# HaydenFaulkner/VidDet

Hardware: AMD Instinct MI355X
Metric: frames/sec (416x416) yolo3_darknet53 fwd+bwd (higher is better)
Workload: dtype f32; 1 GPU; yolo3_darknet53_coco training, batch 64/GPU, 416x416, fp32, fwd+bwd+SGD-momentum (BASELINE configs[2]; the reference trains with SGD, not Adam); classes=80, global_batch=64, parallelism=dp1, hip_graph=False

## Files before the change

### include/viddet_hip.h

```cpp
#ifndef VIDDET_HIP_H
#define VIDDET_HIP_H

#include <stdint.h>

#ifdef __cplusplus
extern "C" {
#endif

#define VD_OK            0
#define VD_EINVAL       -1
#define VD_ELAUNCH      -2
#define VD_EWORKSPACE   -3

#define VD_MAX_TAPS 27

#define VD_EPI_AFFINE    1
#define VD_EPI_LEAKY     2
#define VD_EPI_RESIDUAL  4
#define VD_MATH_SPLIT    16
#define VD_MATH_BF16     32

#define VD_MATH_F16X2    64
#define VD_MATH_NOHALO   128
#define VD_STORE_BF16    256
#define VD_WGRAD_HALO    512
#define VD_CONV_STREAMK  1024
#define VD_CONV_PARITY4  2048
#define VD_CONV_SPLITK   4096
#define VD_SK_MAX_WG        2048
#define VD_SK_HEADER_BYTES  32768
#define VD_SK_SPLIT_CNT_OFF   4096
#define VD_SK_SPLIT_MAX_TILES 4096
#define VD_SK_TIMEOUT_TICKS 4000
#define VD_AMAX_SLOTS    32
#define VD_AMAX_STRIDE   64
#define VD_AMAX_FLOATS   (VD_AMAX_SLOTS * VD_AMAX_STRIDE)

const char* vd_last_error(void);
int vd_version(void);
#define VD_ABI_VERSION 8
int vd_abi_version(void);
int64_t vd_sizeof_desc(int which);

typedef struct {
    const float* in;
    const float* wp;
    float*       out;
    const float* scale;
    const float* shift;
    const float* residual;
    int32_t N, Hi, Wi, Ci;
    int32_t Hg, Wg;
    int32_t in_stride;
    int32_t T;
    int32_t dy[VD_MAX_TAPS], dx[VD_MAX_TAPS];
    int32_t dz[VD_MAX_TAPS];
    int32_t Kfr;
    int32_t Ho, Wo, Co;
    int32_t out_stride, out_oy, out_ox;
    int32_t ldo, ldr;
    int32_t flags;
    float   slope;
    const float* in_scale;
    const float* in_shift;
    float   in_slope;
    int32_t tile;
    float*  stats_part;
    const float* bs_z;
    const float* bs_scale;
    const float* bs_shift;
    const float* bs_mean;
    const float* bs_invstd;
    float*  bs_part;
    float   bs_slope;
    const float* amax_in;
    const float* amax_w;
    float*  amax_out;
    void*   sk_ws;
    int64_t sk_ws_bytes;
    int32_t par_cin;
    int32_t par_mask;
} vd_conv_desc;

int vd_conv_igemm(const vd_conv_desc* d, void* stream);
int vd_conv_igemm_streamk(const vd_conv_desc* d);
int64_t vd_conv_igemm_streamk_ws_bytes(void);
int vd_conv_igemm_mtiles(const vd_conv_desc* d);

int vd_conv_igemm_bf16(const vd_conv_desc* d, int out_f32, void* stream);
int vd_conv_igemm_bf16_streamk(const vd_conv_desc* d, int out_f32);
int vd_conv_igemm_bf16_mtiles(const vd_conv_desc* d);
int vd_pack_weight_bf16(const float* wp_f32, void* wp_bf16, int Co, int Co_pad, int Ci, int Ci_pad, int T,
                        void* stream);
int vd_stem_im2col_bf16(const float* in, void* col, int N, int H, int W, int nchw, void* stream);

typedef struct {
    const float* in;
    const float* dout;
    float*       dwp;
    int32_t N, Hi, Wi, Ci;
    int32_t Hg, Wg, Co, ldd;
    int32_t in_stride;
    int32_t T;
    int32_t dy[VD_MAX_TAPS], dx[VD_MAX_TAPS];
    int32_t dz[VD_MAX_TAPS];
    int32_t Kfr;
    int32_t splits;
    const float* in_scale;
    const float* in_shift;
    float   in_slope;
    int32_t flags;
    const float* amax_in;
    const float* amax_dout;
} vd_wgrad_desc;

int64_t vd_conv_wgrad_ws_bytes(const vd_wgrad_desc* d);
int vd_conv_wgrad(const vd_wgrad_desc* d, void* ws, int64_t ws_bytes, void* stream);
int vd_conv_wgrad_uses_halo(const vd_wgrad_desc* d);

int vd_stem_conv_c32_bf16(const float* x_nchw, const float* stem_wp, const float* stem_scale, const float* stem_shift,
                          float stem_slope, const vd_conv_desc* d, void* stream);
int vd_stem_conv_blocks(int N, int H, int W);
int vd_stem_conv(const float* x_nchw, const float* wp, void* out, int ldo, int N, int H, int W, const float* scale,
                 const float* shift, float slope, int flags, int out_bf16, float* stats_part, void* stream);
int64_t vd_stem_wgrad_ws_bytes(int N, int H, int W);
int vd_stem_wgrad(const float* x_nchw, const float* dz, int ldd, float* dwp, int N, int H, int W, void* ws,
                  int64_t ws_bytes, void* stream);
int vd_stem_im2col(const float* in, float* col, int N, int H, int W, int nchw, void* stream);

int vd_pack_weight_fwd(const float* w_oihw, float* wp, int Co, int Co_pad, int Ci,
                       int kd, int kh, int kw, void* stream);
int vd_pack_weight_dgrad(const float* w_oihw, float* wp, int Co, int Co_pad, int Ci,
                         int kd, int kh, int kw, const int32_t* taps, int ntaps, int src_packed,
                         void* stream);
int vd_pack_weight_dgrad_s2(const float* wp_fwd, float* wp4, int Co, int Co_pad, int Ci, int32_t* par_mask, void* stream);
int vd_unpack_wgrad(const float* dwp, float* dw_oihw, int Co, int Ci, int kd, int kh, int kw,
                    void* stream);

int64_t vd_bn_stats_ws_bytes(int64_t M, int C);
int vd_bn_stats(const float* x, int64_t M, int C, double* sums, void* ws, int64_t ws_bytes,
                void* stream);
int64_t vd_bn_sum_partials_ws_bytes(int nblk, int C);
int vd_bn_sum_partials(const float* part, int nblk, int C, double* sums, void* ws, int64_t ws_bytes, void* stream);
int vd_bn_sum_finalize(const float* part, int nblk, int C, double* sums, double count, const float* gamma,
                       const float* beta, float eps, float momentum, float* running_mean, float* running_var,
                       float* scale, float* shift, float* save_mean, float* save_invstd, void* ws, int64_t ws_bytes,
                       void* stream);
int vd_bn_sum_param_grads(const float* part, int nblk, int C, double* sums2, float* dgamma, float* dbeta, void* ws,
                          int64_t ws_bytes, void* stream);
int vd_bn_finalize(const double* sums, double count, int C, const float* gamma, const float* beta,
                   float eps, float momentum, float* running_mean, float* running_var,
                   float* scale, float* shift, float* save_mean, float* save_invstd, void* stream);
int vd_bn_fold_eval(const float* gamma, const float* beta, const float* running_mean,
                    const float* running_var, float eps, int C, float* scale, float* shift,
                    void* stream);
int vd_bn_apply_leaky(const float* x, const float* scale, const float* shift, const float* residual,
                      float* y, int64_t M, int C, float slope, float* amax_out, void* stream);
int vd_bn_stream_grid(int64_t n_vec, int cvec, int* unroll);
int vd_bn_bwd_reduce(const float* x, const float* dy, const float* scale, const float* shift,
                     const float* save_mean, const float* save_invstd, int64_t M, int C, float slope,
                     double* sums2, void* ws, int64_t ws_bytes, void* stream);
int vd_bn_param_grads(const double* sums2, int C, float* dgamma, float* dbeta, void* stream);
int vd_bn_bwd_apply(const float* x, const float* dy, const float* scale, const float* shift,
                    const float* save_mean, const float* save_invstd,
                    const double* sums2, double count, int64_t M, int C, float slope,
                    float* dx, float* amax_out , void* stream);

typedef struct {
    const float* gamma;
    const float* beta;
    const float* scale;
    int32_t C;
    int32_t pad_;
} vd_guard_item;
int vd_range_guard(const vd_guard_item* items, int n, float thresh, float* ratios, int32_t* flags, void* stream);

int vd_amax_merge(const float* a, const float* b, float* out, void* stream);
int vd_amax(const float* x, int64_t n, float* amax, void* stream);
int vd_amax_segments(const float* base, const int64_t* seg, int nseg, float* amax, void* stream);

int vd_add(const float* a, const float* b, float* out, int64_t n, void* stream);
int vd_fill(float* out, float v, int64_t n, void* stream);
int vd_upsample2x_concat(const float* up, const float* route, float* out,
                         int N, int Ho, int Wo, int Cu, int Cr, void* stream);
int vd_upsample2x_concat_bwd(const float* dout, float* dup, float* droute,
                             int N, int Ho, int Wo, int Cu, int Cr, void* stream);
int vd_nchw_to_nhwc(const float* in, float* out, int N, int C, int H, int W, void* stream);
int vd_preprocess_u8_nhwc(const uint8_t* in, float* out, int64_t npix, void* stream);
int vd_preprocess_u8_nchw(const uint8_t* in, float* out, int N, int H, int W, void* stream);
int vd_temporal_pool(const float* x, float* y, int32_t* argmax, int B, int K, int64_t inner, int type,
                     void* stream);
int vd_temporal_pool_bwd(const float* dy, const int32_t* argmax, float* dx, int B, int K,
                         int64_t inner, int type, void* stream);
int vd_frame_slice(const float* x, float* y, int B, int K, int k0, int kc, int64_t inner, int backward, void* stream);
int vd_temporal_cat(const float* x, float* y, int B, int K, int64_t hw, int C, int backward, void* stream);
int vd_corr_fwd(const float* x, float* y, int B, int K, int H, int W, int C, int d, int ldy, void* stream);
int vd_corr_bwd(const float* dy, const float* x, float* dx, int B, int K, int H, int W, int C, int d, int ldy, void* stream);
int vd_corr_fwd_bf16(const void* x, void* y, int B, int K, int H, int W, int C, int d, int ldy, void* stream);

int vd_gru_gate_fwd(const float* I, const float* H, const float* hbias, const float* hprev, float* h, int B, int K, int t,
                    int64_t HW, int Ch, void* stream);
int vd_gru_gate_bwd(float* I, float* H, int h_valid, const float* hbias, const float* hprev, const float* dy, float dy_scale,
                    float* dh, int carry, int B, int K, int t, int64_t HW, int Ch, void* stream);
int vd_gru_avg(const float* hl, const float* hr, float* y, int B, int K, int64_t inner, float* amax_out, void* stream);

int vd_tdw_fwd(const float* x, const float* w, const float* res, float* y, int B, int K, int64_t HW, int C, float* amax_out,
               void* stream);
int64_t vd_tdw_bwd_ws_bytes(int B, int K, int64_t HW, int C);
int vd_tdw_bwd(const float* dy, const float* x, const float* w, float* dx, float* dw, int B, int K, int64_t HW, int C, void* ws,
               int64_t ws_bytes, void* stream);

typedef struct {
    const float* head[3];
    int32_t g[3];
    int32_t ldh;
    float   stride[3];
    float   anchors[3][6];
    int32_t B, C;
} vd_head_desc;

int vd_yolo_decode_filter(const vd_head_desc* h, float valid_thresh,
                          float* cand_score, int32_t* cand_row, int32_t cap, int32_t* counts,
                          void* stream);
int64_t vd_nms_ws_bytes(int B, int cap, int topk);
int vd_nms_topk(const vd_head_desc* h, const float* cand_score, const int32_t* cand_row,
                int32_t cap, const int32_t* counts, float nms_thresh, int topk, int post_nms,
                float* out_ids, float* out_scores, float* out_boxes, int32_t* out_rows,
                void* ws, int64_t ws_bytes, void* stream);
int vd_yolo_decode_filter_agnostic(const vd_head_desc* h, int head_bf16, float valid_thresh,
                                   float* cand_score, int32_t* cand_row, int32_t cap, int32_t* counts,
                                   void* stream);
int vd_nms_agnostic(const vd_head_desc* h, int head_bf16, const float* cand_score, const int32_t* cand_row,
                    int32_t cap, const int32_t* counts, float nms_thresh, int topk, int post_nms,
                    float* out_ids, float* out_scores, float* out_boxes, int32_t* out_rows,
                    void* ws, int64_t ws_bytes, void* stream);

int vd_yolo_loss_fwd_bwd(const vd_head_desc* h, const float* gt, int M,
                         const float* obj_t, const float* center_t, const float* scale_t,
                         const float* weight_t, const float* class_t,
                         float ignore_thresh, int label_smooth,
                         float* losses, float* const dhead[3], float* box_out,
                         float* const dhead_amax[3] ,
                         void* ws, int64_t ws_bytes, void* stream);
int64_t vd_yolo_loss_ws_bytes(const vd_head_desc* h);

int vd_sgd_momentum(float* w, const float* grad, float* mom, int64_t n,
                    float lr, float momentum, float wd, float rescale, void* stream);

int vd_bn_stats_bf16(const void* x, int64_t M, int C, double* sums, void* ws, int64_t ws_bytes, void* stream);
int vd_bn_apply_leaky_bf16(const void* x, const float* scale, const float* shift, const void* residual, void* y,
                           int64_t M, int C, float slope, void* stream);
int vd_bn_bwd_reduce_bf16(const void* x, const void* dy, const float* scale, const float* shift, const float* save_mean,
                          const float* save_invstd, int64_t M, int C, float slope, double* sums2, void* ws, int64_t ws_bytes,
                          void* stream);
int vd_bn_bwd_apply_bf16(const void* x, const void* dy, const float* scale, const float* shift, const float* save_mean,
                         const float* save_invstd, const double* sums2, double count, int64_t M, int C, float slope,
                         void* dx, void* stream);
int vd_pack_weight_dgrad_bf16(const float* w, void* wp_bf16, int Co, int Co_pad, int Ci, int kd, int kh, int kw,
                              const int32_t* taps, int ntaps, int src_packed, void* stream);
int vd_add_bf16(const void* a, const void* b, void* out, int64_t n, void* stream);
int vd_temporal_pool_bf16(const void* x, void* y, int B, int K, int64_t inner, int type, void* stream);
int vd_upsample2x_concat_bwd_bf16(const void* dout, void* dup, void* droute, int N, int Ho, int Wo, int Cu, int Cr, void* stream);
int vd_temporal_pool_train_bf16(const void* x, void* y, uint8_t* argmax_u8, int B, int K, int64_t inner, int type, void* stream);
int vd_temporal_pool_bwd_bf16(const void* dy, const uint8_t* argmax_u8, void* dx, int B, int K, int64_t inner, int type,
                              void* stream);
int vd_corr_bwd_bf16(const void* dy, const void* x, void* dx, int B, int K, int H, int W, int C, int d, int ldy, void* stream);
int vd_stem_wgrad_bf16(const float* x_nchw, const void* dz, int ldd, float* dwp, int N, int H, int W, void* ws, int64_t ws_bytes,
                       void* stream);
int vd_yolo_loss_fwd_bwd_bf16(const vd_head_desc* h, const float* gt, int M, const float* obj_t, const float* center_t,
                              const float* scale_t, const float* weight_t, const float* class_t, float ignore_thresh,
                              int label_smooth, float* losses, void* const dhead[3], float* box_out, void* ws, int64_t ws_bytes,
                              void* stream);

int vd_temporal_pool_idx(const float* ring, const int32_t* slots, float* y, int S, int B, int K, int64_t inner, int type,
                         void* stream);
int vd_temporal_pool_idx_bf16(const void* ring, const int32_t* slots, void* y, int S, int B, int K, int64_t inner, int type,
                              void* stream);
int vd_temporal_cat_idx(const float* ring, const int32_t* slots, float* y, int S, int B, int K, int64_t hw, int C, void* stream);

int vd_resize_u8_nchw(const uint8_t* in, float* out, uint8_t* out_u8, int N, int H0, int W0, int H, int W, const int32_t* idx_y,
                      const float* w_y, int Ty, const int32_t* idx_x, const float* w_x, int Tx, void* stream);

int vd_resize_nv12_nchw(const uint8_t* in, int64_t in_bytes, int64_t frame_stride, int64_t pitch, int64_t uv_offset, float* out,
                        uint8_t* out_u8, int N, int H0, int W0, int H, int W, const int32_t* idx_y, const float* w_y, int Ty,
                        const int32_t* idx_x, const float* w_x, int Tx, int off, int gain, int ru, int rv, int gu, int gv, int bu,
                        void* stream);

int vd_augment_u8_nchw(const uint8_t* raw, const int64_t* src_off, const int32_t* src_hw, const float* color, const int32_t* idx_y,
                       const float* w_y, int Ty, const int32_t* idx_x, const float* w_x, int Tx, const float* fill, float* out, int N,
                       int K, int H, int W, void* stream);

int vd_yolo_targets(const float* gt, const float* ids, int idw, const float* mix, int N, int M, int C, int H, int W, float* obj,
                    float* ctr, float* scl, float* wgt, float* cls, void* stream);

int vd_voc_match(const float* det_ids, const float* det_scores, const float* det_boxes, int B, int N, const float* gt, int M,
                 int gt_w, float clip_hi, float iou_thresh, int32_t* rec_cls, float* rec_score, int8_t* rec_hit, int32_t* npos,
                 int32_t* ndiff, int C, void* stream);

int vd_vid_match(const double* det, int B, int N, const double* gt, int M, const double* motion_ranges, const double* area_ranges,
                 double iou_thresh, double pixel_tolerance, int32_t* rec_gt, int32_t* rec_tp, int32_t* rec_fp, int32_t* img_nig,
                 int32_t* img_ngt, int32_t* npos, int32_t* nout, int C, void* stream);

int vd_coco_match(const double* det, int B, int N, const double* gt, int M, const double* iou_thrs, const double* area_rng,
                  int32_t* rec_rank, int32_t* rec_bits, int32_t* npig, int K, void* stream);

int vd_seq_nms(const float* ids, const float* scores, const float* bboxes, const int32_t* clip_start, int V, int F, int N,
               int num_class, float link_thresh, float nms_thresh, int rescore, float* out_ids, float* out_scores,
               float* out_bboxes, int32_t* out_perm, void* ws, int64_t ws_bytes, void* stream);
int vd_seq_nms_stages(const float* ids, const float* scores, const float* bboxes, const int32_t* clip_start, int V, int F, int N,
                      int num_class, float link_thresh, float nms_thresh, int rescore, float* out_ids, float* out_scores,
                      float* out_bboxes, int32_t* out_perm, void* ws, int64_t ws_bytes, int stages, void* stream);

#define VD_TRACK_WS_PER_ROW 8
int vd_track(const float* ids, const float* scores, const float* bboxes, const int32_t* clip_start, int V, int F, int N,
             int num_class, float sigma_l, float sigma_h, float sigma_iou, int t_min, int max_age, int32_t* out_track,
             int32_t* out_len, float* out_score, void* ws, int64_t ws_bytes, void* stream);

#ifdef __cplusplus
}
#endif
#endif
```

### viddet_amd/csrc/vd_bn.hip

```cpp
#include "vd_common.h"
#include <stdlib.h>

namespace {

constexpr int RED_THREADS = 256;

template <int MODE, typename T = float>
__global__ __launch_bounds__(RED_THREADS) void k_bn_partial(const T* __restrict__ x,
                                                            const T* __restrict__ dy,
                                                            const float* __restrict__ scale,
                                                            const float* __restrict__ shift,
                                                            const float* __restrict__ mean,
                                                            const float* __restrict__ invstd, int64_t M,
                                                            int C, float slope, float* __restrict__ part) {
    __shared__ f32x4 sa[RED_THREADS], sb[RED_THREADS];
    const int cvec = C >> 2;
    const int cblk = cvec < RED_THREADS ? cvec : RED_THREADS;
    const int rl = RED_THREADS / cblk;
    const int tcol = threadIdx.x % cblk, trow = threadIdx.x / cblk;
    const int64_t rows_per_blk = vd_cdiv(M, gridDim.x);
    const int64_t r0 = (int64_t)blockIdx.x * rows_per_blk;
    int64_t r1 = r0 + rows_per_blk;
    if (r1 > M) r1 = M;
    for (int cb = 0; cb < cvec; cb += cblk) {
        const int col = cb + tcol;
        f32x4 a = {0.f, 0.f, 0.f, 0.f}, b = {0.f, 0.f, 0.f, 0.f};
        if (trow < rl && col < cvec) {
            f32x4 sc, sh, mu, is;
            if (MODE == 1) {
                sc = reinterpret_cast<const f32x4*>(scale)[col];
                sh = reinterpret_cast<const f32x4*>(shift)[col];
                mu = reinterpret_cast<const f32x4*>(mean)[col];
                is = reinterpret_cast<const f32x4*>(invstd)[col];
            }
            for (int64_t r = r0 + trow; r < r1; r += rl) {
                const f32x4 v = vd_ld4(x, r * cvec + col);
                if (MODE == 0) {
                    a += v;
                    b += v * v;
                } else {
                    const f32x4 d = vd_ld4(dy, r * cvec + col);
#pragma unroll
                    for (int e = 0; e < 4; ++e) {
                        const float u = v[e] * sc[e] + sh[e];
                        const float g = u > 0.f ? d[e] : d[e] * slope;
                        a[e] += g;
                        b[e] += g * (v[e] - mu[e]) * is[e];
                    }
                }
            }
        }
        sa[threadIdx.x] = a;
        sb[threadIdx.x] = b;
        __syncthreads();
        if (trow == 0 && col < cvec) {
            for (int j = 1; j < rl; ++j) {
                a += sa[j * cblk + tcol];
                b += sb[j * cblk + tcol];
            }
            float* dst = part + (int64_t)blockIdx.x * 2 * C;
            reinterpret_cast<f32x4*>(dst)[col] = a;
            reinterpret_cast<f32x4*>(dst + C)[col] = b;
        }
        __syncthreads();
    }
}

template <int MODE>
__global__ __launch_bounds__(RED_THREADS) void k_bn_partial_bf16x8(const __bf16* __restrict__ x, const __bf16* __restrict__ dy,
                                                                   const float* __restrict__ scale, const float* __restrict__ shift,
                                                                   const float* __restrict__ mean, const float* __restrict__ invstd,
                                                                   int64_t M, int C, float slope, float* __restrict__ part) {
    __shared__ f32x8 sa[RED_THREADS], sb[RED_THREADS];
    const int cvec = C >> 3;
    const int cblk = cvec < RED_THREADS ? cvec : RED_THREADS;
    const int rl = RED_THREADS / cblk;
    const int tcol = threadIdx.x % cblk, trow = threadIdx.x / cblk;
    const int64_t rows_per_blk = vd_cdiv(M, gridDim.x);
    const int64_t r0 = (int64_t)blockIdx.x * rows_per_blk;
    int64_t r1 = r0 + rows_per_blk;
    if (r1 > M) r1 = M;
    for (int cb = 0; cb < cvec; cb += cblk) {
        const int col = cb + tcol;
        f32x8 a, b;
#pragma unroll
        for (int e = 0; e < 8; ++e) a[e] = b[e] = 0.f;
        if (trow < rl && col < cvec) {
            f32x8 sc, sh, mu, is;
            if (MODE == 1) {
#pragma unroll
                for (int e = 0; e < 8; ++e) {
                    sc[e] = scale[col * 8 + e]; sh[e] = shift[col * 8 + e];
                    mu[e] = mean[col * 8 + e]; is[e] = invstd[col * 8 + e];
                }
            }
            for (int64_t r = r0 + trow; r < r1; r += 2 * rl) {
                const bool two = r + rl < r1;
                const f32x8 v0 = vd_ld8(x, r * cvec + col);
                const f32x8 v1 = two ? vd_ld8(x, (r + rl) * cvec + col) : f32x8{0, 0, 0, 0, 0, 0, 0, 0};
                if (MODE == 0) {
                    a += v0 + v1;
                    b += v0 * v0 + v1 * v1;
                } else {
                    const f32x8 d0 = vd_ld8(dy, r * cvec + col);
                    const f32x8 d1 = two ? vd_ld8(dy, (r + rl) * cvec + col) : f32x8{0, 0, 0, 0, 0, 0, 0, 0};
#pragma unroll
                    for (int e = 0; e < 8; ++e) {
                        const float u0 = v0[e] * sc[e] + sh[e], u1 = v1[e] * sc[e] + sh[e];
                        const float g0 = u0 > 0.f ? d0[e] : d0[e] * slope, g1 = u1 > 0.f ? d1[e] : d1[e] * slope;
                        a[e] += g0 + g1;
                        b[e] += g0 * (v0[e] - mu[e]) * is[e] + (two ? g1 * (v1[e] - mu[e]) * is[e] : 0.f);
                    }
                }
            }
        }
        sa[threadIdx.x] = a;
        sb[threadIdx.x] = b;
        __syncthreads();
        if (trow == 0 && col < cvec) {
            for (int j = 1; j < rl; ++j) {
                a += sa[j * cblk + tcol];
                b += sb[j * cblk + tcol];
            }
            float* dst = part + (int64_t)blockIdx.x * 2 * C;
#pragma unroll
            for (int e = 0; e < 8; ++e) {
                dst[col * 8 + e] = a[e];
                dst[C + col * 8 + e] = b[e];
            }
        }
        __syncthreads();
    }
}

__global__ __launch_bounds__(1024) void k_bn_sum_partials(const float* __restrict__ part, int nblk, int C2,
                                                          double* __restrict__ sums) {
    __shared__ double sh[16][64];
    const int cx = threadIdx.x & 63, sl = threadIdx.x >> 6;
    const int i = blockIdx.x * 64 + cx;
    double s = 0.0;
    if (i < C2) {
        int b = sl;
        for (; b + 48 < nblk; b += 64) {
            const float p0 = part[(int64_t)b * C2 + i], p1 = part[(int64_t)(b + 16) * C2 + i];
            const float p2 = part[(int64_t)(b + 32) * C2 + i], p3 = part[(int64_t)(b + 48) * C2 + i];
            s += (double)p0; s += (double)p1; s += (double)p2; s += (double)p3;
        }
        for (; b < nblk; b += 16) s += (double)part[(int64_t)b * C2 + i];
    }
    sh[sl][cx] = s;
    __syncthreads();
    if (sl == 0 && i < C2) {
        double t = 0.0;
// ... 41 lines not shown
__global__ void k_bn_sum_partials_l2(const double* __restrict__ in, int rows, int C2, double* __restrict__ sums) {
    const int i = blockIdx.x * blockDim.x + threadIdx.x;
    if (i >= C2) return;
    double s = 0.0;
    int r = 0;
    for (; r + 8 <= rows; r += 8) {
        double v[8];
#pragma unroll
        for (int u = 0; u < 8; ++u) v[u] = in[(int64_t)(r + u) * C2 + i];
#pragma unroll
        for (int u = 0; u < 8; ++u) s += v[u];
    }
    for (; r < rows; ++r) s += in[(int64_t)r * C2 + i];
    sums[i] = s;
}

__global__ void k_bn_finalize(const double* __restrict__ sums, double count, int C,
                              const float* __restrict__ gamma, const float* __restrict__ beta, float eps,
                              float momentum, float* __restrict__ rmean, float* __restrict__ rvar,
                              float* __restrict__ scale, float* __restrict__ shift,
                              float* __restrict__ smean, float* __restrict__ sinv) {
    const int c = blockIdx.x * blockDim.x + threadIdx.x;
    if (c >= C) return;
    const double mean = sums[c] / count;
    double var = sums[C + c] / count - mean * mean;
    if (var < 0.0) var = 0.0;
    const float invstd = (float)(1.0 / sqrt(var + (double)eps));
    const float g = gamma[c], b = beta[c];
    const float sc = g * invstd;
    scale[c] = sc;
    shift[c] = b - (float)mean * sc;
    if (smean) smean[c] = (float)mean;
    if (sinv) sinv[c] = invstd;
    if (rmean) rmean[c] = rmean[c] * momentum + (float)mean * (1.f - momentum);
    if (rvar) rvar[c] = rvar[c] * momentum + (float)var * (1.f - momentum);
}

template <int MODE>
__global__ __launch_bounds__(1024) void k_bn_sum_fused(const float* __restrict__ part, int nblk, int C, double* __restrict__ sums,
                                                       double count, const float* __restrict__ gamma,
                                                       const float* __restrict__ beta, float eps, float momentum,
                                                       float* __restrict__ rmean, float* __restrict__ rvar,
                                                       float* __restrict__ scale, float* __restrict__ shift,
                                                       float* __restrict__ smean, float* __restrict__ sinv,
                                                       float* __restrict__ dgamma, float* __restrict__ dbeta) {
    __shared__ double sh[16][64];
    const int cx = threadIdx.x & 63, sl = threadIdx.x >> 6;
    const int ch = blockIdx.x * 32 + (cx & 31);
    const int col = (cx >> 5) * C + ch;
    double s = 0.0;
    if (ch < C) {
        const int C2 = 2 * C;
        int b = sl;
        for (; b + 48 < nblk; b += 64) {
            const float p0 = part[(int64_t)b * C2 + col], p1 = part[(int64_t)(b + 16) * C2 + col];
            const float p2 = part[(int64_t)(b + 32) * C2 + col], p3 = part[(int64_t)(b + 48) * C2 + col];
            s += (double)p0; s += (double)p1; s += (double)p2; s += (double)p3;
        }
        for (; b < nblk; b += 16) s += (double)part[(int64_t)b * C2 + col];
    }
    sh[sl][cx] = s;
    __syncthreads();
    if (sl == 0 && ch < C) {
        double t = 0.0;
#pragma unroll
        for (int j = 0; j < 16; ++j) t += sh[j][cx];
        sums[col] = t;
        sh[0][cx] = t;
    }
    __syncthreads();
    if (threadIdx.x < 32 && ch < C) {
        const double a = sh[0][threadIdx.x], bq = sh[0][32 + threadIdx.x];
        if (MODE == 0) {
            const double mean = a / count;
            double var = bq / count - mean * mean;
            if (var < 0.0) var = 0.0;
            const float invstd = (float)(1.0 / sqrt(var + (double)eps));
            const float sc = gamma[ch] * invstd;
            scale[ch] = sc;
            shift[ch] = beta[ch] - (float)mean * sc;
            if (smean) smean[ch] = (float)mean;
            if (sinv) sinv[ch] = invstd;
            if (rmean) rmean[ch] = rmean[ch] * momentum + (float)mean * (1.f - momentum);
            if (rvar) rvar[ch] = rvar[ch] * momentum + (float)var * (1.f - momentum);
        } else {
            dbeta[ch] = (float)a;
            dgamma[ch] = (float)bq;
        }
    }
}

constexpr int SUMP_FUSED = 1024;

__global__ void k_bn_fold_eval(const float* __restrict__ gamma, const float* __restrict__ beta,
                               const float* __restrict__ rmean, const float* __restrict__ rvar, float eps,
                               int C, float* __restrict__ scale, float* __restrict__ shift) {
    const int c = blockIdx.x * blockDim.x + threadIdx.x;
    if (c >= C) return;
    const float sc = gamma[c] / sqrtf(rvar[c] + eps);
    scale[c] = sc;
    shift[c] = beta[c] - rmean[c] * sc;
}

template <typename T = float>
__global__ void k_bn_apply_leaky_v0(const T* __restrict__ x, const float* __restrict__ scale,
                                 const float* __restrict__ shift, const T* __restrict__ res,
                                 T* __restrict__ y, int64_t n4, int cvec, float slope, float* __restrict__ amax) {
    const int64_t i0 = (int64_t)blockIdx.x * blockDim.x + threadIdx.x;
    const int col = (int)(i0 % cvec);
    const f32x4 sc = reinterpret_cast<const f32x4*>(scale)[col];
    const f32x4 sh = reinterpret_cast<const f32x4*>(shift)[col];
    float amx = 0.f;
    for (int64_t i = i0; i < n4; i += (int64_t)gridDim.x * blockDim.x) {
        const f32x4 v = vd_ld4(x, i);
        f32x4 o;
#pragma unroll
        for (int e = 0; e < 4; ++e) {
            const float u = v[e] * sc[e] + sh[e];
            o[e] = u > 0.f ? u : u * slope;
        }
        if (res) o += vd_ld4(res, i);
        vd_st4(y, i, o);
        amx = fmaxf(amx, fmaxf(fmaxf(fabsf(o[0]), fabsf(o[1])), fmaxf(fabsf(o[2]), fabsf(o[3]))));
    }
    if (amax) vd_amax_publish(amax, amx);
}

template <typename T = float>
__global__ void k_bn_bwd_apply_v0(const T* __restrict__ x, const T* __restrict__ dy,
                               const float* __restrict__ scale, const float* __restrict__ shift,
                               const float* __restrict__ mean, const float* __restrict__ invstd,
                               const double* __restrict__ sums2, double count, int64_t n4, int C,
                               float slope, T* __restrict__ dx, float* __restrict__ amax) {
    const int cvec = C >> 2;
    const float inv_count = (float)(1.0 / count);
    const int64_t i0 = (int64_t)blockIdx.x * blockDim.x + threadIdx.x;
    const int col = (int)(i0 % cvec);
    const f32x4 sc = reinterpret_cast<const f32x4*>(scale)[col];
    const f32x4 sh = reinterpret_cast<const f32x4*>(shift)[col];
    const f32x4 mu = reinterpret_cast<const f32x4*>(mean)[col];
    const f32x4 is = reinterpret_cast<const f32x4*>(invstd)[col];
    f32x4 mg, mgx;
#pragma unroll
    for (int e = 0; e < 4; ++e) {
        mg[e] = (float)sums2[col * 4 + e] * inv_count;
        mgx[e] = (float)sums2[C + col * 4 + e] * inv_count;
    }
    float amx = 0.f;
    for (int64_t i = i0; i < n4; i += (int64_t)gridDim.x * blockDim.x) {
        const f32x4 v = vd_ld4(x, i);
        const f32x4 d = vd_ld4(dy, i);
        f32x4 o;
#pragma unroll
        for (int e = 0; e < 4; ++e) {
            const float u = v[e] * sc[e] + sh[e];
            const float g = u > 0.f ? d[e] : d[e] * slope;
            const float xh = (v[e] - mu[e]) * is[e];
            o[e] = sc[e] * (g - mg[e] - xh * mgx[e]);
        }
        vd_st4(dx, i, o);
        amx = fmaxf(amx, fmaxf(fmaxf(fabsf(o[0]), fabsf(o[1])), fmaxf(fabsf(o[2]), fabsf(o[3]))));
    }
    if (amax) vd_amax_publish(amax, amx);
}

typedef unsigned int u32x2 __attribute__((ext_vector_type(2)));
typedef unsigned int u32x4 __attribute__((ext_vector_type(4)));
template <int V> struct bn_vec { typedef f32x4 type; };
template <> struct bn_vec<8> { typedef f32x8 type; };

template <int V, bool NT> struct bn_io;
template <bool NT> struct bn_io<4, NT> {
    static __device__ __forceinline__ f32x4 ld(const float* p, int64_t i) {
        const f32x4* q = reinterpret_cast<const f32x4*>(p) + i;
        return NT ? __builtin_nontemporal_load(q) : *q;
    }
    static __device__ __forceinline__ f32x4 ld(const __bf16* p, int64_t i) {
        const u32x2* q = reinterpret_cast<const u32x2*>(p) + i;
        const vd_bf16x4 v = __builtin_bit_cast(vd_bf16x4, NT ? __builtin_nontemporal_load(q) : *q);
        return f32x4{(float)v[0], (float)v[1], (float)v[2], (float)v[3]};
    }
    template <typename T> static __device__ __forceinline__ void st(T* p, int64_t i, const f32x4 v) { vd_st4(p, i, v); }
};
template <bool NT> struct bn_io<8, NT> {
    static __device__ __forceinline__ f32x8 ld(const __bf16* p, int64_t i) {
        const u32x4* q = reinterpret_cast<const u32x4*>(p) + i;
        const vd_bf16x8 v = __builtin_bit_cast(vd_bf16x8, NT ? __builtin_nontemporal_load(q) : *q);
        f32x8 o;
#pragma unroll
        for (int e = 0; e < 8; ++e) o[e] = (float)v[e];
        return o;
    }
    static __device__ __forceinline__ void st(__bf16* p, int64_t i, const f32x8 v) { vd_st8(p, i, v); }
};

template <int V, typename VEC> __device__ __forceinline__ float bn_vec_amax(float amx, const VEC o) {
    float m = fmaxf(fmaxf(fabsf(o[0]), fabsf(o[1])), fmaxf(fabsf(o[2]), fabsf(o[3])));
    if (V == 8) m = fmaxf(m, fmaxf(fmaxf(fabsf(o[4]), fabsf(o[5])), fmaxf(fabsf(o[6]), fabsf(o[7]))));
    return fmaxf(amx, m);
}

template <typename T, int V, int U, bool NT, bool FULL, typename VEC>
__device__ __forceinline__ void bn_apply_trip(const T* __restrict__ x, const T* __restrict__ res, T* __restrict__ y, int64_t i,
                                              int64_t stride, int64_t nv, const VEC sc, const VEC sh, float slope, float& amx) {
    VEC v[U], r[U];
    bool ok[U];
#pragma unroll
    for (int j = 0; j < U; ++j) {
        ok[j] = FULL || i + j * stride < nv;
        if (ok[j]) v[j] = bn_io<V, NT>::ld(x, i + j * stride);
    }
    if (res) {
#pragma unroll
        for (int j = 0; j < U; ++j)
            if (ok[j]) r[j] = bn_io<V, false>::ld(res, i + j * stride);
    }
    __builtin_amdgcn_sched_barrier(0);
#pragma unroll
    for (int j = 0; j < U; ++j) {
        if (!ok[j]) continue;
        VEC o;
#pragma unroll
        for (int e = 0; e < V; ++e) {
            const float u = v[j][e] * sc[e] + sh[e];
            o[e] = u > 0.f ? u : u * slope;
        }
        if (res) o += r[j];
        bn_io<V, false>::st(y, i + j * stride, o);
        amx = bn_vec_amax<V>(amx, o);
    }
}

template <typename T, int V, int U, bool NT>
__global__ __launch_bounds__(256) void k_bn_apply_leaky(const T* __restrict__ x, const float* __restrict__ scale,
                                                        const float* __restrict__ shift, const T* __restrict__ res,
                                                        T* __restrict__ y, int64_t nv, int cvec, float slope,
                                                        float* __restrict__ amax, int step) {
    typedef typename bn_vec<V>::type VEC;
    const int64_t span = (int64_t)step * 256;
    const int64_t i = (int64_t)(blockIdx.x / step) * U * span + (blockIdx.x % step) * 256 + threadIdx.x;
    const int col = (int)(i % cvec);
    VEC sc, sh;
#pragma unroll
    for (int e = 0; e < V; ++e) {
        sc[e] = scale[col * V + e];
        sh[e] = shift[col * V + e];
    }
    float amx = 0.f;
    if (i + (U - 1) * span < nv) bn_apply_trip<T, V, U, NT, true>(x, res, y, i, span, nv, sc, sh, slope, amx);
    else if (i < nv) bn_apply_trip<T, V, U, NT, false>(x, res, y, i, span, nv, sc, sh, slope, amx);
    if (amax) vd_amax_publish(amax, amx);
}

template <typename VEC> struct bn_bwd_consts { VEC sc, sh, mu, is, mg, mgx; };

template <typename T, int V, int U, bool NT, bool FULL, typename VEC>
__device__ __forceinline__ void bn_bwd_trip(const T* __restrict__ x, const T* __restrict__ dy, T* __restrict__ dx, int64_t i,
                                            int64_t stride, int64_t nv, const bn_bwd_consts<VEC>& k, float slope, float& amx) {
    VEC v[U], d[U];
    bool ok[U];
#pragma unroll
    for (int j = 0; j < U; ++j) {
        ok[j] = FULL || i + j * stride < nv;
        if (ok[j]) {
            v[j] = bn_io<V, NT>::ld(x, i + j * stride);
            d[j] = bn_io<V, NT>::ld(dy, i + j * stride);
        }
    }
    __builtin_amdgcn_sched_barrier(0);
#pragma unroll
    for (int j = 0; j < U; ++j) {
        if (!ok[j]) continue;
        VEC o;
#pragma unroll
        for (int e = 0; e < V; ++e) {
            const float u = v[j][e] * k.sc[e] + k.sh[e];
            const float g = u > 0.f ? d[j][e] : d[j][e] * slope;
            const float xh = (v[j][e] - k.mu[e]) * k.is[e];
            o[e] = k.sc[e] * (g - k.mg[e] - xh * k.mgx[e]);
        }
        bn_io<V, false>::st(dx, i + j * stride, o);
        amx = bn_vec_amax<V>(amx, o);
    }
}

template <typename T, int V, int U, bool NT>
__global__ __launch_bounds__(256) void k_bn_bwd_apply(const T* __restrict__ x, const T* __restrict__ dy,
                                                      const float* __restrict__ scale, const float* __restrict__ shift,
                                                      const float* __restrict__ mean, const float* __restrict__ invstd,
                                                      const double* __restrict__ sums2, double count, int64_t nv, int C,
                                                      float slope, T* __restrict__ dx, float* __restrict__ amax, int step) {
    typedef typename bn_vec<V>::type VEC;
    const int cvec = C / V;
    const float inv_count = (float)(1.0 / count);
    const int64_t span = (int64_t)step * 256;
    const int64_t i = (int64_t)(blockIdx.x / step) * U * span + (blockIdx.x % step) * 256 + threadIdx.x;
    const int col = (int)(i % cvec);
    bn_bwd_consts<VEC> k;
#pragma unroll
    for (int e = 0; e < V; ++e) {
        k.sc[e] = scale[col * V + e];
        k.sh[e] = shift[col * V + e];
        k.mu[e] = mean[col * V + e];
        k.is[e] = invstd[col * V + e];
        k.mg[e] = (float)sums2[col * V + e] * inv_count;
        k.mgx[e] = (float)sums2[C + col * V + e] * inv_count;
    }
    float amx = 0.f;
    if (i + (U - 1) * span < nv) bn_bwd_trip<T, V, U, NT, true>(x, dy, dx, i, span, nv, k, slope, amx);
    else if (i < nv) bn_bwd_trip<T, V, U, NT, false>(x, dy, dx, i, span, nv, k, slope, amx);
    if (amax) vd_amax_publish(amax, amx);
}

__global__ void k_bn_param_grads(const double* __restrict__ sums2, int C, float* __restrict__ dgamma,
                                 float* __restrict__ dbeta) {
    const int c = blockIdx.x * blockDim.x + threadIdx.x;
    if (c >= C) return;
    dbeta[c] = (float)sums2[c];
    dgamma[c] = (float)sums2[C + c];
}

bool bf16x8_enabled() {
    static const int v = getenv("VD_BN_BF16X8") ? atoi(getenv("VD_BN_BF16X8")) : 1;
    return v != 0;
}

int red_blocks(int64_t M) {
    int64_t nb = vd_cdiv(M, 64);
    if (nb > 1024) nb = 1024;
    if (nb < 1) nb = 1;
    return (int)nb;
}

int stream_blocks(int64_t n) {
    int64_t nb = vd_cdiv(n, 256);
    if (nb > 4096) nb = 4096;
    if (nb < 1) nb = 1;
    return (int)nb;
}

int fixed_col_blocks(int64_t n4, int cvec) {
    int a = 256, b = cvec;
    while (b) { const int t = a % b; a = b; b = t; }
    const int64_t step = cvec / a;
    int64_t nb = stream_blocks(n4);
    nb = vd_cdiv(nb, step) * step;
    return (int)nb;
}

bool bn_stream_enabled() {
    static const int v = getenv("VD_BN_STREAM") ? atoi(getenv("VD_BN_STREAM")) : 1;
    return v != 0;
}

constexpr int64_t BN_NT_MIN_BYTES = (int64_t)128 << 20;
constexpr int BN_UNROLL = 4;

int stream_step(int cvec) {
    int a = 256, b = cvec;
    while (b) { const int t = a % b; a = b; b = t; }
    return cvec / a;
}

int64_t stream_grid(int64_t nv, int cvec) {
    const int64_t step = stream_step(cvec);
    return vd_cdiv(nv, BN_UNROLL * step * 256) * step;
}

bool aligned16(const void* a, const void* b, const void* c) {
    return (((uintptr_t)a | (uintptr_t)b | (uintptr_t)c) & 15) == 0;
}

template <typename T, int V>
void launch_apply(const T* x, const float* scale, const float* shift, const T* res, T* y, int64_t M, int C, float slope,
                  float* amax, hipStream_t s) {
    const int cvec = C / V;
    const int64_t nv = M * cvec;
    const int step = stream_step(cvec);
    const dim3 g((unsigned)stream_grid(nv, cvec)), b(256);
    const bool nt = nv * V * (int64_t)sizeof(T) >= BN_NT_MIN_BYTES;
#define VD_GO(NT_) hipLaunchKernelGGL((k_bn_apply_leaky<T, V, BN_UNROLL, NT_>), g, b, 0, s, x, scale, shift, res, y, nv, cvec, slope, amax, step)
    if (nt) VD_GO(true); else VD_GO(false);
#undef VD_GO
}

template <typename T, int V>
void launch_bwd_apply(const T* x, const T* dy, const float* scale, const float* shift, const float* mean, const float* invstd,
                      const double* sums2, double count, int64_t M, int C, float slope, T* dx, float* amax, hipStream_t s) {
    const int cvec = C / V;
    const int64_t nv = M * cvec;
    const int step = stream_step(cvec);
    const dim3 g((unsigned)stream_grid(nv, cvec)), b(256);
    const bool nt = nv * V * (int64_t)sizeof(T) >= BN_NT_MIN_BYTES;
#define VD_GO(NT_) hipLaunchKernelGGL((k_bn_bwd_apply<T, V, BN_UNROLL, NT_>), g, b, 0, s, x, dy, scale, shift, mean, invstd, sums2, count, nv, C, slope, dx, amax, step)
    if (nt) VD_GO(true); else VD_GO(false);
#undef VD_GO
}

__global__ void k_range_guard(const vd_guard_item* __restrict__ items, float thresh, float* __restrict__ ratios,
                              int32_t* __restrict__ flags) {
    const vd_guard_item it = items[blockIdx.x];
    float lo[2] = {3.0e38f, 3.0e38f}, hi[2] = {0.f, 0.f};
    for (int c = threadIdx.x; c < it.C; c += blockDim.x) {
        const float u = fabsf(it.gamma[c]) + fabsf(it.beta[c]);
        const float v = it.scale ? fabsf(it.scale[c]) : 1.f;
        lo[0] = fminf(lo[0], u); hi[0] = fmaxf(hi[0], u);
        lo[1] = fminf(lo[1], v); hi[1] = fmaxf(hi[1], v);
    }
    __shared__ float red[4][4];
#pragma unroll
    for (int k = 0; k < 2; ++k) {
#pragma unroll
        for (int off = 32; off > 0; off >>= 1) {
            lo[k] = fminf(lo[k], __shfl_xor(lo[k], off));
            hi[k] = fmaxf(hi[k], __shfl_xor(hi[k], off));
        }
    }
    const int wave = threadIdx.x >> 6;
    if ((threadIdx.x & 63) == 0) { red[wave][0] = lo[0]; red[wave][1] = hi[0]; red[wave][2] = lo[1]; red[wave][3] = hi[1]; }
    __syncthreads();
    if (threadIdx.x == 0) {
        const int nw = blockDim.x >> 6;
        float a = red[0][0], b = red[0][1], c2 = red[0][2], d = red[0][3];
        for (int w = 1; w < nw; ++w) { a = fminf(a, red[w][0]); b = fmaxf(b, red[w][1]); c2 = fminf(c2, red[w][2]); d = fmaxf(d, red[w][3]); }
        const float r0 = b > 0.f ? a / b : 1.f, r1 = d > 0.f ? c2 / d : 1.f;
        ratios[2 * blockIdx.x] = r0;
        ratios[2 * blockIdx.x + 1] = r1;
        flags[2 * blockIdx.x] = r0 < thresh ? 1 : 0;
        flags[2 * blockIdx.x + 1] = r1 < thresh ? 1 : 0;
    }
}

}
// ... 251 lines not shown
```

### viddet_amd/csrc/vd_stem.hip

```cpp
#include "vd_common.h"
#include <stdlib.h>

namespace {

typedef __bf16 bf16x4 __attribute__((ext_vector_type(4)));

constexpr int SC = 32;
constexpr int SK = 27;
constexpr int SPX = 256;

template <bool OUT_BF16, bool MF = false>
__global__ __launch_bounds__(SPX) void k_stem_fwd(const float* __restrict__ x, const float* __restrict__ w,
                                                  void* __restrict__ out, int ldo, int N, int H, int W,
                                                  const float* __restrict__ scale, const float* __restrict__ shift,
                                                  float slope, int flags, float* __restrict__ stats_part) {
    __shared__ float tile[SPX][SC + 1];
    if constexpr (MF) {
        typedef __bf16 bf16x8_t __attribute__((ext_vector_type(8)));
        const int tid = threadIdx.x, lane = tid & 63, wave = tid >> 6;
        const int64_t HW = (int64_t)H * W;
        const int64_t P = (int64_t)N * HW;
        const int hh = lane >> 5;
        bf16x8_t b0, b1;
#pragma unroll
        for (int e = 0; e < 8; ++e) {
            b0[e] = (__bf16)w[(lane & 31) * 32 + 8 * hh + e];
            b1[e] = (__bf16)w[(lane & 31) * 32 + 16 + 8 * hh + e];
        }
#pragma unroll
        for (int gsel = 0; gsel < 2; ++gsel) {
            const int prow = wave * 64 + gsel * 32 + (lane & 31);
            const int64_t pix = (int64_t)blockIdx.x * SPX + prow;
            bf16x8_t a0, a1;
            {
                const bool pin = pix < P;
                const int64_t pp = pin ? pix : 0;
                const int n = (int)(pp / HW);
                const int r = (int)(pp - (int64_t)n * HW);
                const int y = r / W, xx = r - y * W;
                const float* xn = x + (int64_t)n * 3 * HW;
                float v[16];
#pragma unroll
                for (int e = 0; e < 16; ++e) {
                    const int k = (e < 8 ? 8 * hh : 16 + 8 * hh) + (e & 7);
                    const int tap = k / 3, c = k - 3 * tap;
                    const int iy = y + tap / 3 - 1, ix = xx + tap % 3 - 1;
                    const bool ok = pin && k < SK && (unsigned)iy < (unsigned)H && (unsigned)ix < (unsigned)W;
                    const float t = xn[ok ? (int64_t)c * HW + (int64_t)iy * W + ix : 0];
                    v[e] = ok ? t : 0.f;
                }
#pragma unroll
                for (int e = 0; e < 8; ++e) { a0[e] = (__bf16)v[e]; a1[e] = (__bf16)v[8 + e]; }
            }
            f32x16 acc;
#pragma unroll
            for (int r2 = 0; r2 < 16; ++r2) acc[r2] = 0.f;
            acc = __builtin_amdgcn_mfma_f32_32x32x16_bf16(a0, b0, acc, 0, 0, 0);
            acc = __builtin_amdgcn_mfma_f32_32x32x16_bf16(a1, b1, acc, 0, 0, 0);
            const int co = lane & 31;
            const float sc = (flags & VD_EPI_AFFINE) ? scale[co] : 1.f, sh = (flags & VD_EPI_AFFINE) ? shift[co] : 0.f;
#pragma unroll
            for (int r2 = 0; r2 < 16; ++r2) {
                float t = acc[r2];
                if (flags & VD_EPI_AFFINE) t = t * sc + sh;
                if (flags & VD_EPI_LEAKY) t = t > 0.f ? t : t * slope;
                tile[wave * 64 + gsel * 32 + (r2 & 3) + 8 * (r2 >> 2) + 4 * hh][co] = t;
            }
        }
        __syncthreads();
    } else {
    __shared__ __attribute__((aligned(16))) float wT[SK][SC];
    const int tid = threadIdx.x;
    for (int i = tid; i < SK * SC; i += SPX) wT[i / SC][i % SC] = w[(i % SC) * 32 + i / SC];
    __syncthreads();
    const int64_t HW = (int64_t)H * W;
    const int64_t P = (int64_t)N * HW;
    const int64_t pix = (int64_t)blockIdx.x * SPX + tid;
    float acc[SC];
#pragma unroll
    for (int c = 0; c < SC; ++c) acc[c] = 0.f;
    if (pix < P) {
        const int n = (int)(pix / HW);
        const int r = (int)(pix - (int64_t)n * HW);
        const int y = r / W, xx = r - y * W;
        const float* xn = x + (int64_t)n * 3 * HW;
        float xv[SK];
#pragma unroll
        for (int ky = 0; ky < 3; ++ky)
#pragma unroll
            for (int kx = 0; kx < 3; ++kx) {
                const int iy = y + ky - 1, ix = xx + kx - 1;
                const bool ok = (unsigned)iy < (unsigned)H && (unsigned)ix < (unsigned)W;
                const int64_t o = ok ? (int64_t)iy * W + ix : 0;
#pragma unroll
                for (int c = 0; c < 3; ++c) {
                    const float t = xn[(int64_t)c * HW + o];
                    xv[(ky * 3 + kx) * 3 + c] = ok ? t : 0.f;
                }
            }
#pragma unroll
        for (int k = 0; k < SK; ++k) {
#pragma unroll
            for (int c4 = 0; c4 < SC; c4 += 4) {
                const f32x4 wv = *reinterpret_cast<const f32x4*>(&wT[k][c4]);
#pragma unroll
                for (int e = 0; e < 4; ++e) acc[c4 + e] = fmaf(xv[k], wv[e], acc[c4 + e]);
            }
            __builtin_amdgcn_sched_barrier(0);
        }
    }
#pragma unroll
    for (int c = 0; c < SC; ++c) {
        float v = acc[c];
        if (flags & VD_EPI_AFFINE) v = v * scale[c] + shift[c];
        if (flags & VD_EPI_LEAKY) v = v > 0.f ? v : v * slope;
        tile[tid][c] = v;
    }
    __syncthreads();
    }
    const int tid = threadIdx.x;
    const int64_t P = (int64_t)N * H * W;
    if (stats_part) {
        __shared__ float red[8][2 * SC];
        const int c = tid & 31, seg = tid >> 5;
        float s1 = 0.f, s2 = 0.f;
#pragma unroll 8
        for (int r = seg * 32; r < seg * 32 + 32; ++r) {
            const float v = tile[r][c];
            s1 += v;
            s2 += v * v;
        }
        red[seg][c] = s1;
        red[seg][SC + c] = s2;
        __syncthreads();
        if (tid < 2 * SC) {
            float t = 0.f;
#pragma unroll
            for (int q = 0; q < 8; ++q) t += red[q][tid];
            stats_part[(int64_t)blockIdx.x * 2 * SC + tid] = t;
        }
    }
    const int64_t p0 = (int64_t)blockIdx.x * SPX;
#pragma unroll
    for (int j = 0; j < 8; ++j) {
        const int pl = (tid >> 3) + 32 * j, c4 = (tid & 7) * 4;
        if (p0 + pl < P) {
            const f32x4 v = {tile[pl][c4], tile[pl][c4 + 1], tile[pl][c4 + 2], tile[pl][c4 + 3]};
            if (OUT_BF16) {
                bf16x4 o;
#pragma unroll
                for (int e = 0; e < 4; ++e) o[e] = (__bf16)v[e];
                *reinterpret_cast<bf16x4*>(reinterpret_cast<__bf16*>(out) + (p0 + pl) * ldo + c4) = o;
            } else {
                *reinterpret_cast<f32x4*>(reinterpret_cast<float*>(out) + (p0 + pl) * ldo + c4) = v;
            }
        }
    }
}

template <typename T>
__global__ __launch_bounds__(256) void k_stem_wgrad(const float* __restrict__ x, const T* __restrict__ dz, int ldd,
                                                    float* __restrict__ part, int N, int H, int W, int64_t px_per_wave) {
    const int lane = threadIdx.x & 63, wave = threadIdx.x >> 6;
    const int64_t HW = (int64_t)H * W, P = (int64_t)N * HW;
    const int64_t gw = (int64_t)blockIdx.x * 4 + wave;
    const int64_t p_begin = gw * px_per_wave;
    int64_t p_end = p_begin + px_per_wave;
    if (p_end > P) p_end = P;
    const int k = lane & 31, par = lane >> 5;
    const bool k_ok = k < SK;
    const int c = k_ok ? k % 3 : 0, tap = k_ok ? k / 3 : 0;
    const int dy = tap / 3 - 1, dx = tap % 3 - 1;
    f32x16 acc;
#pragma unroll
    for (int r = 0; r < 16; ++r) acc[r] = 0.f;
    int64_t p = p_begin + par;
    int n = 0, y = 0, xx = 0;
    if (p < P) {
        n = (int)(p / HW);
        const int r = (int)(p - (int64_t)n * HW);
        y = r / W;
        xx = r - y * W;
    }
    constexpr int UNR = 8;
    for (; p - par < p_end; p += 2 * UNR) {
        float a[UNR], b[UNR];
#pragma unroll
        for (int u = 0; u < UNR; ++u) {
            const int64_t pu = p + 2 * u;
            const bool in_run = pu < p_end;
            a[u] = in_run ? (float)dz[pu * ldd + k] : 0.f;
            const int iy = y + dy, ix = xx + dx;
            const bool ok = in_run && k_ok && (unsigned)iy < (unsigned)H && (unsigned)ix < (unsigned)W;
            b[u] = ok ? x[((int64_t)n * 3 + c) * HW + (int64_t)iy * W + ix] : 0.f;
            xx += 2;
            while (xx >= W) { xx -= W; ++y; }
            if (y >= H) { y -= H; ++n; }
        }
#pragma unroll
        for (int u = 0; u < UNR; ++u) acc = __builtin_amdgcn_mfma_f32_32x32x2f32(a[u], b[u], acc, 0, 0, 0);
    }
    float* dst = part + gw * (SC * 32);
#pragma unroll
    for (int r = 0; r < 16; ++r) {
        const int co = (r & 3) + 8 * (r >> 2) + 4 * (lane >> 5);
        dst[co * 32 + (lane & 31)] = acc[r];
    }
}

constexpr int SROWS = 4;
template <typename T>
__global__ __launch_bounds__(256) void k_stem_wgrad_rows(const float* __restrict__ x, const T* __restrict__ dz, int ldd,
                                                         float* __restrict__ part, int N, int H, int W, int P) {
    extern __shared__ float win[];
    const int tid = threadIdx.x, lane = tid & 63, wave = tid >> 6;
    const int groups = (H + SROWS - 1) / SROWS;
    const int n = blockIdx.x / groups, y0 = (blockIdx.x % groups) * SROWS;
    const int64_t HW = (int64_t)H * W;
    const float* xn = x + (int64_t)n * 3 * HW;
    for (int i = tid; i < 3 * (SROWS + 2) * P; i += 256) {
        const int col = i % P - 1, rr = i / P;
        const int c = rr / (SROWS + 2), iy = y0 - 1 + rr % (SROWS + 2);
        const bool ok = (unsigned)iy < (unsigned)H && (unsigned)col < (unsigned)W;
        win[i] = ok ? xn[(int64_t)c * HW + (int64_t)iy * W + col] : 0.f;
    }
    __syncthreads();
    const int k = lane & 31, par = lane >> 5;
    const bool k_ok = k < SK;
    const int c = k_ok ? k % 3 : 0, tap = k_ok ? k / 3 : 0;
    const int y = y0 + wave;
    f32x16 acc;
#pragma unroll
    for (int r = 0; r < 16; ++r) acc[r] = 0.f;
    if (y < H) {
        const float* b0 = win + (c * (SROWS + 2) + wave + tap / 3) * P + (tap % 3) + par;
        const T* a0 = dz + ((int64_t)n * HW + (int64_t)y * W + par) * ldd + k;
        constexpr int UNR = 8;
        for (int x0 = 0; x0 < W; x0 += 2 * UNR) {
            float a[UNR], b[UNR];
#pragma unroll
            for (int u = 0; u < UNR; ++u) {
                const bool in = x0 + 2 * u + par < W;
                a[u] = in ? (float)a0[(int64_t)(x0 + 2 * u) * ldd] : 0.f;
                b[u] = (in && k_ok) ? b0[x0 + 2 * u] : 0.f;
            }
#pragma unroll
            for (int u = 0; u < UNR; ++u) acc = __builtin_amdgcn_mfma_f32_32x32x2f32(a[u], b[u], acc, 0, 0, 0);
        }
    }
    __syncthreads();
#pragma unroll
    for (int r = 0; r < 16; ++r) {
        const int co = (r & 3) + 8 * (r >> 2) + 4 * (lane >> 5);
        win[wave * (SC * 32) + co * 32 + (lane & 31)] = acc[r];
    }
    __syncthreads();
    float* dst = part + (int64_t)blockIdx.x * (SC * 32);
    for (int i = tid; i < SC * 32; i += 256)
        dst[i] = ((win[i] + win[SC * 32 + i]) + win[2 * SC * 32 + i]) + win[3 * SC * 32 + i];
}

__global__ void k_stem_wgrad_reduce(const float* __restrict__ part, int nparts, float* __restrict__ dst) {
    const int i = blockIdx.x * blockDim.x + threadIdx.x;
    if (i >= SC * 32) return;
    const int per = (nparts + gridDim.y - 1) / gridDim.y;
    int q = blockIdx.y * per;
    int q1 = q + per;
    if (q1 > nparts) q1 = nparts;
    float s = 0.f;
    for (; q + 8 <= q1; q += 8) {
        float v[8];
#pragma unroll
        for (int u = 0; u < 8; ++u) v[u] = part[(int64_t)(q + u) * (SC * 32) + i];
#pragma unroll
        for (int u = 0; u < 8; ++u) s += v[u];
    }
    for (; q < q1; ++q) s += part[(int64_t)q * (SC * 32) + i];
    dst[(int64_t)blockIdx.y * (SC * 32) + i] = s;
}

constexpr int STEM_RED_CHUNKS = 64;
constexpr int64_t STEM_WG_WAVES = 8192;

}

extern "C" {

int vd_stem_conv_blocks(int N, int H, int W) { return (int)vd_cdiv((int64_t)N * H * W, SPX); }

int vd_stem_conv(const float* x_nchw, const float* wp, void* out, int ldo, int N, int H, int W, const float* scale,
                 const float* shift, float slope, int flags, int out_bf16, float* stats_part, void* stream) {
    VD_REQUIRE(x_nchw && wp && out && N > 0 && H > 0 && W > 0 && ldo >= SC && ldo % 4 == 0, "vd_stem_conv: bad args");
    VD_REQUIRE(!(flags & VD_EPI_AFFINE) || (scale && shift), "vd_stem_conv: affine epilogue needs scale and shift");
    VD_REQUIRE(!stats_part || flags == 0, "vd_stem_conv: fused statistics need the raw output (they come from the fp32 values, bf16 output or not)");
    VD_REQUIRE((int64_t)N * H * W < (1ll << 31), "vd_stem_conv: pixel count overflows int32");
    const int nb = vd_stem_conv_blocks(N, H, W);
    static const int use_mf = getenv("VD_STEM_MFMA") ? atoi(getenv("VD_STEM_MFMA")) : 1;
    if (out_bf16 && use_mf)
        hipLaunchKernelGGL((k_stem_fwd<true, true>), dim3(nb), dim3(SPX), 0, (hipStream_t)stream, x_nchw, wp, out, ldo, N, H, W,
                           scale, shift, slope, flags, stats_part);
    else if (out_bf16)
        hipLaunchKernelGGL(k_stem_fwd<true>, dim3(nb), dim3(SPX), 0, (hipStream_t)stream, x_nchw, wp, out, ldo, N, H, W,
                           scale, shift, slope, flags, stats_part);
    else
        hipLaunchKernelGGL(k_stem_fwd<false>, dim3(nb), dim3(SPX), 0, (hipStream_t)stream, x_nchw, wp, out, ldo, N, H, W,
                           scale, shift, slope, flags, stats_part);
    VD_CHECK_LAUNCH("vd_stem_conv");
    return VD_OK;
}

static int stem_rows_pitch(int W) {
    int p = W + 2;
    while (p % 32 != 4) ++p;
    return p;
}
static int64_t stem_rows_lds(int W) {
    const int64_t win = (int64_t)3 * (SROWS + 2) * stem_rows_pitch(W) * 4, tiles = (int64_t)4 * SC * 32 * 4;
    return win > tiles ? win : tiles;
}
static bool stem_rows_ok(int W) {
    static const int on = getenv("VD_STEM_WGRAD_ROWS") ? atoi(getenv("VD_STEM_WGRAD_ROWS")) : 1;
    return on && stem_rows_lds(W) <= 64 * 1024;
}
static int64_t stem_run_waves(int N, int H, int W) {
    const int64_t P = (int64_t)N * H * W;
    int64_t waves = vd_cdiv(P, 256);
    if (waves > STEM_WG_WAVES) waves = STEM_WG_WAVES;
    return vd_cdiv(waves, 4) * 4;
}

int64_t vd_stem_wgrad_ws_bytes(int N, int H, int W) {
    const int64_t tiles_rows = (int64_t)N * vd_cdiv(H, SROWS), tiles_run = stem_run_waves(N, H, W);
    const int64_t tiles = tiles_rows > tiles_run ? tiles_rows : tiles_run;
    return (tiles + STEM_RED_CHUNKS) * SC * 32 * (int64_t)sizeof(float);
}

static int stem_wgrad_any(const float* x_nchw, const void* dz, int dz_bf16, int ldd, float* dwp, int N, int H, int W, void* ws,
                         int64_t ws_bytes, void* stream) {
    VD_REQUIRE(x_nchw && dz && dwp && N > 0 && H > 0 && W > 0 && ldd >= SC, "vd_stem_wgrad: bad args");
    const int64_t need = vd_stem_wgrad_ws_bytes(N, H, W);
    if (!ws || ws_bytes < need) {
        vd_set_error("vd_stem_wgrad: workspace %lld < %lld", (long long)ws_bytes, (long long)need);
        return VD_EWORKSPACE;
    }
    hipStream_t s = (hipStream_t)stream;
    int64_t tiles;
    if (stem_rows_ok(W)) {
        tiles = (int64_t)N * vd_cdiv(H, SROWS);
        const int P = stem_rows_pitch(W), lds = (int)stem_rows_lds(W);
        if (dz_bf16)
            hipLaunchKernelGGL(k_stem_wgrad_rows<__bf16>, dim3((unsigned)tiles), dim3(256), lds, s, x_nchw, (const __bf16*)dz, ldd,
                               (float*)ws, N, H, W, P);
        else
            hipLaunchKernelGGL(k_stem_wgrad_rows<float>, dim3((unsigned)tiles), dim3(256), lds, s, x_nchw, (const float*)dz, ldd,
                               (float*)ws, N, H, W, P);
    } else {
        const int64_t P = (int64_t)N * H * W;
        tiles = stem_run_waves(N, H, W);
        int64_t ppw = vd_cdiv(P, tiles);
        ppw = vd_cdiv(ppw, 2) * 2;
        if (dz_bf16)
            hipLaunchKernelGGL(k_stem_wgrad<__bf16>, dim3((unsigned)(tiles / 4)), dim3(256), 0, s, x_nchw, (const __bf16*)dz, ldd, (float*)ws,
                               N, H, W, ppw);
        else
            hipLaunchKernelGGL(k_stem_wgrad<float>, dim3((unsigned)(tiles / 4)), dim3(256), 0, s, x_nchw, (const float*)dz, ldd, (float*)ws,
                               N, H, W, ppw);
    }
    VD_CHECK_LAUNCH("vd_stem_wgrad");
    float* lvl1 = (float*)ws + tiles * (SC * 32);
    hipLaunchKernelGGL(k_stem_wgrad_reduce, dim3(4, STEM_RED_CHUNKS), dim3(256), 0, s, (const float*)ws, (int)tiles, lvl1);
    VD_CHECK_LAUNCH("vd_stem_wgrad/reduce1");
    hipLaunchKernelGGL(k_stem_wgrad_reduce, dim3(4, 1), dim3(256), 0, s, (const float*)lvl1, STEM_RED_CHUNKS, dwp);
    VD_CHECK_LAUNCH("vd_stem_wgrad/reduce2");
    return VD_OK;
}

int vd_stem_wgrad(const float* x_nchw, const float* dz, int ldd, float* dwp, int N, int H, int W, void* ws, int64_t ws_bytes,
                  void* stream) {
    return stem_wgrad_any(x_nchw, dz, 0, ldd, dwp, N, H, W, ws, ws_bytes, stream);
}

int vd_stem_wgrad_bf16(const float* x_nchw, const void* dz, int ldd, float* dwp, int N, int H, int W, void* ws, int64_t ws_bytes,
                       void* stream) {
    return stem_wgrad_any(x_nchw, dz, 1, ldd, dwp, N, H, W, ws, ws_bytes, stream);
}

}
```

### viddet_amd/lib.py

```python
import ctypes as C
import os

_HERE = os.path.dirname(os.path.abspath(__file__))
LIB_PATH = os.environ.get("VD_LIB") or os.path.join(_HERE, "csrc", "libviddet_hip.so")

ABI_VERSION = 8
VOC_MATCH_MAX_DET, VOC_MATCH_MAX_GT = 1024, 512
VID_MATCH_MAX_DET, VID_MATCH_MAX_GT = 1024, 512
COCO_MATCH_MAX_DET, COCO_MATCH_MAX_GT = 1024, 512
SEQ_NMS_MAX_ROWS = 128
SEQ_NMS_WS_PER_ROW = 48
TRACK_MAX_ROWS, TRACK_MAX_ACTIVE = 128, 1024
TRACK_WS_PER_ROW = 8
VD_MAX_TAPS = 27
EPI_AFFINE, EPI_LEAKY, EPI_RESIDUAL = 1, 2, 4
MATH_SPLIT = 16
MATH_BF16 = 32
MATH_F16X2 = 64
MATH_NOHALO = 128
STORE_BF16 = 256
WGRAD_HALO = 512
CONV_STREAMK = 1024
CONV_SPLITK = 4096
CONV_PARITY4 = 2048
SK_HEADER_BYTES = 32768
AMAX_SLOTS, AMAX_STRIDE = 32, 64
AMAX_FLOATS = AMAX_SLOTS * AMAX_STRIDE
BN_STREAM_UNROLL = 4

_fp = C.c_void_p


class ConvDesc(C.Structure):
    _fields_ = [
        ("in_", _fp), ("wp", _fp), ("out", _fp), ("scale", _fp), ("shift", _fp), ("residual", _fp),
        ("N", C.c_int32), ("Hi", C.c_int32), ("Wi", C.c_int32), ("Ci", C.c_int32),
        ("Hg", C.c_int32), ("Wg", C.c_int32), ("in_stride", C.c_int32), ("T", C.c_int32),
        ("dy", C.c_int32 * VD_MAX_TAPS), ("dx", C.c_int32 * VD_MAX_TAPS), ("dz", C.c_int32 * VD_MAX_TAPS),
        ("Kfr", C.c_int32),
        ("Ho", C.c_int32), ("Wo", C.c_int32), ("Co", C.c_int32),
        ("out_stride", C.c_int32), ("out_oy", C.c_int32), ("out_ox", C.c_int32),
        ("ldo", C.c_int32), ("ldr", C.c_int32), ("flags", C.c_int32), ("slope", C.c_float),
        ("in_scale", _fp), ("in_shift", _fp), ("in_slope", C.c_float), ("tile", C.c_int32),
        ("stats_part", _fp),
        ("bs_z", _fp), ("bs_scale", _fp), ("bs_shift", _fp), ("bs_mean", _fp), ("bs_invstd", _fp), ("bs_part", _fp),
        ("bs_slope", C.c_float),
        ("amax_in", _fp), ("amax_w", _fp), ("amax_out", _fp),
        ("sk_ws", _fp), ("sk_ws_bytes", C.c_int64),
        ("par_cin", C.c_int32), ("par_mask", C.c_int32),
    ]


class WgradDesc(C.Structure):
    _fields_ = [
        ("in_", _fp), ("dout", _fp), ("dwp", _fp),
        ("N", C.c_int32), ("Hi", C.c_int32), ("Wi", C.c_int32), ("Ci", C.c_int32),
        ("Hg", C.c_int32), ("Wg", C.c_int32), ("Co", C.c_int32), ("ldd", C.c_int32),
        ("in_stride", C.c_int32), ("T", C.c_int32),
        ("dy", C.c_int32 * VD_MAX_TAPS), ("dx", C.c_int32 * VD_MAX_TAPS), ("dz", C.c_int32 * VD_MAX_TAPS),
        ("Kfr", C.c_int32), ("splits", C.c_int32),
        ("in_scale", _fp), ("in_shift", _fp), ("in_slope", C.c_float), ("flags", C.c_int32),
        ("amax_in", _fp), ("amax_dout", _fp),
    ]


class GuardItem(C.Structure):
    _fields_ = [("gamma", _fp), ("beta", _fp), ("scale", _fp), ("C", C.c_int32), ("pad_", C.c_int32)]


class HeadDesc(C.Structure):
    _fields_ = [
        ("head", _fp * 3), ("g", C.c_int32 * 3), ("ldh", C.c_int32),
        ("stride", C.c_float * 3), ("anchors", (C.c_float * 6) * 3),
        ("B", C.c_int32), ("C", C.c_int32),
    ]


_i, _i64, _f, _d, _p = C.c_int, C.c_int64, C.c_float, C.c_double, C.c_void_p
SIGNATURES = {
    "vd_last_error": (C.c_char_p, []),
    "vd_version": (_i, []),
    "vd_abi_version": (_i, []),
    "vd_sizeof_desc": (_i64, [_i]),
    "vd_conv_igemm": (_i, [C.POINTER(ConvDesc), _p]),
    "vd_conv_igemm_mtiles": (_i, [C.POINTER(ConvDesc)]),
    "vd_conv_igemm_streamk": (_i, [C.POINTER(ConvDesc)]),
    "vd_conv_igemm_streamk_ws_bytes": (_i64, []),
    "vd_conv_igemm_bf16": (_i, [C.POINTER(ConvDesc), _i, _p]),
    "vd_conv_igemm_bf16_mtiles": (_i, [C.POINTER(ConvDesc)]),
    "vd_conv_igemm_bf16_streamk": (_i, [C.POINTER(ConvDesc), _i]),
    "vd_pack_weight_bf16": (_i, [_p, _p, _i, _i, _i, _i, _i, _p]),
    "vd_stem_im2col_bf16": (_i, [_p, _p, _i, _i, _i, _i, _p]),
    "vd_conv_wgrad_ws_bytes": (_i64, [C.POINTER(WgradDesc)]),
    "vd_conv_wgrad": (_i, [C.POINTER(WgradDesc), _p, _i64, _p]),
    "vd_conv_wgrad_uses_halo": (_i, [C.POINTER(WgradDesc)]),
    "vd_stem_im2col": (_i, [_p, _p, _i, _i, _i, _i, _p]),
    "vd_pack_weight_fwd": (_i, [_p, _p, _i, _i, _i, _i, _i, _i, _p]),
    "vd_pack_weight_dgrad": (_i, [_p, _p, _i, _i, _i, _i, _i, _i, C.POINTER(C.c_int32), _i, _i, _p]),
    "vd_pack_weight_dgrad_s2": (_i, [_p, _p, _i, _i, _i, C.POINTER(C.c_int32), _p]),
    "vd_unpack_wgrad": (_i, [_p, _p, _i, _i, _i, _i, _i, _p]),
    "vd_bn_stats_ws_bytes": (_i64, [_i64, _i]),
    "vd_bn_stats": (_i, [_p, _i64, _i, _p, _p, _i64, _p]),
    "vd_bn_sum_partials_ws_bytes": (_i64, [_i, _i]),
    "vd_bn_sum_partials": (_i, [_p, _i, _i, _p, _p, _i64, _p]),
    "vd_bn_finalize": (_i, [_p, _d, _i, _p, _p, _f, _f, _p, _p, _p, _p, _p, _p, _p]),
    "vd_bn_sum_finalize": (_i, [_p, _i, _i, _p, _d, _p, _p, _f, _f, _p, _p, _p, _p, _p, _p, _p, _i64, _p]),
    "vd_bn_sum_param_grads": (_i, [_p, _i, _i, _p, _p, _p, _p, _i64, _p]),
    "vd_bn_fold_eval": (_i, [_p, _p, _p, _p, _f, _i, _p, _p, _p]),
    "vd_bn_stream_grid": (_i, [_i64, _i, _p]),
    "vd_bn_apply_leaky": (_i, [_p, _p, _p, _p, _p, _i64, _i, _f, _p, _p]),
    "vd_bn_bwd_reduce": (_i, [_p, _p, _p, _p, _p, _p, _i64, _i, _f, _p, _p, _i64, _p]),
    "vd_bn_param_grads": (_i, [_p, _i, _p, _p, _p]),
    "vd_bn_bwd_apply": (_i, [_p, _p, _p, _p, _p, _p, _p, _d, _i64, _i, _f, _p, _p, _p]),
    "vd_range_guard": (_i, [_p, _i, _f, _p, _p, _p]),
    "vd_amax": (_i, [_p, _i64, _p, _p]),
    "vd_amax_segments": (_i, [_p, _p, _i, _p, _p]),
    "vd_amax_merge": (_i, [_p, _p, _p, _p]),
    "vd_add": (_i, [_p, _p, _p, _i64, _p]),
    "vd_fill": (_i, [_p, _f, _i64, _p]),
    "vd_upsample2x_concat": (_i, [_p, _p, _p, _i, _i, _i, _i, _i, _p]),
    "vd_upsample2x_concat_bwd": (_i, [_p, _p, _p, _i, _i, _i, _i, _i, _p]),
    "vd_nchw_to_nhwc": (_i, [_p, _p, _i, _i, _i, _i, _p]),
    "vd_stem_conv_blocks": (_i, [_i, _i, _i]),
    "vd_stem_conv": (_i, [_p, _p, _p, _i, _i, _i, _i, _p, _p, C.c_float, _i, _i, _p, _p]),
    "vd_stem_conv_c32_bf16": (_i, [_p, _p, _p, _p, C.c_float, C.POINTER(ConvDesc), _p]),
    "vd_stem_wgrad_ws_bytes": (_i64, [_i, _i, _i]),
    "vd_stem_wgrad": (_i, [_p, _p, _i, _p, _i, _i, _i, _p, _i64, _p]),
    "vd_preprocess_u8_nhwc": (_i, [_p, _p, _i64, _p]),
    "vd_preprocess_u8_nchw": (_i, [_p, _p, _i, _i, _i, _p]),
    "vd_temporal_pool": (_i, [_p, _p, _p, _i, _i, _i64, _i, _p]),
    "vd_temporal_pool_bwd": (_i, [_p, _p, _p, _i, _i, _i64, _i, _p]),
    "vd_temporal_cat": (_i, [_p, _p, _i, _i, _i64, _i, _i, _p]),
    "vd_corr_fwd": (_i, [_p, _p, _i, _i, _i, _i, _i, _i, _i, _p]),
    "vd_corr_bwd": (_i, [_p, _p, _p, _i, _i, _i, _i, _i, _i, _i, _p]),
    "vd_corr_fwd_bf16": (_i, [_p, _p, _i, _i, _i, _i, _i, _i, _i, _p]),
    "vd_corr_bwd_bf16": (_i, [_p, _p, _p, _i, _i, _i, _i, _i, _i, _i, _p]),
    "vd_gru_gate_fwd": (_i, [_p, _p, _p, _p, _p, _i, _i, _i, _i64, _i, _p]),
    "vd_gru_gate_bwd": (_i, [_p, _p, _i, _p, _p, _p, _f, _p, _i, _i, _i, _i, _i64, _i, _p]),
    "vd_gru_avg": (_i, [_p, _p, _p, _i, _i, _i64, _p, _p]),
    "vd_tdw_fwd": (_i, [_p, _p, _p, _p, _i, _i, _i64, _i, _p, _p]),
    "vd_tdw_bwd_ws_bytes": (_i64, [_i, _i, _i64, _i]),
    "vd_tdw_bwd": (_i, [_p, _p, _p, _p, _p, _i, _i, _i64, _i, _p, _i64, _p]),
    "vd_frame_slice": (_i, [_p, _p, _i, _i, _i, _i, _i64, _i, _p]),
    "vd_yolo_decode_filter": (_i, [C.POINTER(HeadDesc), _f, _p, _p, C.c_int32, _p, _p]),
    "vd_nms_ws_bytes": (_i64, [_i, _i, _i]),
    "vd_nms_topk": (_i, [C.POINTER(HeadDesc), _p, _p, C.c_int32, _p, _f, _i, _i, _p, _p, _p, _p, _p, _i64, _p]),
    "vd_yolo_decode_filter_agnostic": (_i, [C.POINTER(HeadDesc), _i, _f, _p, _p, C.c_int32, _p, _p]),
    "vd_nms_agnostic": (_i, [C.POINTER(HeadDesc), _i, _p, _p, C.c_int32, _p, _f, _i, _i, _p, _p, _p, _p, _p, _i64, _p]),
    "vd_yolo_loss_ws_bytes": (_i64, [C.POINTER(HeadDesc)]),
    "vd_yolo_loss_fwd_bwd": (_i, [C.POINTER(HeadDesc), _p, _i, _p, _p, _p, _p, _p, _f, _i, _p,
                                  C.POINTER(_fp * 3), _p, C.POINTER(_fp * 3), _p, _i64, _p]),
    "vd_sgd_momentum": (_i, [_p, _p, _p, _i64, _f, _f, _f, _f, _p]),
    "vd_bn_stats_bf16": (_i, [_p, _i64, _i, _p, _p, _i64, _p]),
    "vd_bn_apply_leaky_bf16": (_i, [_p, _p, _p, _p, _p, _i64, _i, _f, _p]),
    "vd_bn_bwd_reduce_bf16": (_i, [_p, _p, _p, _p, _p, _p, _i64, _i, _f, _p, _p, _i64, _p]),
    "vd_bn_bwd_apply_bf16": (_i, [_p, _p, _p, _p, _p, _p, _p, _d, _i64, _i, _f, _p, _p]),
    "vd_add_bf16": (_i, [_p, _p, _p, _i64, _p]),
    "vd_temporal_pool_bf16": (_i, [_p, _p, _i, _i, _i64, _i, _p]),
    "vd_temporal_pool_train_bf16": (_i, [_p, _p, _p, _i, _i, _i64, _i, _p]),
    "vd_temporal_pool_bwd_bf16": (_i, [_p, _p, _p, _i, _i, _i64, _i, _p]),
    "vd_pack_weight_dgrad_bf16": (_i, [_p, _p, _i, _i, _i, _i, _i, _i, C.POINTER(C.c_int32), _i, _i, _p]),
    "vd_upsample2x_concat_bwd_bf16": (_i, [_p, _p, _p, _i, _i, _i, _i, _i, _p]),
    "vd_stem_wgrad_bf16": (_i, [_p, _p, _i, _p, _i, _i, _i, _p, _i64, _p]),
    "vd_yolo_loss_fwd_bwd_bf16": (_i, [C.POINTER(HeadDesc), _p, _i, _p, _p, _p, _p, _p, _f, _i, _p,
                                       C.POINTER(_fp * 3), _p, _p, _i64, _p]),
    "vd_temporal_pool_idx": (_i, [_p, _p, _p, _i, _i, _i, _i64, _i, _p]),
    "vd_temporal_pool_idx_bf16": (_i, [_p, _p, _p, _i, _i, _i, _i64, _i, _p]),
    "vd_temporal_cat_idx": (_i, [_p, _p, _p, _i, _i, _i, _i64, _i, _p]),
    "vd_resize_u8_nchw": (_i, [_p, _p, _p, _i, _i, _i, _i, _i, _p, _p, _i, _p, _p, _i, _p]),
    "vd_resize_nv12_nchw": (_i, [_p, _i64, _i64, _i64, _i64, _p, _p, _i, _i, _i, _i, _i, _p, _p, _i, _p, _p, _i,
                                 _i, _i, _i, _i, _i, _i, _i, _p]),
    "vd_augment_u8_nchw": (_i, [_p, _p, _p, _p, _p, _p, _i, _p, _p, _i, _p, _p, _i, _i, _i, _i, _p]),
    "vd_yolo_targets": (_i, [_p, _p, _i, _p, _i, _i, _i, _i, _i, _p, _p, _p, _p, _p, _p]),
    "vd_voc_match": (_i, [_p, _p, _p, _i, _i, _p, _i, _i, _f, _f, _p, _p, _p, _p, _p, _i, _p]),
    "vd_vid_match": (_i, [_p, _i, _i, _p, _i, _p, _p, _d, _d, _p, _p, _p, _p, _p, _p, _p, _i, _p]),
    "vd_coco_match": (_i, [_p, _i, _i, _p, _i, _p, _p, _p, _p, _p, _i, _p]),
    "vd_seq_nms": (_i, [_p, _p, _p, _p, _i, _i, _i, _i, _f, _f, _i, _p, _p, _p, _p, _p, _i64, _p]),
    "vd_seq_nms_stages": (_i, [_p, _p, _p, _p, _i, _i, _i, _i, _f, _f, _i, _p, _p, _p, _p, _p, _i64, _i, _p]),
    "vd_track": (_i, [_p, _p, _p, _p, _i, _i, _i, _i, _f, _f, _f, _i, _i, _p, _p, _p, _p, _i64, _p]),
}

_lib = None


class VidDetHipError(RuntimeError):
    pass


def load():
    global _lib
    if _lib is not None:
        return _lib
    if not os.path.exists(LIB_PATH):
        raise VidDetHipError(
            "libviddet_hip.so not built (%s). Run `python -c 'import __graft_entry__ as g; g.build()'` "
            "or `make -C viddet_amd/csrc`. There is no CPU fallback." % LIB_PATH)
    import torch
    lib = C.CDLL(LIB_PATH)
    for name, (res, args) in SIGNATURES.items():
        fn = getattr(lib, name)
        fn.restype = res
        fn.argtypes = args
    if lib.vd_abi_version() != ABI_VERSION:
        raise VidDetHipError("%s has ABI revision %d, this binding is written for %d: rebuild (make -C viddet_amd/csrc)"
                             % (LIB_PATH, lib.vd_abi_version(), ABI_VERSION))
    for i, st in enumerate((ConvDesc, WgradDesc, HeadDesc)):
        if lib.vd_sizeof_desc(i) != C.sizeof(st):
            raise VidDetHipError("%s: sizeof(%s) is %d in the library, %d in this binding" %
                                 (LIB_PATH, st.__name__, lib.vd_sizeof_desc(i), C.sizeof(st)))
    _lib = lib
    return lib


def check(rc, what=""):
    if rc != 0:
        raise VidDetHipError("%s failed (rc=%d): %s" % (what, rc, load().vd_last_error().decode()))


def stream_ptr():
    import torch
    return C.c_void_p(torch.cuda.current_stream().cuda_stream)


def ptr(t):
    if t is None:
        return None
    return C.c_void_p(t.data_ptr())
```

### viddet_amd/model.py

```python
import ctypes as C
import math
import os
import re
from collections import OrderedDict

import numpy as np
import torch

from . import lib as L
from . import ops
from .lib import ConvDesc, WgradDesc, EPI_AFFINE, EPI_LEAKY, EPI_RESIDUAL
from .ops import round_up, fwd_taps, dgrad_plans

from .consts import BN_EPS, BN_MOMENTUM, LEAKY_SLOPE


class Slot:

    def __init__(self):
        self.value = None


class Program:

    def __init__(self):
        self.recs = []
        self.meta = []
        self.keep = []
        self.streams = []

    def add(self, fname, *args, meta=None, stream=None):
        fn = getattr(L.load(), fname)
        self.recs.append((fname, fn, args))
        self.meta.append(meta)
        self.streams.append(stream)

    def add_py(self, fn):
        self.recs.append((None, fn, ()))
        self.meta.append(None)
        self.streams.append(None)

    def add_coll(self, fn):
        self.recs.append((None, fn, ()))
        self.meta.append(dict(kind='collective'))
        self.streams.append(None)

    def hold(self, *objs):
        self.keep.extend(objs)

    def run(self):
        s = L.stream_ptr()
        for (fname, fn, args), st in zip(self.recs, self.streams):
            if fname is None:
                fn()
                continue
            a = [x.value if isinstance(x, Slot) else x for x in args]
            rc = fn(*a, s if st is None else C.c_void_p(st.cuda_stream))
            if rc != 0:
                L.check(rc, fname)

    def run_timed(self, select):
        s = L.stream_ptr()
        out = []
        for (fname, fn, args), meta in zip(self.recs, self.meta):
            if fname is None:
                if meta and meta.get('kind') == 'collective':
                    fn()
                continue
            a = [x.value if isinstance(x, Slot) else x for x in args]
            if fname in select:
                e0, e1 = torch.cuda.Event(enable_timing=True), torch.cuda.Event(enable_timing=True)
                e0.record()
                rc = fn(*a, s)
                e1.record()
                if fname in ("vd_conv_igemm", "vd_conv_wgrad"):
                    d = args[0]._obj
                    meta = dict(meta or {}, split=bool(d.flags & L.MATH_SPLIT), bf16=bool(d.flags & L.MATH_BF16),
                                f16x2=bool(d.flags & L.MATH_F16X2), nohalo=bool(d.flags & L.MATH_NOHALO), tile=int(getattr(d, "tile", 0)),
                                streamk=bool(fname == "vd_conv_igemm" and L.load().vd_conv_igemm_streamk(args[0])))
                    if fname == "vd_conv_wgrad":
                        meta["wgrad_halo"] = bool(L.load().vd_conv_wgrad_uses_halo(args[0]))
                    if fname == "vd_conv_igemm" and meta.get("bytes"):
                        out_bytes = 4.0 * d.N * d.Hg * d.Wg * d.Co
                        extra = (out_bytes if d.residual else 0.0) + (out_bytes if getattr(d, "bs_part", None) else 0.0)
                        meta["bytes_epilogue_reads"] = extra
                        meta["bytes"] = meta["bytes"] + extra
                if fname == "vd_conv_igemm_bf16":
                    form = int(L.load().vd_conv_igemm_bf16_streamk(args[0], args[1]))
                    meta = dict(meta or {}, tile=int(args[0]._obj.tile), nohalo=bool(args[0]._obj.flags & L.MATH_NOHALO),
                                streamk=form == 1, splitk=form == 2)
                out.append((fname, meta, e0, e1))
            else:
                rc = fn(*a, s)
            if rc != 0:
                L.check(rc, fname)
        return out


class TuneCache(dict):

    def __init__(self):
        super().__init__()
        self._loaded, self._dirty, self.tuned, self.hits, self._synced_world = False, False, 0, 0, 1

    @staticmethod
    def library_id():
        import hashlib
        here = os.path.dirname(os.path.abspath(__file__))
        srcs = [os.path.join(here, "csrc", f) for f in ("vd_conv.hip", "vd_conv_igemm.h", "vd_conv_sk.hip", "vd_conv_par.hip",
                                                         "vd_conv_bf16.hip", "vd_conv_igemm_bf16.h", "vd_conv_bf16_sk.hip", "vd_conv_c32_bf16.hip",
                                                         "vd_wgrad_halo.hip", "vd_common.h")]
        h = hashlib.sha256()
        if all(os.path.exists(f) for f in srcs):
            for f in srcs:
                h.update(open(f, "rb").read())
        else:
            h.update(open(L.LIB_PATH, "rb").read())
        for sw in ("VD_WGRAD_RESERVE",):
            if os.environ.get(sw):
                h.update(("%s=%s" % (sw, os.environ[sw])).encode())
        return h.hexdigest()[:12]

    def path(self):
        p = os.environ.get("VD_TUNE_CACHE", "")
        if p.lower() in ("off", "0", "none"):
            return None
        if p:
            return p
        return os.path.join(os.path.dirname(os.path.abspath(__file__)), "tune", "gfx950_%s.json" % self.library_id())

    @staticmethod
    def _world():
        if not torch.distributed.is_available() or not torch.distributed.is_initialized():
            return 1
        return torch.distributed.get_world_size()

    @staticmethod
    def device_arch():
        if not torch.cuda.is_available():
            return None
        return str(torch.cuda.get_device_properties(torch.cuda.current_device()).gcnArchName).split(":")[0]

    def _read_file(self):
        import ast
        import json
        out = {}
        p = self.path()
        if p is None or not os.path.exists(p):
            return out
        try:
            doc = json.load(open(p))
            if doc.get("library") not in (None, self.library_id()):
                return out
            arch = self.device_arch()
            if arch is not None and doc.get("device") not in (None, arch):
                return out
            for k, v in doc.get("entries", {}).items():
                out[ast.literal_eval(k)] = tuple(v) if isinstance(v, list) else v
        except (OSError, ValueError, SyntaxError) as e:
            print("viddet_amd: ignoring tuning table %s (%s)" % (p, e), flush=True)
            return {}
        return out

    def load(self):
        self._loaded = True
        world = self._world()
        self._synced_world = world
        if world > 1 and os.environ.get("VD_TUNE_AGREE", "1") != "0":
            box = [self._read_file() if torch.distributed.get_rank() == 0 else None]
            torch.distributed.broadcast_object_list(box, src=0)
            dict.clear(self)
            entries = box[0]
        else:
            entries = self._read_file()
        for key, v in entries.items():
            if not dict.__contains__(self, key):
                dict.__setitem__(self, key, v)

    def __contains__(self, key):
        if not self._loaded or self._synced_world != self._world():
            self.load()
        hit = dict.__contains__(self, key)
        self.hits += int(hit)
        return hit

    def __setitem__(self, key, value):
# ... 1021 lines not shown
            else:
                kind = 'stem_weight' if n.stem else 'conv_weight'
                reg(n.name + ".0.weight", n.weight_shape(), kind, n, wv, gv, off=n.w_off)
                n.gamma = self.weights[n.gamma_off:n.gamma_off + n.cout]
                n.beta = self.weights[n.beta_off:n.beta_off + n.cout]
                n.ggamma = self.grads[n.gamma_off:n.gamma_off + n.cout]
                n.gbeta = self.grads[n.beta_off:n.beta_off + n.cout]
                c64 = round_up(n.cout, 64)
                n.rmean = self.running[n.stat_off:n.stat_off + n.cout]
                n.rvar = self.running[n.stat_off + c64:n.stat_off + c64 + n.cout]
                reg(n.name + ".1.gamma", (n.cout,), 'vector', n, n.gamma, n.ggamma, off=n.gamma_off)
                reg(n.name + ".1.beta", (n.cout,), 'vector', n, n.beta, n.gbeta, off=n.beta_off)
                reg(n.name + ".1.running_mean", (n.cout,), 'vector', n, n.rmean, None, trainable=False)
                reg(n.name + ".1.running_var", (n.cout,), 'vector', n, n.rvar, None, trainable=False)
                t = getattr(n, 'tdw', None)
                if t is not None:
                    t.w = self.weights[t.w_off:t.w_off + t.w_numel]
                    t.gw = self.grads[t.w_off:t.w_off + t.w_numel]
                    reg(t.pname, (t.C, 1, 3, 1, 1), 'vector', t, t.w, t.gw, off=t.w_off)
        self._params = P
        self._opt_ranges = None

    @property
    def classes(self):
        return self._classes

    def collect_params(self, select=None):
        return self._params if select is None else self._params.select(select)

    def hybridize(self, active=True):
        return None

    def set_nms(self, nms_thresh=0.45, nms_topk=400, post_nms=100):
        self.nms_thresh, self.nms_topk, self.post_nms = nms_thresh, nms_topk, post_nms
        self._programs = {k: v for k, v in self._programs.items() if k[0] not in ('infer', 'infer_bf16', 'stream', 'stream_bf16')}
        self._graph_cache.clear()

    def initialize(self, init='uniform', seed=233, obj_bias=0.0):
        g = torch.Generator(device='cpu').manual_seed(seed)
        for name, p in self._params.items():
            if name.endswith('weight'):
                if init == 'uniform':
                    v = (torch.rand(p.shape, generator=g) * 2 - 1) * 0.07
                else:
                    fan = int(np.prod(p.shape[1:]))
                    v = torch.randn(p.shape, generator=g) * math.sqrt(2.0 / fan)
                    if 'prediction' in name:
                        v *= 0.05
                p.set_data(v)
            elif name.endswith('gamma') or name.endswith('running_var'):
                v = torch.ones(p.shape)
                if init == 'he' and name.endswith('gamma') and '.body.1.1.' in name and name.startswith('stages'):
                    v *= 0.3
                p.set_data(v)
            elif name.endswith('bias'):
                v = torch.zeros(p.shape)
                if obj_bias != 0.0 and p.kind != 'gru_bias':
                    v.view(3, -1)[:, 4] = obj_bias
                p.set_data(v)
            else:
                p.set_data(torch.zeros(p.shape))
        self.momentum_buf.zero_()
        self.grads.zero_()

    def reset_class(self, classes, reuse_weights=None):
        if self._rnn_pos == 'out':
            raise NotImplementedError("reset_class on an rnn_pos='out' network: its predictions come from the GRU cells' gate "
                                      "blocks, and the reference's own YOLOOutputV3.reset_class doubts that path; retrain it")
        old_classes, old = self._classes, {k: p.data().cpu() for k, p in self._params.items()}
        old_attr = {k: (p.grad_req, p.wd_mult, p.lr_mult) for k, p in self._params.items()}
        old_npred = 5 + len(old_classes)
        if isinstance(reuse_weights, (dict, list)):
            if isinstance(reuse_weights, dict):
                m = {}
                for k, v in reuse_weights.items():
                    if isinstance(v, str):
                        if v not in old_classes:
                            raise ValueError("{} not found in old class names {}".format(v, old_classes))
                        v = old_classes.index(v)
                    elif v < 0 or v >= len(old_classes):
                        raise ValueError("Index {} out of bounds for old class names".format(v))
                    if isinstance(k, str):
                        if k not in classes:
                            raise ValueError("{} not found in new class names {}".format(k, classes))
                        k = list(classes).index(k)
                    elif k < 0 or k >= len(classes):
                        raise ValueError("Index {} out of bounds for new class names".format(k))
                    m[k] = v
                reuse_weights = m
            else:
                reuse_weights = {list(classes).index(x): old_classes.index(x) for x in reuse_weights
                                 if x in classes and x in old_classes}
        self._classes = list(classes)
        self._programs.clear()
        self._graph_cache.clear()
        self._build(len(self._classes))
        new_npred = 5 + len(self._classes)
        g = torch.Generator(device='cpu').manual_seed(233)
        for name, p in self._params.items():
            if "yolo_outputs" not in name:
                p.set_data(old[name])
                if p.span is not None:
                    p.grad_req, p.wd_mult, p.lr_mult = old_attr[name]
                continue
            new = (torch.rand(p.shape, generator=g) * 2 - 1) * 0.07 if name.endswith('weight') else torch.zeros(p.shape)
            if reuse_weights:
                od = old[name]
                for k, v in reuse_weights.items():
                    for a in range(3):
                        new[5 + k + a * new_npred] = od[5 + v + a * old_npred]
                        new[a * new_npred:a * new_npred + 5] = od[a * old_npred:a * old_npred + 5]
            p.set_data(new)

    def _grad_req_changed(self):
        self._programs = {k: v for k, v in self._programs.items() if k[0] != 'train'}
        self._opt_ranges = None

    def _node_trainable(self, n):
        P = self._params
        if getattr(n, 'gru', None) is not None:
            return P[n.pw].grad_req != 'null', P[n.pb].grad_req != 'null'
        if n.head:
            return P[n.name + ".weight"].grad_req != 'null', P[n.name + ".bias"].grad_req != 'null'
        return (P[n.name + ".0.weight"].grad_req != 'null',
                P[n.name + ".1.gamma"].grad_req != 'null' or P[n.name + ".1.beta"].grad_req != 'null')

    def _optimizer_ranges(self):
        if self._opt_ranges is None:
            ps = sorted((p for p in self._params.values() if p.span is not None and p.grad_req != 'null'),
                        key=lambda p: p.span[0])
            out = []
            for p in ps:
                lo, hi = p.span
                if out and out[-1][1] == lo and out[-1][2] == p.lr_mult and out[-1][3] == p.wd_mult and \
                        (lo != self.n_weight):
                    out[-1][1] = hi
                else:
                    out.append([lo, hi, p.lr_mult, p.wd_mult])
            self._opt_ranges = [tuple(r) for r in out]
        return self._opt_ranges

    def _params_changed(self):
        self._fold_dirty = True
        self._weights_version += 1
        self._wamax_dirty = True

    def _refresh_wamax(self):
        if self._wamax_dirty:
            L.check(L.load().vd_amax_segments(self.weights.data_ptr(), self._wamax_seg.data_ptr(), len(self.conv_nodes),
                                              self._wamax.data_ptr(), L.stream_ptr()), 'vd_amax_segments')
            self._wamax_dirty = False

    def _buffers(self, key, B, H, W, train, bf16=False):
        ck = ('buf', B, H, W, train) + (('bf16',) if bf16 else ())
        if ck in self._programs:
            return self._programs[ck]
        dev = self.device
        dt = torch.bfloat16 if bf16 else torch.float32
        zeroed = set(self.head_names) | {'d:' + h for h in self.head_names} if bf16 else set()
        bufs = {}
        for name, (c, div, ld, fr) in self.tensors.items():
            if name == 'in':
                bufs['in'] = torch.empty(B * fr, 3, H, W, device=dev)
            elif name in zeroed:
                bufs[name] = torch.zeros(B * fr, H // div, W // div, _bf16_pitch(ld), device=dev)
            else:
                bufs[name] = torch.empty(B * fr, H // div, W // div, ld, dtype=dt, device=dev)
        if self.noback:
            for nm, c_, d_ in ROUTE_TENSORS:
                bufs['in:' + nm] = torch.empty(B, c_, H // d_, W // d_, device=dev)
        for g in self.gru_nodes:
            h_, w_ = H // g.div, W // g.div
            for cname, i2h, h2h in g.cells:
                bufs[i2h.dst] = torch.empty(B * g.K, h_, w_, 3 * g.chp, device=dev)
                bufs[h2h.dst] = torch.empty(B * g.K if train else B, h_, w_, 3 * g.chp, device=dev)
                bufs[g.key(cname, 'h')] = torch.empty(B * g.K, h_, w_, g.chp, device=dev)
                if train:
                    bufs[g.key(cname, 'dh')] = torch.empty(B, h_, w_, g.chp, device=dev)
        if not bf16:
            names = [nm for nm in self.tensors if nm != 'in'] + (['dz:' + n.name for n in self.conv_nodes] if train else [])
            bufs['amax'] = torch.zeros(len(names) * L.AMAX_FLOATS, device=dev)
            for i, nm in enumerate(names):
                bufs['amax:' + nm] = bufs['amax'][i * L.AMAX_FLOATS:(i + 1) * L.AMAX_FLOATS]
        for n in self.conv_nodes:
            if getattr(n, 'tvalid', False):
                bufs['zf:' + n.dst] = torch.empty(B * n.fr, H // n.div_out, W // n.div_out, n.cout, device=dev)
                if train:
                    bufs['dzf:' + n.dst] = torch.empty_like(bufs['zf:' + n.dst])
                else:
                    bufs['zs:' + n.dst] = torch.empty_like(bufs[n.dst])
        if train:
            for n in self.nodes:
                if isinstance(n, PoolNode) and n.type == 0:
                    bufs['am:' + n.dst] = torch.empty(bufs[n.dst].shape, dtype=torch.uint8 if bf16 else torch.int32, device=dev)
            for n in self.conv_nodes:
                if n.bn:
                    bufs['z:' + n.dst] = torch.empty_like(bufs[n.dst])
            for name in self.tensors:
                if name != 'in':
                    bufs['d:' + name] = (torch.zeros_like if 'd:' + name in zeroed else torch.empty_like)(bufs[name], dtype=dt)
            mx = max(bufs[n.dst].numel() for n in self.conv_nodes)
            bufs['dz'] = torch.empty(mx, dtype=dt, device=dev)
            bufs['dz2'] = torch.empty(mx, dtype=dt, device=dev)
            bufs['tmp'] = torch.empty(mx, dtype=dt, device=dev)
        for nm, t in bufs.items():
            if torch.is_tensor(t) and t.dtype == dt and not nm.startswith('amax') and nm not in zeroed:
                t.normal_()
        self._programs[ck] = bufs
        return bufs

    def _grid(self, H, W):
        assert H == W, "square inputs only (the reference resizes to data_shape x data_shape)"
        assert H % 32 == 0, "input side must be a multiple of 32"
        return [H // 32, H // 16, H // 8]

    def _conv_desc(self, n, bufs, B, H, W, out, *, scale=None, shift=None, residual=None, leaky=False, amax_out=False):
        d = ConvDesc()
        x = bufs[n.src]
        Hi, Wi = H // n.div_in, W // n.div_in
        Ho, Wo = H // n.div_out, W // n.div_out
        d.in_, d.wp, d.out = x.data_ptr(), n.wp.data_ptr(), out.data_ptr()
        d.N, d.Hi, d.Wi, d.Ci = B * n.fr, Hi, Wi, n.ci_eff
        d.Hg, d.Wg, d.in_stride = Ho, Wo, n.stride
        ops._set_taps(d, n.taps())
        d.Kfr = n.fr if n.kd > 1 else 1
        d.Ho, d.Wo, d.Co = Ho, Wo, n.co_pad
        d.out_stride, d.out_oy, d.out_ox = 1, 0, 0
        d.ldo = d.ldr = n.co_pad
        flags = 0
        if scale is not None or shift is not None:
            flags |= EPI_AFFINE
            d.scale = scale.data_ptr() if scale is not None else None
            d.shift = shift.data_ptr() if shift is not None else None
        if leaky:
            flags |= EPI_LEAKY
        if residual is not None:
            flags |= EPI_RESIDUAL
            d.residual = residual.data_ptr()
        d.flags, d.slope = flags, LEAKY_SLOPE
        d.amax_in, d.amax_w = self._amax_or_none(bufs, n.src), n.wamax.data_ptr()
        self._set_streamk(d, 0)
        if amax_out:
            d.amax_out = bufs['amax:' + n.dst].data_ptr()
        return d

    def _amax_or_none(self, bufs, name):
        if name in self._range_exact:
            return None
        return bufs['amax:' + name].data_ptr()

    def check_operand_ranges(self, thresh=2.0 ** -16):
        bn = [n for n in self.conv_nodes if n.bn]
        if not bn:
            return {}
        if getattr(self, '_guard', None) is None:
            arr = (L.GuardItem * len(bn))()
            for i, n in enumerate(bn):
                arr[i].gamma, arr[i].beta, arr[i].scale, arr[i].C = n.gamma.data_ptr(), n.beta.data_ptr(), n.b_scale.data_ptr(), n.cout
            items = torch.frombuffer(bytearray(bytes(arr)), dtype=torch.uint8).to(self.device)
            self._guard = (items, torch.zeros(2 * len(bn), device=self.device), torch.zeros(2 * len(bn), dtype=torch.int32, device=self.device))
        items, ratios, flags = self._guard
        L.check(L.load().vd_range_guard(items.data_ptr(), len(bn), float(thresh), ratios.data_ptr(), flags.data_ptr(), L.stream_ptr()),
                'vd_range_guard')
        if torch.distributed.is_available() and torch.distributed.is_initialized() and \
                torch.distributed.get_world_size(self.process_group) > 1:
            torch.distributed.all_reduce(flags, op=torch.distributed.ReduceOp.MAX, group=self.process_group)
        fl, ra = flags.cpu().numpy(), ratios.cpu().numpy()
        new = {}
        for i, n in enumerate(bn):
            for k, name in ((0, n.tdw.dst if getattr(n, 'tdw', None) is not None else n.dst), (1, 'dz:' + n.name)):
                if fl[2 * i + k] and name not in self._range_exact:
                    new[name] = float(ra[2 * i + k])
        if new:
            self._range_exact.update(new)
            self._drop_plans()
        return new

    def _set_streamk(self, d, stream_idx):
        if not _streamk_on():
            return
        ws = self._sk_ws.get(stream_idx)
        if ws is None:
            ws = self._sk_ws[stream_idx] = ops.streamk_workspace(self.device)
        d.sk_ws, d.sk_ws_bytes = ws.data_ptr(), ws.numel()

    def _syncbn_exchange(self, t):
        def f():
            if getattr(self, '_syncbn_suppress', False):
                return
            torch.distributed.all_reduce(t, group=self.process_group)
            if getattr(self, '_dp_stats', None) is not None:
                self._dp_stats['syncbn_exchanges'] = self._dp_stats.get('syncbn_exchanges', 0) + 1
        return f

    def _add_sel_add_fwd(self, prog, n, bufs, B, bf16=False):
        am = lambda t: bufs['amax:' + t].data_ptr()
        if isinstance(n, SelNode):
            xs, o = bufs[n.src], bufs[n.dst]
            prog.add('vd_frame_slice', xs.data_ptr(), o.data_ptr(), B, n.K, n.k0, n.kc, xs[0].numel() // (2 if bf16 else 1), 0)
            if not bf16:
                prog.add('vd_amax_merge', am(n.src), None, am(n.dst))
        else:
            a, b_, o = bufs[n.a], bufs[n.b], bufs[n.dst]
            prog.add('vd_add_bf16' if bf16 else 'vd_add', a.data_ptr(), b_.data_ptr(), o.data_ptr(), o.numel())
            if not bf16:
                prog.add('vd_amax', o.data_ptr(), o.numel(), am(n.dst))

    def _gru_conv_desc(self, cn, x, out, N, H, W, sidx, amax_in=None):
        d = ConvDesc()
        Hc, Wc = H // cn.div_in, W // cn.div_in
        d.in_, d.wp, d.out = x.data_ptr(), cn.wp.data_ptr(), out.data_ptr()
        d.N, d.Hi, d.Wi, d.Ci = N, Hc, Wc, cn.cin
        d.Hg, d.Wg, d.in_stride = Hc, Wc, 1
        ops._set_taps(d, cn.taps())
        d.Kfr, d.Ho, d.Wo, d.Co = 1, Hc, Wc, cn.co_pad
        d.out_stride, d.out_oy, d.out_ox = 1, 0, 0
        d.ldo = d.ldr = cn.co_pad
        d.flags, d.slope, d.shift = EPI_AFFINE, LEAKY_SLOPE, cn.bias.data_ptr()
        d.amax_in, d.amax_w = amax_in, cn.wamax.data_ptr()
        self._set_streamk(d, sidx)
        return d

    @staticmethod
    def _gru_meta(cn, N, H, W, kind):
        px = N * (H // cn.div_in) * (W // cn.div_in)
        return dict(kind=kind, node=cn.name, k=cn.k, stride=1, flops=2.0 * cn.cin * cn.cout * cn.k * cn.k * px,
                    bytes=4.0 * (px * cn.cin + px * cn.cout + cn.cout * cn.cin * cn.k * cn.k))

    def _add_gru_fwd(self, prog, g, bufs, B, H, W, train, side=None):
        K, hw = g.K, (H // g.div) * (W // g.div)
        x = bufs[g.src]
        par = train and side is not None
        if par:
            e_x, e_r = torch.cuda.Event(), torch.cuda.Event()
            prog.add_py(ev_record(e_x))
            prog.add_py(ev_wait(e_x, side))
            prog.hold(e_x, e_r)
        for di, (cname, i2h, h2h) in reversed(list(enumerate(g.cells))):
            st = side if (par and di == 1) else None
            sidx = 4 if st is not None else 0
            I, Hb, hs = bufs[i2h.dst], bufs[h2h.dst], bufs[g.key(cname, 'h')]
            d = self._gru_conv_desc(i2h, x, I, B * K, H, W, sidx, self._amax_or_none(bufs, g.src))
            prog.hold(d)
            prog.add('vd_conv_igemm', C.byref(d), meta=self._gru_meta(i2h, B * K, H, W, 'fwd'), stream=st)
            for s_ in range(K):
                t = s_ if di == 0 else K - 1 - s_
                Hs = None
                if s_ > 0:
                    Hs = Hb[s_ * B:(s_ + 1) * B] if train else Hb
                    d = self._gru_conv_desc(h2h, hs[(s_ - 1) * B:s_ * B], Hs, B, H, W, sidx)
                    prog.hold(d)
                    prog.add('vd_conv_igemm', C.byref(d), meta=self._gru_meta(h2h, B, H, W, 'fwd'), stream=st)
                prog.add('vd_gru_gate_fwd', I.data_ptr(), Hs.data_ptr() if s_ > 0 else None, h2h.bias.data_ptr(),
                         hs[(s_ - 1) * B:].data_ptr() if s_ > 0 else None, hs[s_ * B:].data_ptr(), B, K, t, hw, g.chp,
                         meta=dict(kind='gru_gate_fwd', node=g.name, flops=14.0 * B * hw * g.chp,
                                   bytes=4.0 * B * hw * g.chp * (8 if s_ > 0 else 4)), stream=st)
            if st is not None:
                prog.add_py(ev_record(e_r, side))
        if par:
            prog.add_py(ev_wait(e_r))
        y = bufs[g.dst]
        prog.add('vd_gru_avg', bufs[g.key('l_cell', 'h')].data_ptr(), bufs[g.key('r_cell', 'h')].data_ptr(), y.data_ptr(), B, K,
                 hw * g.chp, bufs['amax:' + g.dst].data_ptr(),
                 meta=dict(kind='gru_avg', node=g.name, flops=2.0 * B * K * hw * g.chp, bytes=12.0 * B * K * hw * g.chp))

    def _add_tdw_fwd(self, prog, n, bufs, B, H, W):
        hw = (H // n.div) * (W // n.div)
        prog.add('vd_tdw_fwd', bufs[n.src].data_ptr(), n.w.data_ptr(), bufs[n.residual].data_ptr() if n.residual else None,
                 bufs[n.dst].data_ptr(), B, n.K, hw, n.C, bufs['amax:' + n.dst].data_ptr(),
                 meta=dict(kind='tdw_fwd', node=n.name, flops=6.0 * B * n.K * hw * n.C,
                           bytes=4.0 * B * n.K * hw * n.C * (3 if n.residual else 2)))

    def _add_input_stage(self, prog, bufs, B, H, W):
        prog.add('vd_fill', bufs['amax'].data_ptr(), 0.0, bufs['amax'].numel())
        if self.noback:
            for nm, c_, d_ in ROUTE_TENSORS:
                prog.add('vd_nchw_to_nhwc', bufs['in:' + nm].data_ptr(), bufs[nm].data_ptr(), B, c_, H // d_, W // d_)
                prog.add('vd_amax', bufs[nm].data_ptr(), bufs[nm].numel(), bufs['amax:' + nm].data_ptr())

    def _add_stem(self, prog, n, bufs, B, H, W, out, *, scale=None, shift=None, leaky=False, bf16=False, stats=None):
        flags = (EPI_AFFINE if scale is not None else 0) | (EPI_LEAKY if leaky else 0)
        prog.add('vd_stem_conv', bufs['in'].data_ptr(), n.wp.data_ptr(), out.data_ptr(), out.shape[-1], bufs['in'].shape[0], H, W,
                 scale.data_ptr() if scale is not None else None, shift.data_ptr() if shift is not None else None,
                 LEAKY_SLOPE, flags, 1 if bf16 else 0, stats, meta=self._flops(n, B, H, W, 'fwd'))

    def _stage_inputs(self, bufs, x):
        if self.noback:
            for (nm, _, _), t in zip(ROUTE_TENSORS, x):
                bufs['in:' + nm].copy_(t.reshape(bufs['in:' + nm].shape))
        elif x.dtype == torch.uint8 and self._dev_nv12 is not None:
            n_ = bufs['in'].shape[0]
            assert x.numel() == n_ * x.shape[-2] * x.shape[-1], "NV12 input must be (B[,K],H0*3/2,W0)"
            self._preprocess_u8(self._frames_to_device(x), bufs['in'], n_)
        elif x.dtype == torch.uint8:
            n_, h_, w_ = bufs['in'].shape[0], bufs['in'].shape[2], bufs['in'].shape[3]
            if self._dev_resize is not None:
                h_, w_ = x.shape[-3], x.shape[-2]
            assert x.shape[-1] == 3 and x.numel() == n_ * h_ * w_ * 3, "uint8 input must be (B[,K],H,W,3)"
            self._preprocess_u8(x.to(self.device).contiguous(), bufs['in'], n_)
        else:
            bufs['in'].copy_(x.reshape(bufs['in'].shape))

    def _preprocess_u8(self, xd, dst, n):
        if self._dev_nv12 is not None:
            return self._preprocess_nv12(xd, dst, n)
        h, w = dst.shape[2], dst.shape[3]
        h0, w0 = xd.shape[-3], xd.shape[-2]
        if self._dev_resize is None or (h0, w0) == (h, w):
            L.check(L.load().vd_preprocess_u8_nchw(xd.data_ptr(), dst.data_ptr(), n, h, w, L.stream_ptr()), 'vd_preprocess_u8_nchw')
            return
        t = self._resize_tables(h0, w0)
        if t['dev'] is None:
            t['dev'] = [torch.from_numpy(a).to(self.device) for a in t['host']]
        iy, wy, ix, wx = t['dev']
        L.check(L.load().vd_resize_u8_nchw(xd.data_ptr(), dst.data_ptr(), None, n, h0, w0, h, w, iy.data_ptr(), wy.data_ptr(),
                                           iy.shape[1], ix.data_ptr(), wx.data_ptr(), ix.shape[1], L.stream_ptr()),
                'vd_resize_u8_nchw')

    def _frames_to_device(self, x):
        x = x.to(self.device)
        return x if self._dev_nv12 is not None else x.contiguous()

    def _preprocess_nv12(self, xd, dst, n):
# ... 782 lines not shown
```

### viddet_amd/ops.py

```python
import ctypes as C

import torch

from . import lib as L
from .lib import (ConvDesc, WgradDesc, HeadDesc, EPI_AFFINE, EPI_LEAKY, EPI_RESIDUAL, MATH_SPLIT, MATH_BF16, MATH_F16X2,
                  MATH_NOHALO, AMAX_FLOATS, check, ptr)


def round_up(v, m):
    return (v + m - 1) // m * m


def _lib():
    return L.load()


def _s():
    return L.stream_ptr()


def fwd_taps(k, pad, kd=1, pad_d=0):
    taps = []
    for kz in range(kd):
        for ky in range(k):
# ... 102 lines not shown
    d.N, d.Hi, d.Wi, d.Ci, d.Hg, d.Wg, d.in_stride = N, Hi, Wi, Ci, Hg, Wg, in_stride
    _set_taps(d, taps)
    d.Kfr, d.Ho, d.Wo, d.Co = 1, Ho, Wo, Co
    d.out_stride, d.out_oy, d.out_ox, d.ldo, d.ldr = out_stride, out_oy, out_ox, ldo, ldr
    d.flags = (EPI_AFFINE if (scale is not None or shift is not None) else 0) | (EPI_LEAKY if leaky else 0) | \
              (EPI_RESIDUAL if residual is not None else 0) | (MATH_NOHALO if nohalo else 0)
    d.slope, d.stats_part = slope, ptr(stats_part)
    if streamk_ws is not None:
        d.flags |= L.CONV_STREAMK | (L.CONV_SPLITK if splitk else 0)
        d.sk_ws, d.sk_ws_bytes = ptr(streamk_ws), streamk_ws.numel() * streamk_ws.element_size()
    check(_lib().vd_conv_igemm_bf16(C.byref(d), 1 if out.dtype == torch.float32 else 0, _s()), "vd_conv_igemm_bf16")
    return d


def conv_bf16_mtiles(N, Hg, Wg, Ci, Co, tile=0):
    d = ConvDesc()
    d.N, d.Hg, d.Wg, d.Ci, d.Co, d.tile = N, Hg, Wg, Ci, Co, tile
    return _lib().vd_conv_igemm_bf16_mtiles(C.byref(d))


def pack_weight_bf16(wp32, wb, *, Co, Co_pad, Ci, Ci_pad, T):
    check(_lib().vd_pack_weight_bf16(ptr(wp32), ptr(wb), Co, Co_pad, Ci, Ci_pad, T, _s()), "vd_pack_weight_bf16")


def conv_wgrad(x, dout, dwp, ws, *, k, stride, pad, Co, kd=1, pad_d=0, kfr=1, splits=0, split=False, amax_in=None,
               amax_dout=None, in_scale=None, in_shift=None, in_slope=0.1):
    N, Hi, Wi, Ci = x.shape
    _, Ho, Wo, ldd = dout.shape
    d = WgradDesc()
    d.in_, d.dout, d.dwp = ptr(x), ptr(dout), ptr(dwp)
    d.N, d.Hi, d.Wi, d.Ci = N, Hi, Wi, Ci
    d.Hg, d.Wg, d.Co, d.ldd = Ho, Wo, Co, ldd
    d.in_stride = stride
    _set_taps(d, fwd_taps(k, pad, kd, pad_d))
    d.Kfr, d.splits = kfr, splits
    d.in_scale, d.in_shift, d.in_slope = ptr(in_scale), ptr(in_shift), in_slope
    if split in ('f16x2', 'f16x2nh', 'f16x2h'):
        d.flags = MATH_F16X2 | (L.WGRAD_HALO if split == 'f16x2h' else 0)
        amax_in = amax(x) if amax_in is None else amax_in
        amax_dout = amax(dout) if amax_dout is None else amax_dout
        d.amax_in, d.amax_dout = ptr(amax_in), ptr(amax_dout)
    else:
        d.flags = (MATH_BF16 if split == 'bf16' else MATH_SPLIT) if split else 0
    if x.dtype == torch.bfloat16:
        assert dout.dtype == torch.bfloat16 and dwp.dtype == torch.float32
        assert Ci % 8 == 0 and Co % 8 == 0 and ldd % 8 == 0 and x.data_ptr() % 16 == 0 and dout.data_ptr() % 16 == 0, \
            "bf16-stored operands: Ci, Co and the gradient pitch multiples of 8, 16-byte aligned tensors"
        d.flags = L.STORE_BF16 | MATH_BF16 | (L.WGRAD_HALO if split == 'halo' else 0)
    lib = _lib()
    need = lib.vd_conv_wgrad_ws_bytes(C.byref(d))
    if need > ws.numel() * ws.element_size():
        raise L.VidDetHipError("conv_wgrad: workspace %d < %d bytes" % (ws.numel() * ws.element_size(), need))
    check(lib.vd_conv_wgrad(C.byref(d), ptr(ws), ws.numel() * ws.element_size(), _s()), "vd_conv_wgrad")


def wgrad_ws_bytes(N, Hi, Wi, Ci, Ho, Wo, Co, k, stride, pad, kd=1, pad_d=0):
    d = WgradDesc()
    d.N, d.Hi, d.Wi, d.Ci, d.Hg, d.Wg, d.Co, d.ldd = N, Hi, Wi, Ci, Ho, Wo, Co, Co
    d.in_stride = stride
    _set_taps(d, fwd_taps(k, pad, kd, pad_d))
    d.Kfr, d.splits = 1, 0
    need = 0
    for fl in (0, MATH_SPLIT, MATH_F16X2 | L.WGRAD_HALO, L.STORE_BF16 | L.WGRAD_HALO):
        d.flags = fl
        d.amax_in = d.amax_dout = 1 if fl & MATH_F16X2 else None
        need = max(need, _lib().vd_conv_wgrad_ws_bytes(C.byref(d)))
    return need


def pack_weight_fwd(w_oihw, wp, Co_pad):
    Co, Ci = w_oihw.shape[0], w_oihw.shape[1]
    if w_oihw.dim() == 4:
        kd, kh, kw = 1, w_oihw.shape[2], w_oihw.shape[3]
    else:
        kd, kh, kw = w_oihw.shape[2:]
    check(_lib().vd_pack_weight_fwd(ptr(w_oihw), ptr(wp), Co, Co_pad, Ci, kd, kh, kw, _s()), "vd_pack_weight_fwd")


def pack_weight_dgrad(w, wp, *, Co, Co_pad, Ci, kd, kh, kw, tap_ids, src_packed):
    arr = (C.c_int32 * len(tap_ids))(*tap_ids)
    check(_lib().vd_pack_weight_dgrad(ptr(w), ptr(wp), Co, Co_pad, Ci, kd, kh, kw, arr, len(tap_ids),
                                      1 if src_packed else 0, _s()), "vd_pack_weight_dgrad")


PARITY4_TAPS = [(0, 0, 0), (0, 1, 0), (1, 0, 0), (1, 1, 0)]


def _parity4_mask():
    tap = lambda parity, off: (1 if off == 0 else -1) if parity == 0 else (2 if off == 0 else 0)
    m = 0
    for o in range(4):
        for c in range(4):
            if tap(c >> 1, o >> 1) >= 0 and tap(c & 1, o & 1) >= 0:
                m |= 1 << (4 * o + c)
    return m


PARITY4_MASK = _parity4_mask()


def pack_weight_dgrad_s2(wp_fwd, wp4, *, Co, Co_pad, Ci):
    m = C.c_int32(0)
    check(_lib().vd_pack_weight_dgrad_s2(ptr(wp_fwd), ptr(wp4), Co, Co_pad, Ci, C.byref(m), _s()), "vd_pack_weight_dgrad_s2")
    return int(m.value)


def conv_dgrad_s2_fused(dz, wp4, dx, *, Cin, par_mask, residual=None, tile=0, amax_in=None, amax_w=None, desc_out=None):
    N, Ho, Wo, Cout = dz.shape
    d = ConvDesc()
    d.tile = tile
    d.in_, d.wp, d.out, d.residual = ptr(dz), ptr(wp4), ptr(dx), ptr(residual)
    d.N, d.Hi, d.Wi, d.Ci, d.Hg, d.Wg, d.in_stride = N, Ho, Wo, Cout, Ho, Wo, 1
    _set_taps(d, PARITY4_TAPS)
    d.Kfr, d.Ho, d.Wo, d.Co = 1, 2 * Ho, 2 * Wo, 4 * Cin
    d.out_stride, d.out_oy, d.out_ox, d.ldo, d.ldr = 2, 0, 0, dx.shape[-1], dx.shape[-1]
    d.flags = MATH_F16X2 | L.CONV_PARITY4 | (EPI_RESIDUAL if residual is not None else 0)
    d.par_cin, d.par_mask, d.slope = Cin, par_mask, 0.1
    amax_in = amax(dz) if amax_in is None else amax_in
    amax_w = amax(wp4) if amax_w is None else amax_w
    d.amax_in, d.amax_w = ptr(amax_in), ptr(amax_w)
    if desc_out is not None:
        desc_out.append((d, amax_in, amax_w))
    check(_lib().vd_conv_igemm(C.byref(d), _s()), "vd_conv_igemm/parity4")


def unpack_weight(wp, w_oihw):
    Co, Ci = w_oihw.shape[0], w_oihw.shape[1]
    if w_oihw.dim() == 4:
        kd, kh, kw = 1, w_oihw.shape[2], w_oihw.shape[3]
    else:
        kd, kh, kw = w_oihw.shape[2:]
    check(_lib().vd_unpack_wgrad(ptr(wp), ptr(w_oihw), Co, Ci, kd, kh, kw, _s()), "vd_unpack_wgrad")


def stem_im2col(x, col, nchw):
    if nchw:
        N, _, H, W = x.shape
    else:
        N, H, W, _ = x.shape
    check(_lib().vd_stem_im2col(ptr(x), ptr(col), N, H, W, 1 if nchw else 0, _s()), "vd_stem_im2col")


def stem_conv(x_nchw, wp, out, *, scale=None, shift=None, leaky=False, slope=0.1, stats_part=None):
    N, _, H, W = x_nchw.shape
    flags = (EPI_AFFINE if scale is not None else 0) | (EPI_LEAKY if leaky else 0)
    check(_lib().vd_stem_conv(ptr(x_nchw), ptr(wp), ptr(out), out.shape[-1], N, H, W, ptr(scale), ptr(shift), slope, flags,
                              1 if out.dtype == torch.bfloat16 else 0, ptr(stats_part), _s()), "vd_stem_conv")


def stem_wgrad(x_nchw, dz, dwp, ws):
    N, _, H, W = x_nchw.shape
    fn = _lib().vd_stem_wgrad_bf16 if dz.dtype == torch.bfloat16 else _lib().vd_stem_wgrad
    check(fn(ptr(x_nchw), ptr(dz), dz.shape[-1], ptr(dwp), N, H, W, ptr(ws), ws.numel() * ws.element_size(), _s()), "vd_stem_wgrad")


def bn_stats(x2d_rows, C_, x, sums, ws):
    fn = _lib().vd_bn_stats_bf16 if x.dtype == torch.bfloat16 else _lib().vd_bn_stats
    check(fn(ptr(x), x2d_rows, C_, ptr(sums), ptr(ws), ws.numel() * ws.element_size(), _s()), "vd_bn_stats")


def bn_stats_ws_bytes(M, C_):
    return _lib().vd_bn_stats_ws_bytes(M, C_)


def bn_finalize(sums, count, C_, gamma, beta, eps, momentum, rmean, rvar, scale, shift, smean, sinv):
    check(_lib().vd_bn_finalize(ptr(sums), float(count), C_, ptr(gamma), ptr(beta), eps, momentum, ptr(rmean),
                                ptr(rvar), ptr(scale), ptr(shift), ptr(smean), ptr(sinv), _s()), "vd_bn_finalize")


def _nbytes(t):
    return 0 if t is None else t.numel() * t.element_size()


def bn_sum_partials_ws_bytes(nblk, C_):
    return int(_lib().vd_bn_sum_partials_ws_bytes(nblk, C_))


def bn_sum_partials(part, nblk, C_, sums, ws=None):
    check(_lib().vd_bn_sum_partials(ptr(part), nblk, C_, ptr(sums), ptr(ws), _nbytes(ws), _s()), "vd_bn_sum_partials")


def bn_sum_finalize(part, nblk, C_, sums, count, gamma, beta, eps, momentum, rmean, rvar, scale, shift, smean, sinv, ws=None):
    check(_lib().vd_bn_sum_finalize(ptr(part), nblk, C_, ptr(sums), float(count), ptr(gamma), ptr(beta), eps, momentum,
                                    ptr(rmean), ptr(rvar), ptr(scale), ptr(shift), ptr(smean), ptr(sinv), ptr(ws), _nbytes(ws),
                                    _s()), "vd_bn_sum_finalize")


def bn_sum_param_grads(part, nblk, C_, sums2, dgamma, dbeta, ws=None):
    check(_lib().vd_bn_sum_param_grads(ptr(part), nblk, C_, ptr(sums2), ptr(dgamma), ptr(dbeta), ptr(ws), _nbytes(ws), _s()),
          "vd_bn_sum_param_grads")


def bn_fold_eval(gamma, beta, rmean, rvar, eps, scale, shift):
    check(_lib().vd_bn_fold_eval(ptr(gamma), ptr(beta), ptr(rmean), ptr(rvar), eps, gamma.numel(), ptr(scale),
                                 ptr(shift), _s()), "vd_bn_fold_eval")


def bn_apply_leaky(x, scale, shift, residual, y, M, C_, slope=0.1, amax_out=None):
    if x.dtype == torch.bfloat16:
        check(_lib().vd_bn_apply_leaky_bf16(ptr(x), ptr(scale), ptr(shift), ptr(residual), ptr(y), M, C_, slope, _s()),
              "vd_bn_apply_leaky_bf16")
        return
    check(_lib().vd_bn_apply_leaky(ptr(x), ptr(scale), ptr(shift), ptr(residual), ptr(y), M, C_, slope, ptr(amax_out),
                                   _s()), "vd_bn_apply_leaky")


def bn_bwd_reduce(x, dy, scale, shift, smean, sinv, M, C_, sums2, ws, slope=0.1):
    if x.dtype == torch.bfloat16:
        check(_lib().vd_bn_bwd_reduce_bf16(ptr(x), ptr(dy), ptr(scale), ptr(shift), ptr(smean), ptr(sinv), M, C_, slope,
                                           ptr(sums2), ptr(ws), ws.numel() * ws.element_size(), _s()), "vd_bn_bwd_reduce_bf16")
        return
    check(_lib().vd_bn_bwd_reduce(ptr(x), ptr(dy), ptr(scale), ptr(shift), ptr(smean), ptr(sinv), M, C_, slope,
                                  ptr(sums2), ptr(ws), ws.numel() * ws.element_size(), _s()), "vd_bn_bwd_reduce")


def bn_param_grads(sums2, C_, dgamma, dbeta):
    check(_lib().vd_bn_param_grads(ptr(sums2), C_, ptr(dgamma), ptr(dbeta), _s()), "vd_bn_param_grads")


def bn_bwd_apply(x, dy, scale, shift, smean, sinv, sums2, count, M, C_, dx, slope=0.1, amax_out=None):
    if x.dtype == torch.bfloat16:
        check(_lib().vd_bn_bwd_apply_bf16(ptr(x), ptr(dy), ptr(scale), ptr(shift), ptr(smean), ptr(sinv), ptr(sums2),
                                          float(count), M, C_, slope, ptr(dx), _s()), "vd_bn_bwd_apply_bf16")
        return
    check(_lib().vd_bn_bwd_apply(ptr(x), ptr(dy), ptr(scale), ptr(shift), ptr(smean), ptr(sinv), ptr(sums2),
                                 float(count), M, C_, slope, ptr(dx), ptr(amax_out), _s()), "vd_bn_bwd_apply")


def amax(x, out=None):
    out = torch.empty(AMAX_FLOATS, device=x.device) if out is None else out
    check(_lib().vd_amax(ptr(x), x.numel(), ptr(out), _s()), "vd_amax")
    return out


def amax_value(slots):
    return float(slots.view(-1)[::L.AMAX_STRIDE][:L.AMAX_SLOTS].max())


def add(a, b, out):
    if out.dtype == torch.bfloat16:
        check(_lib().vd_add_bf16(ptr(a), ptr(b), ptr(out), out.numel(), _s()), "vd_add_bf16")
        return
    check(_lib().vd_add(ptr(a), ptr(b), ptr(out), out.numel(), _s()), "vd_add")


def fill(t, v):
    check(_lib().vd_fill(ptr(t), float(v), t.numel(), _s()), "vd_fill")


def upsample2x_concat(up, route, out):
    N, Ho, Wo, Cr = route.shape
    Cu = up.shape[3]
    if out.dtype == torch.bfloat16:
        Cu, Cr = Cu // 2, Cr // 2
    check(_lib().vd_upsample2x_concat(ptr(up), ptr(route), ptr(out), N, Ho, Wo, Cu, Cr, _s()), "vd_upsample2x_concat")


def upsample2x_concat_bwd(dout, dup, droute):
    N, Ho, Wo, Cr = droute.shape
    Cu = dup.shape[3]
    if dout.dtype == torch.bfloat16:
        check(_lib().vd_upsample2x_concat_bwd_bf16(ptr(dout), ptr(dup), ptr(droute), N, Ho, Wo, Cu, Cr, _s()),
              "vd_upsample2x_concat_bwd_bf16")
        return
    check(_lib().vd_upsample2x_concat_bwd(ptr(dout), ptr(dup), ptr(droute), N, Ho, Wo, Cu, Cr, _s()),
          "vd_upsample2x_concat_bwd")


def nchw_to_nhwc(x, out):
    N, Cc, H, W = x.shape
    check(_lib().vd_nchw_to_nhwc(ptr(x), ptr(out), N, Cc, H, W, _s()), "vd_nchw_to_nhwc")


def preprocess_u8(x_u8, out):
    check(_lib().vd_preprocess_u8_nhwc(ptr(x_u8), ptr(out), x_u8.numel() // 3, _s()), "vd_preprocess_u8_nhwc")


def augment_u8_nchw(raw, src_off, src_hw, color, idx_y, w_y, Ty, idx_x, w_x, Tx, fill, out, N, K, H, W):
    check(_lib().vd_augment_u8_nchw(ptr(raw), ptr(src_off), ptr(src_hw), ptr(color), ptr(idx_y), ptr(w_y), Ty, ptr(idx_x), ptr(w_x),
                                    Tx, ptr(fill), ptr(out), N, K, H, W, _s()), "vd_augment_u8_nchw")


def yolo_targets(gt, ids, idw, mix, N, M, C, H, W, obj, ctr, scl, wgt, cls):
    check(_lib().vd_yolo_targets(ptr(gt), ptr(ids), idw, ptr(mix), N, M, C, H, W, ptr(obj), ptr(ctr), ptr(scl), ptr(wgt),
                                 ptr(cls), _s()), "vd_yolo_targets")


def voc_match(det_ids, det_scores, det_boxes, gt, clip_hi, iou_thresh, rec_cls, rec_score, rec_hit, npos, ndiff=None):
    if det_boxes.dim() != 3 or det_boxes.shape[-1] != 4:
        raise ValueError("voc_match: det_boxes must be (B,N,4), got %r" % (tuple(det_boxes.shape),))
    B, N = int(det_boxes.shape[0]), int(det_boxes.shape[1])
    if gt.dim() != 3 or gt.shape[-1] not in (5, 6):
        raise ValueError("voc_match: gt must be (B,M,5|6) [x1, y1, x2, y2, id(, difficult)], got %r" % (tuple(gt.shape),))
    M, gt_w = int(gt.shape[1]), int(gt.shape[2])
    if N > L.VOC_MATCH_MAX_DET:
        raise ValueError("voc_match: N=%d detections per image, vd_voc_match takes at most %d" % (N, L.VOC_MATCH_MAX_DET))
    if M > L.VOC_MATCH_MAX_GT:
        raise ValueError("voc_match: M=%d label rows per image, vd_voc_match takes at most %d" % (M, L.VOC_MATCH_MAX_GT))
    if int(gt.shape[0]) != B:
        raise ValueError("voc_match: gt holds %d images, det_boxes %d" % (int(gt.shape[0]), B))
    for name, t, n, dt in (("det_ids", det_ids, B * N, torch.float32), ("det_scores", det_scores, B * N, torch.float32),
                           ("det_boxes", det_boxes, B * N * 4, torch.float32), ("gt", gt, B * M * gt_w, torch.float32),
                           ("rec_cls", rec_cls, B * N, torch.int32), ("rec_score", rec_score, B * N, torch.float32),
                           ("rec_hit", rec_hit, B * N, torch.int8), ("npos", npos, npos.numel(), torch.int32),
                           ("ndiff", ndiff, npos.numel(), torch.int32)):
        if t is None and name == "ndiff":
# ... 230 lines not shown
```

### viddet_amd/train_plan.py

```python
import ctypes as C
import math
import os

import torch

from . import lib as L
from . import ops
from .consts import ANCHORS, STRIDES, BN_EPS, BN_MOMENTUM, LEAKY_SLOPE
from .lib import ConvDesc, WgradDesc, EPI_AFFINE, EPI_RESIDUAL
from .model import (Program, Slot, ConvNode, UpcatNode, PoolNode, CorrNode, GruNode, SelNode, AddNode, TdwNode,
                    autotune_desc, autotune_program, autotune_wgrad, autotune_wgrad_bf16, consumers_of, ev_record, ev_wait,
                    fp32_math, grad_required, _bf16_pitch, _TUNE_CACHE)
from .ops import dgrad_plans


class Switches:

    def __init__(self, env=os.environ):
        self.side_prio = int(env.get('VD_SIDE_PRIO', '0'))
        self.fuse_bwd_bf16 = env.get('VD_FUSE_BWD_BF16', '0') == '1'
        self.s2_fused = env.get('VD_S2_FUSED', '1') == '1'
        self.s2_fused_max_cin = int(env.get('VD_S2_FUSED_MAX_CIN', '64'))
        self.s2_chunk_mb = float(env.get('VD_S2_CHUNK_MB', '0'))
        self.parity_streams = env.get('VD_PARITY_STREAMS', '1') == '1'
        self.fuse_bwd_s2 = env.get('VD_FUSE_BWD_S2', '1') == '1'
        self.autotune = env.get('VD_AUTOTUNE', '1') != '0'


class TrainPlan:

    FWD = {UpcatNode: 'fwd_upcat', PoolNode: 'fwd_pool', CorrNode: 'fwd_corr', SelNode: 'fwd_sel_add', AddNode: 'fwd_sel_add',
           GruNode: 'fwd_gru', TdwNode: 'fwd_tdw', ConvNode: 'fwd_conv'}
    BWD = {UpcatNode: 'bwd_upcat', PoolNode: 'bwd_pool', CorrNode: 'bwd_corr', SelNode: 'bwd_sel', AddNode: 'bwd_add',
           GruNode: 'bwd_gru', TdwNode: 'bwd_tdw', ConvNode: 'bwd_conv'}

    def __init__(self, net, B, H, W):
        self.net, self.B, self.H, self.W = net, B, H, W
        self.sw = Switches()
        bf16 = self.bf16 = getattr(net, 'storage', 'fp32') == 'bf16'
        self.sfx, self.esz = ('_bf16', 2) if bf16 else ('', 4)
        self.dt = torch.bfloat16 if bf16 else torch.float32
        self.cw = 2 if bf16 else 1
        self.bufs = net._buffers('train', B, H, W, True, bf16=bf16)
        self.dev, self.lib = net.device, L.load()
        self.mtiles = self.lib.vd_conv_igemm_bf16_mtiles if bf16 else self.lib.vd_conv_igemm_mtiles
        self.size_workspaces()
        self.side = torch.cuda.Stream(priority=self.sw.side_prio) if net.overlap_wgrad else None
        self.seg = None

    def amx(self, t):
        return self.bufs['amax:' + t].data_ptr()

    def amx_arg(self, t):
        return () if self.bf16 else (None if t is None else self.amx(t),)

    def size_workspaces(self):
        net, bf16, lib, B, H, W = self.net, self.bf16, self.lib, self.B, self.H, self.W
        ws_bytes = 1 << 20
        for n in net.conv_nodes:
            Hi, Wi = H // n.div_in, W // n.div_in
            Ho, Wo = H // n.div_out, W // n.div_out
            if n.stem:
                ws_bytes = max(ws_bytes, int(lib.vd_stem_wgrad_ws_bytes(B * n.fr, Hi, Wi)))
            elif bf16:
                wd_ = WgradDesc()
                wd_.N, wd_.Hi, wd_.Wi, wd_.Ci, wd_.Hg, wd_.Wg, wd_.Co, wd_.ldd = B * n.fr, Hi, Wi, n.cin, Ho, Wo, n.co_pad, n.co_pad
                ops._set_taps(wd_, n.taps())
                for fl_ in (0, L.WGRAD_HALO):
                    wd_.in_stride, wd_.Kfr, wd_.flags = n.stride, (n.fr if n.kd > 1 else 1), L.STORE_BF16 | L.MATH_BF16 | fl_
                    ws_bytes = max(ws_bytes, int(lib.vd_conv_wgrad_ws_bytes(C.byref(wd_))))
            else:
                ws_bytes = max(ws_bytes, ops.wgrad_ws_bytes(B * n.fr, Hi, Wi, n.cin, Ho, Wo, n.co_pad, n.k, n.stride,
                                                            n.pad, n.kd, n.pad_d))
            ws_bytes = max(ws_bytes, ops.bn_stats_ws_bytes(B * n.fr * Ho * Wo, _bf16_pitch(n.co_pad) if bf16 else n.co_pad))
        for n in net.tdw_nodes:
            ws_bytes = max(ws_bytes, int(lib.vd_tdw_bwd_ws_bytes(B, n.K, (H // n.div) * (W // n.div), n.C)))
        self.ws_bytes = ws_bytes
        self.ws = torch.empty(ws_bytes, dtype=torch.uint8, device=self.dev)
        self.world = 1
        if torch.distributed.is_available() and torch.distributed.is_initialized():
            self.world = torch.distributed.get_world_size(net.process_group)
            if (self.world > 1 and net.syncbn_scope and net.bucketed_allreduce and net._bucket_group is None
                    and net.process_group is None):
                net._bucket_group = torch.distributed.new_group()
        smax = 16
        for n in net.conv_nodes:
            if n.bn:
                smax = max(smax, ((B * n.fr * (H // n.div_out) * (W // n.div_out) + 63) // 64 + 8 + 256) * 2 * n.cout)
        self.stats_ws = torch.empty(smax, device=self.dev)
        self.wb_arena = torch.empty(net.n_weight, dtype=self.dt, device=self.dev) if bf16 else None

    def stats_rows_fit(self, rows, cout):
        assert rows * 2 * cout <= self.stats_ws.numel(), "stats workspace too small"

    def tune(self, d, of32=0):
        if self.bf16:
            self.net._tune_bf16_desc(d, of32)
        else:
            autotune_desc(d)

    def add_conv(self, d, of32=0, **kw):
        if self.bf16:
            self.seg.add('vd_conv_igemm_bf16', C.byref(d), of32, **kw)
        else:
            self.seg.add('vd_conv_igemm', C.byref(d), **kw)

    def fwd_desc(self, n, out):
        net, bufs, B, H, W = self.net, self.bufs, self.B, self.H, self.W
        if not self.bf16:
            d = net._conv_desc(n, bufs, B, H, W, out, shift=n.bias if n.head else None)
            self.seg.hold(d)
            return d
        wb = self.wb_arena[n.w_off:n.w_off + n.w_numel]
        assert n.w_numel == n.co_pad * n.T * n.cin and n.w_off % 8 == 0
        Ho, Wo = H // n.div_out, W // n.div_out
        d = ConvDesc()
        net._set_streamk(d, 0)
        d.in_, d.wp, d.out = bufs[n.src].data_ptr(), wb.data_ptr(), out.data_ptr()
        d.N, d.Hi, d.Wi, d.Ci, d.Hg, d.Wg, d.in_stride = B * n.fr, H // n.div_in, W // n.div_in, n.cin, Ho, Wo, n.stride
        ops._set_taps(d, n.taps())
        d.Kfr, d.Ho, d.Wo, d.Co = (n.fr if n.kd > 1 else 1), Ho, Wo, n.co_pad
        d.out_stride, d.out_oy, d.out_ox, d.slope = 1, 0, 0, LEAKY_SLOPE
        d.ldo = d.ldr = out.shape[-1]
        if n.head:
            d.flags, d.shift = EPI_AFFINE, n.bias.data_ptr()
        self.seg.hold(d, wb)
        return d

    def build(self):
        net = self.net
        self.seg = Program()
        if not self.bf16:
            net._add_input_stage(self.seg, self.bufs, self.B, self.H, self.W)
        for n in net.nodes:
            getattr(self, self.FWD[type(n)])(n)
        slots, losses = self.add_loss()
        fwd = [self.seg]
        self.seg = Program()
        self.begin_backward()
        for n in reversed(net.nodes):
            getattr(self, self.BWD[type(n)])(n)
        if self.side is not None and self.last_side is not None:
            self.seg.add_py(ev_wait(self.last_side))
        self.seg.hold(self.ws_w, self.side, self.stats_ws)
        bwd = [self.seg]
        for sg in fwd + bwd:
            if isinstance(sg, Program):
                autotune_program(sg)
        _TUNE_CACHE.save()
        return dict(fwd=fwd, bwd=bwd, bufs=self.bufs, slots=slots, losses=losses, dgrad_packs=self.dgrad_packs, ws=self.ws,
                    wb_arena=self.wb_arena, storage='bf16' if self.bf16 else 'fp32')

    def fwd_upcat(self, n):
        seg, bufs = self.seg, self.bufs
        o = bufs[n.dst]
        seg.add('vd_upsample2x_concat', bufs[n.up].data_ptr(), bufs[n.route].data_ptr(), o.data_ptr(), self.B * n.fr,
                o.shape[1], o.shape[2], n.cu // self.cw, n.cr // self.cw)
        if not self.bf16:
            seg.add('vd_amax_merge', self.amx(n.up), self.amx(n.route), self.amx(n.dst))

    def fwd_pool(self, n):
        seg, bufs, B, cw = self.seg, self.bufs, self.B, self.cw
        o, xs = bufs[n.dst], bufs[n.src]
        if n.type == 2:
            assert xs.shape[3] % (4 * cw) == 0, "cat join: C = %d must keep 16-byte units" % xs.shape[3]
            seg.add('vd_temporal_cat', xs.data_ptr(), o.data_ptr(), B, n.K, xs.shape[1] * xs.shape[2], xs.shape[3] // cw, 0)
        else:
            am = bufs['am:' + n.dst].data_ptr() if n.type == 0 else None
            seg.add('vd_temporal_pool_train_bf16' if self.bf16 else 'vd_temporal_pool', xs.data_ptr(), o.data_ptr(), am, B, n.K,
                    o[0].numel(), n.type)
        if not self.bf16:
            seg.add('vd_amax_merge', self.amx(n.src), None, self.amx(n.dst))

    def fwd_corr(self, n):
        bufs = self.bufs
        xs = bufs[n.src]
        assert xs.shape[3] == n.C and bufs[n.dst].shape[3] == n.ldy
        self.seg.add('vd_corr_fwd' + self.sfx, xs.data_ptr(), bufs[n.dst].data_ptr(), self.B, n.K, xs.shape[1], xs.shape[2], n.C,
                     n.d, n.ldy, meta=self.net._corr_meta(n, self.B, xs, 'fwd', self.esz))

    def fwd_sel_add(self, n):
        if self.bf16:
            raise NotImplementedError("bf16-storage training: node type %s" % type(n).__name__)
        self.net._add_sel_add_fwd(self.seg, n, self.bufs, self.B)

    def fwd_gru(self, n):
        self.net._add_gru_fwd(self.seg, n, self.bufs, self.B, self.H, self.W, True, self.side)

    def fwd_tdw(self, n):
        self.net._add_tdw_fwd(self.seg, n, self.bufs, self.B, self.H, self.W)

    def fwd_conv(self, n):
        net, seg, bufs, B, H, W = self.net, self.seg, self.bufs, self.B, self.H, self.W
        Ho, Wo = H // n.div_out, W // n.div_out
        tvalid = getattr(n, 'tvalid', False)
        M = B * (n.fr - 2 if tvalid else n.fr) * Ho * Wo
        meta = net._flops(n, B, H, W, 'fwd', self.esz)
        if n.head:
            d = self.fwd_desc(n, bufs[n.dst])
            if self.bf16:
                self.tune(d, 1)
            self.add_conv(d, 1, meta=meta)
            return
        z = bufs['z:' + n.dst]
        ws, ws_bytes, stats_ws = self.ws, self.ws_bytes, self.stats_ws
        table_rows = None
        if n.stem:
            table_rows = self.lib.vd_stem_conv_blocks(B * n.fr, H, W)
            self.stats_rows_fit(table_rows, n.cout)
            net._add_stem(seg, n, bufs, B, H, W, z, bf16=self.bf16, stats=stats_ws.data_ptr())
        elif tvalid:
            zf = bufs['zf:' + n.dst]
            self.add_conv(self.fwd_desc(n, zf), meta=meta)
            seg.add('vd_frame_slice', zf.data_ptr(), z.data_ptr(), B, n.fr, 1, n.fr - 2, zf[0].numel(), 0)
            seg.add('vd_bn_stats', z.data_ptr(), M, n.cout, n.sums.data_ptr(), ws.data_ptr(), ws_bytes)
        elif self.bf16 or net.fuse_bn_stats:
            d = self.fwd_desc(n, z)
            d.stats_part = stats_ws.data_ptr()
            self.tune(d)
            table_rows = self.mtiles(C.byref(d))
            self.stats_rows_fit(table_rows, n.cout)
            self.add_conv(d, meta=meta)
        else:
            self.add_conv(self.fwd_desc(n, z), meta=meta)
            seg.add('vd_bn_stats', z.data_ptr(), M, n.cout, n.sums.data_ptr(), ws.data_ptr(), ws_bytes)
        count = float(M)
        fin = (n.gamma.data_ptr(), n.beta.data_ptr(), BN_EPS, BN_MOMENTUM, n.rmean.data_ptr(), n.rvar.data_ptr(),
               n.b_scale.data_ptr(), n.b_shift.data_ptr(), n.b_mean.data_ptr(), n.b_invstd.data_ptr())
        if table_rows is not None and not net._syncbn(n):
            seg.add('vd_bn_sum_finalize', stats_ws.data_ptr(), table_rows, n.cout, n.sums.data_ptr(), count, *fin,
                    ws.data_ptr(), ws_bytes)
        else:
            if table_rows is not None:
                seg.add('vd_bn_sum_partials', stats_ws.data_ptr(), table_rows, n.cout, n.sums.data_ptr(), ws.data_ptr(),
                        ws_bytes)
            if net._syncbn(n):
                seg.add_coll(net._syncbn_exchange(n.sums))
                count = float(M * self.world)
            seg.add('vd_bn_finalize', n.sums.data_ptr(), count, n.cout, *fin)
        res = bufs[n.residual].data_ptr() if n.residual else None
        seg.add('vd_bn_apply_leaky' + self.sfx, z.data_ptr(), n.b_scale.data_ptr(), n.b_shift.data_ptr(), res,
                bufs[n.dst].data_ptr(), M, n.cout, LEAKY_SLOPE, *self.amx_arg(n.dst),
                meta=dict(node=n.name, bytes=float(self.esz) * M * n.cout * (3 if n.residual else 2),
                          single_conv_consumer=not self.bf16 and n.dst in net.single_conv_consumer_tensors()))

    def add_loss(self):
        net, seg, bufs, bf16 = self.net, self.seg, self.bufs, self.bf16
        frames = self.B * net._head_frames
        grids = net._grid(self.H, self.W)
        hd = ops.make_head_desc([bufs[h] for h in net.head_names], grids, bufs[net.head_names[0]].shape[-1],
                                STRIDES[::-1], ANCHORS[::-1], frames, net.num_class)
        slots = dict(gt=Slot(), M=Slot(), obj=Slot(), ctr=Slot(), scl=Slot(), wgt=Slot(), cls=Slot(), smooth=Slot())
        losses = torch.zeros(frames, 4, device=self.dev)
        dh = (C.c_void_p * 3)(*[bufs['d:' + h].data_ptr() for h in net.head_names])
        head_node = {m.dst: m for m in net.conv_nodes if m.head}
        dha = None if (bf16 or not head_node) else \
            (C.c_void_p * 3)(*[self.amx('dz:' + head_node[h].name) for h in net.head_names])
        lws = torch.empty(max(16, ops.yolo_loss_ws_bytes(hd)), dtype=torch.uint8, device=self.dev)
        seg.hold(hd, dh, dha, lws)
        seg.add('vd_yolo_loss_fwd_bwd' + self.sfx, C.byref(hd), slots['gt'], slots['M'], slots['obj'], slots['ctr'], slots['scl'],
                slots['wgt'], slots['cls'], float(net._ignore_iou_thresh), slots['smooth'], losses.data_ptr(),
                C.byref(dh), None, *([] if bf16 else [C.byref(dha) if dha is not None else None]), lws.data_ptr(), lws.numel())
        return slots, losses

    def begin_backward(self):
        net, bufs = self.net, self.bufs
        self.ws_w = torch.empty(self.ws_bytes, dtype=torch.uint8, device=self.dev) if self.side is not None else self.ws
        self.dz_bufs = [bufs['dz'], bufs['dz2']]
        self.dz_free = [None, None]
        self.n_dz = 0
        self.last_side = None
        self.bucket_hi, self.bucket_acc = net.n_wconv, 0
        self.written = set(net.head_names)
        self.dgrad_packs = []
        self.alias = {}
        self.producers = {m.dst: m for m in net.conv_nodes if m.bn}
        self.consumers = consumers_of(net.nodes)
        self.fused_bwd = set()
        self.tgrad = grad_required(net.nodes, self.trainable, lambda t: t in net.input_tensors)
        wtrain = [m for m in net.conv_nodes if net._node_trainable(m)[0]]
        self.first_wtrain = wtrain[0] if wtrain else None

    def trainable(self, m):
        if isinstance(m, TdwNode):
            return self.net._params[m.pname].grad_req != 'null'
        return any(self.net._node_trainable(m))

    def copy_grad(self, src, dst):
        c = src.shape[-1]
        self.seg.add('vd_bn_apply_leaky' + self.sfx, src.data_ptr(), self.net._ones(c).data_ptr(), self.net._zeros(c).data_ptr(),
                     None, dst.data_ptr(), src.numel() // c, c, 1.0, *self.amx_arg(None))

    def materialize(self, name):
        if name in self.alias:
            self.copy_grad(self.alias.pop(name), self.bufs['d:' + name])

    def grad_into(self, name, can_alias=False):
        if name in self.written:
            if not can_alias:
                self.materialize(name)
            return self.bufs['d:' + name], True
        self.written.add(name)
        return self.bufs['d:' + name], False

    def add_grad(self, dsrc, acc, launch):
        target = self.bufs['tmp'][:dsrc.numel()] if acc else dsrc
        launch(target.data_ptr())
        if acc:
            self.seg.add('vd_add' + self.sfx, dsrc.data_ptr(), target.data_ptr(), dsrc.data_ptr(), dsrc.numel())

    def incoming(self, n):
        assert n.dst in self.written, n.name
        self.materialize(n.dst)
        return self.bufs['d:' + n.dst]

    def skip_grad(self, n, dy):
        if not (n.residual and self.tgrad[n.residual]):
            return
        dres, acc = self.grad_into(n.residual)
        if acc:
            self.seg.add('vd_add' + self.sfx, dres.data_ptr(), dy.data_ptr(), dres.data_ptr(), dy.numel())
        else:
            self.alias[n.residual] = dy
            if not self.net.alias_skip_grad:
                self.materialize(n.residual)

    def side_launch(self, *wargs, meta):
        seg, side = self.seg, self.side
        if side is None:
            seg.add(*wargs, self.ws.data_ptr(), self.ws_bytes, meta=meta)
            return None
        e_ready, e_done = torch.cuda.Event(), torch.cuda.Event()
        seg.add_py(ev_record(e_ready))
        seg.add_py(ev_wait(e_ready, side))
        seg.add(*wargs, self.ws_w.data_ptr(), self.ws_bytes, meta=meta, stream=side)
        seg.add_py(ev_record(e_done, side))
        seg.hold(e_ready, e_done)
        self.last_side = e_done
        return e_done

    def close_bucket(self, cn, last):
        net = self.net
        self.bucket_acc += cn.w_numel
        if net.bucketed_allreduce and (self.bucket_acc >= net.bucket_elems or last):
            lo, hi = cn.w_off, self.bucket_hi
            self.seg.add_py(net._bucket_launcher(lo, hi, self.side))
            self.bucket_hi, self.bucket_acc = lo, 0

    def dgrad_desc(self, cn, src, Hd, Wd, Kd, N, wpk, plan, dst, res):
        d = ConvDesc()
        d.in_, d.wp, d.out = src, wpk.data_ptr(), dst
        d.N, d.Hi, d.Wi, d.Ci = N, Hd, Wd, Kd
        d.Hg, d.Wg, d.in_stride = plan['Hg'], plan['Wg'], 1
        ops._set_taps(d, plan['taps'])
        d.Kfr, d.Ho, d.Wo, d.Co = 1, self.H // cn.div_in, self.W // cn.div_in, cn.cin
        d.out_stride, d.out_oy, d.out_ox = 1, 0, 0
        d.ldo = d.ldr = cn.cin
        d.flags, d.slope = (EPI_RESIDUAL if res is not None else 0), LEAKY_SLOPE
        if res is not None:
            d.residual = res
        self.seg.hold(d, wpk)
        return d

    def fuse_bn_bwd(self, d, m, z_off, part_off):
        d.bs_z = self.bufs['z:' + m.dst].data_ptr() + z_off
        d.bs_scale, d.bs_shift = m.b_scale.data_ptr(), m.b_shift.data_ptr()
        d.bs_mean, d.bs_invstd = m.b_mean.data_ptr(), m.b_invstd.data_ptr()
        d.bs_part, d.bs_slope = self.stats_ws.data_ptr() + part_off, LEAKY_SLOPE

    def fused_param_grads(self, m, rows):
        self.seg.add('vd_bn_sum_param_grads', self.stats_ws.data_ptr(), rows, m.cout, m.sums2.data_ptr(),
                     m.ggamma.data_ptr(), m.gbeta.data_ptr(), self.ws.data_ptr(), self.ws_bytes)
        self.fused_bwd.add(m.name)

    def bwd_tdw(self, n):
        if not self.tgrad[n.dst]:
            return
        B = self.B
        dy = self.incoming(n)
        self.skip_grad(n, dy)
        t_train = self.trainable(n)
        dxp = None
        if self.tgrad[n.src]:
            dsrc, acc = self.grad_into(n.src)
            assert not acc, n.name
            dxp = dsrc.data_ptr()
        if dxp is not None or t_train:
            hw = (self.H // n.div) * (self.W // n.div)
            self.seg.add('vd_tdw_bwd', dy.data_ptr(), self.bufs[n.src].data_ptr(), n.w.data_ptr(), dxp,
                         n.gw.data_ptr() if t_train else None, B, n.K, hw, n.C, self.ws.data_ptr(), self.ws_bytes,
                         meta=dict(kind='tdw_bwd', node=n.name, flops=(12.0 if t_train else 6.0) * B * n.K * hw * n.C,
                                   bytes=4.0 * B * n.K * hw * n.C * (1 + (dxp is not None) + t_train)))

    def bwd_upcat(self, n):
        tgrad, seg = self.tgrad, self.seg
        if not tgrad[n.dst]:
            return
        dout = self.bufs['d:' + n.dst]
        dup_p = None
        if tgrad[n.up]:
            dup, acc_u = self.grad_into(n.up)
            assert not acc_u
            dup_p = dup.data_ptr()
        launch = lambda p: seg.add('vd_upsample2x_concat_bwd' + self.sfx, dout.data_ptr(), dup_p, p, self.B * n.fr,
                                   dout.shape[1], dout.shape[2], n.cu, n.cr)
        if tgrad[n.route]:
            self.add_grad(*self.grad_into(n.route), launch)
        elif dup_p:
            launch(None)

    def bwd_sel(self, n):
        if not self.tgrad[n.src]:
            return
        dout = self.incoming(n)
        dsrc, acc = self.grad_into(n.src)
        self.add_grad(dsrc, acc, lambda p: self.seg.add('vd_frame_slice', dout.data_ptr(), p, self.B, n.K, n.k0, n.kc,
                                                        dsrc[0].numel(), 1))

    def bwd_add(self, n):
        if not self.tgrad[n.dst]:
            return
        dout = self.incoming(n)
        for t_ in (n.a, n.b):
            if not self.tgrad[t_]:
                continue
            dsrc, acc = self.grad_into(t_)
            if acc:
                self.seg.add('vd_add', dsrc.data_ptr(), dout.data_ptr(), dsrc.data_ptr(), dsrc.numel())
            else:
                self.copy_grad(dout, dsrc)

    def bwd_pool(self, n):
        if not self.tgrad[n.src]:
            return
        seg, B = self.seg, self.B
        dout = self.bufs['d:' + n.dst]
        assert n.dst in self.written, n.name
        dsrc, acc = self.grad_into(n.src)
        am = self.bufs['am:' + n.dst].data_ptr() if n.type == 0 else None
        if n.type == 2:
            launch = lambda p: seg.add('vd_temporal_cat', dout.data_ptr(), p, B, n.K, dsrc.shape[1] * dsrc.shape[2],
                                       dsrc.shape[3] // self.cw, 1)
        else:
            launch = lambda p: seg.add('vd_temporal_pool_bwd' + self.sfx, dout.data_ptr(), am, p, B, n.K, dout[0].numel(), n.type)
        self.add_grad(dsrc, acc, launch)

    def bwd_corr(self, n):
        if not self.tgrad[n.src]:
            return
        dout, xs = self.incoming(n), self.bufs[n.src]
        dsrc, acc = self.grad_into(n.src)
        self.add_grad(dsrc, acc, lambda p: self.seg.add(
            'vd_corr_bwd' + self.sfx, dout.data_ptr(), xs.data_ptr(), p, self.B, n.K, xs.shape[1], xs.shape[2], n.C, n.d, n.ldy,
            meta=self.net._corr_meta(n, self.B, xs, 'bwd', self.esz)))

    def gru_dgrad(self, cn, din, nfr, dout, acc, sidx, st, packs):
        Hc, Wc = self.H // cn.div_in, self.W // cn.div_in
        if cn not in packs:
            plan = dgrad_plans(cn.k, cn.pad, 1, Hc, Wc)[0]
            wpk = torch.empty(cn.cin * len(plan['taps']) * cn.co_pad, device=self.dev)
            self.dgrad_packs.append((cn, plan, wpk))
            packs[cn] = (plan, wpk)
        plan, wpk = packs[cn]
        d = self.dgrad_desc(cn, din.data_ptr(), Hc, Wc, cn.co_pad, nfr, wpk, plan, dout.data_ptr(),
                            dout.data_ptr() if acc else None)
        d.out_oy, d.out_ox = plan['py'], plan['px']
        d.amax_in, d.amax_w = None, cn.wamax.data_ptr()
        self.net._set_streamk(d, sidx)
        self.seg.add('vd_conv_igemm', C.byref(d), meta=self.net._gru_meta(cn, nfr, self.H, self.W, 'dgrad'), stream=st)

    def gru_wgrad(self, cn, xin, dout, nfr, amax_in):
        Hc, Wc = self.H // cn.div_in, self.W // cn.div_in
        wd_ = WgradDesc()
        wd_.in_, wd_.dout, wd_.dwp = xin.data_ptr(), dout.data_ptr(), cn.gwp.data_ptr()
        wd_.N, wd_.Hi, wd_.Wi, wd_.Ci = nfr, Hc, Wc, cn.cin
        wd_.Hg, wd_.Wg, wd_.Co, wd_.ldd = Hc, Wc, cn.co_pad, cn.co_pad
        wd_.in_stride = 1
        ops._set_taps(wd_, cn.taps())
        wd_.Kfr, wd_.splits = 1, 0
        wd_.amax_in, wd_.amax_dout = amax_in, None
        autotune_wgrad(wd_, self.ws.data_ptr(), self.ws_bytes)
        self.seg.hold(wd_)
        self.side_launch('vd_conv_wgrad', C.byref(wd_), meta=self.net._gru_meta(cn, nfr, self.H, self.W, 'wgrad'))
        self.close_bucket(cn, cn is self.first_wtrain)

    def bwd_gru(self, g):
        if not self.tgrad[g.dst]:
            return
        net, seg, bufs, B, side = self.net, self.seg, self.bufs, self.B, self.side
        dy = self.incoming(g)
        K, hw = g.K, (self.H // g.div) * (self.W // g.div)
        packs = {}
        if side is not None:
            e_dy, e_r = torch.cuda.Event(), torch.cuda.Event()
            seg.add_py(ev_record(e_dy))
            seg.add_py(ev_wait(e_dy, side))
            seg.hold(e_dy, e_r)
        for di, (cname, i2h, h2h) in reversed(list(enumerate(g.cells))):
            st = side if (side is not None and di == 1) else None
            sidx = 4 if st is not None else 0
            I, Hb, hs, dh = bufs[i2h.dst], bufs[h2h.dst], bufs[g.key(cname, 'h')], bufs[g.key(cname, 'dh')]
            for s_ in reversed(range(K)):
                t = s_ if di == 0 else K - 1 - s_
                Hs = Hb[s_ * B:(s_ + 1) * B]
                seg.add('vd_gru_gate_bwd', I.data_ptr(), Hs.data_ptr(), 1 if s_ > 0 else 0, h2h.bias.data_ptr(),
                        hs[(s_ - 1) * B:].data_ptr() if s_ > 0 else None, dy.data_ptr(), 0.5, dh.data_ptr(),
                        1 if s_ < K - 1 else 0, B, K, t, hw, g.chp,
                        meta=dict(kind='gru_gate_bwd', node=g.name, flops=30.0 * B * hw * g.chp,
                                  bytes=4.0 * B * hw * g.chp * (16 if s_ > 0 else 11)), stream=st)
                if s_ > 0:
                    self.gru_dgrad(h2h, Hs, B, dh, True, sidx, st, packs)
            if st is not None:
                seg.add_py(ev_record(e_r, side))
        if side is not None:
            seg.add_py(ev_wait(e_r))
        if self.tgrad[g.src]:
            dsrc, acc = self.grad_into(g.src)
            for di, (cname, i2h, h2h) in enumerate(g.cells):
                self.gru_dgrad(i2h, bufs[i2h.dst], B * K, dsrc, acc or di > 0, 0, None, packs)
        for cname, i2h, h2h in g.cells:
            for cn in (i2h, h2h):
                if net._node_trainable(cn)[1]:
                    dz_ = bufs[cn.dst]
                    seg.add('vd_bn_stats', dz_.data_ptr(), B * K * hw, cn.co_pad, cn.sums.data_ptr(), self.ws.data_ptr(),
                            self.ws_bytes)
                    seg.add('vd_bn_param_grads', cn.sums.data_ptr(), cn.co_pad, bufs['tmp'].data_ptr(), cn.gbias.data_ptr())
        for cname, i2h, h2h in reversed(g.cells):
            hs, Hb = bufs[g.key(cname, 'h')], bufs[h2h.dst]
            if net._node_trainable(h2h)[0]:
                self.gru_wgrad(h2h, hs, Hb[B:], B * (K - 1), None)
            if net._node_trainable(i2h)[0]:
                self.gru_wgrad(i2h, bufs[g.src], bufs[i2h.dst], B * K, net._amax_or_none(bufs, g.src))

    def bwd_conv(self, n):
        if not self.tgrad[n.dst]:
            return
        net = self.net
        w_train, v_train = net._node_trainable(n)
        dy = self.incoming(n)
        if n.head:
            dz, slot = self.head_bias_grad(n, dy), None
        else:
            self.skip_grad(n, dy)
            dz, slot = self.bn_backward(n, dy)
        if w_train:
            self.conv_wgrad(n, dz, slot)
        if n.stem or n.src in net.input_tensors or not self.tgrad[n.src]:
            return
        self.conv_dgrad(n, dz)

    def out_rows(self, n):
        frames = n.fr - 2 if getattr(n, 'tvalid', False) else n.fr
        return self.B * frames * (self.H // n.div_out) * (self.W // n.div_out)

    def head_bias_grad(self, n, dz):
        sums = n.sums
        if self.bf16:
            if getattr(n, 'sums_b', None) is None or n.sums_b.numel() != 2 * dz.shape[-1]:
                n.sums_b = torch.zeros(2 * dz.shape[-1], dtype=torch.float64, device=self.dev)
            sums = n.sums_b
        self.seg.add('vd_bn_stats' + self.sfx, dz.data_ptr(), self.out_rows(n), dz.shape[-1], sums.data_ptr(),
                     self.ws.data_ptr(), self.ws_bytes)
        self.seg.add('vd_bn_param_grads', sums.data_ptr(), n.co_pad, self.bufs['tmp'].data_ptr(), n.gbias.data_ptr())
        return dz

    def bn_backward(self, n, dy):
        seg, bufs, sfx, M = self.seg, self.bufs, self.sfx, self.out_rows(n)
        z = bufs['z:' + n.dst]
        slot = self.n_dz % 2
        self.n_dz += 1
        dz = self.dz_bufs[slot][:M * n.cout].view(-1, self.H // n.div_out, self.W // n.div_out, n.cout)
        bn = (n.b_scale.data_ptr(), n.b_shift.data_ptr(), n.b_mean.data_ptr(), n.b_invstd.data_ptr())
        if n.name not in self.fused_bwd:
            seg.add('vd_bn_bwd_reduce' + sfx, z.data_ptr(), dy.data_ptr(), *bn, M, n.cout, LEAKY_SLOPE, n.sums2.data_ptr(),
                    self.ws.data_ptr(), self.ws_bytes)
            seg.add('vd_bn_param_grads', n.sums2.data_ptr(), n.cout, n.ggamma.data_ptr(), n.gbeta.data_ptr())
        count = float(M)
        if self.net._syncbn(n):
            seg.add_coll(self.net._syncbn_exchange(n.sums2))
            count = float(M * self.world)
        if self.side is not None and self.dz_free[slot] is not None:
            seg.add_py(ev_wait(self.dz_free[slot]))
        seg.add('vd_bn_bwd_apply' + sfx, z.data_ptr(), dy.data_ptr(), *bn, n.sums2.data_ptr(), count, M, n.cout, LEAKY_SLOPE,
                dz.data_ptr(), *self.amx_arg('dz:' + n.name))
        if getattr(n, 'tvalid', False):
            dzf = bufs['dzf:' + n.dst]
            seg.add('vd_frame_slice', dz.data_ptr(), dzf.data_ptr(), self.B, n.fr, 1, n.fr - 2, dzf[0].numel(), 1)
            dz = dzf
        return dz, slot

    def conv_wgrad(self, n, dz, slot):
        net, bufs, B, H, W = self.net, self.bufs, self.B, self.H, self.W
        Hi, Wi = H // n.div_in, W // n.div_in
        if n.stem:
            wargs = ('vd_stem_wgrad' + self.sfx, bufs['in'].data_ptr(), dz.data_ptr(), n.co_pad, n.gwp.data_ptr(),
                     B * n.fr, Hi, Wi)
        else:
            wd_ = WgradDesc()
            wd_.in_, wd_.dout, wd_.dwp = bufs[n.src].data_ptr(), dz.data_ptr(), n.gwp.data_ptr()
            wd_.N, wd_.Hi, wd_.Wi, wd_.Ci = B * n.fr, Hi, Wi, n.ci_eff
            wd_.Hg, wd_.Wg, wd_.Co, wd_.ldd = H // n.div_out, W // n.div_out, n.co_pad, dz.shape[-1]
            wd_.in_stride = n.stride
            ops._set_taps(wd_, n.taps())
            wd_.Kfr, wd_.splits = (n.fr if n.kd > 1 else 1), 0
            if self.bf16:
                wd_.flags = L.STORE_BF16 | L.MATH_BF16
                autotune_wgrad_bf16(wd_, self.ws.data_ptr(), self.ws_bytes)
            else:
                wd_.amax_in, wd_.amax_dout = net._amax_or_none(bufs, n.src), net._amax_or_none(bufs, 'dz:' + n.name)
                autotune_wgrad(wd_, self.ws.data_ptr(), self.ws_bytes)
            self.seg.hold(wd_)
            wargs = ('vd_conv_wgrad', C.byref(wd_))
        e_done = self.side_launch(*wargs, meta=net._flops(n, B, H, W, 'wgrad', self.esz))
        if e_done is not None and not n.head:
            self.dz_free[slot] = e_done
        self.close_bucket(n, n is self.first_wtrain or n.stem)

    def conv_dgrad(self, n, dz):
        net, H, W = self.net, self.H, self.W
        dsrc, acc = self.grad_into(n.src, can_alias=True)
        res_src = self.alias.pop(n.src) if n.src in self.alias else dsrc
        res = res_src if acc else None
        plans = dgrad_plans(n.k, n.pad, n.stride, H // n.div_in, W // n.div_in, n.kd, n.pad_d)
        pm = self.producers.get(n.src)
        fuse_m = pm if (pm is not None and self.consumers[n.src][0] is n and
                        (self.sw.fuse_bwd_bf16 if self.bf16 else
                         net.fuse_bn_bwd and (len(plans) == 1 or (n.kd == 1 and self.sw.fuse_bwd_s2)) and pm.fr == n.fr)) else None
        if self.fused_s2(n, plans):
            self.dgrad_parity4(n, dz, dsrc, res, fuse_m)
        else:
            self.dgrad_parity_loop(n, dz, dsrc, res, fuse_m, plans)

    def fused_s2(self, n, plans):
        Hi, Wi = self.H // n.div_in, self.W // n.div_in
        return (not self.bf16 and len(plans) == 4 and n.k == 3 and n.stride == 2 and n.pad == 1 and n.kd == 1 and
                Hi % 2 == 0 and Wi % 2 == 0 and self.sw.s2_fused and n.cin % 32 == 0 and
                n.cin <= self.sw.s2_fused_max_cin and
                self.net._amax_or_none(self.bufs, 'dz:' + n.name) is not None and
                (fp32_math() == 'split2' or (fp32_math() == 'auto' and self.sw.autotune)))

    def dgrad_parity4(self, n, dz, dsrc, res, fuse_m):
        net, seg, B, H, W = self.net, self.seg, self.B, self.H, self.W
        Ho, Wo = H // n.div_out, W // n.div_out
        wp4 = torch.empty(16 * n.cin * n.co_pad, device=self.dev)
        self.dgrad_packs.append((n, dict(fused_s2=True), wp4))
        d = self.dgrad_desc(n, dz.data_ptr(), Ho, Wo, n.co_pad, B * n.fr, wp4, dict(Hg=Ho, Wg=Wo, taps=ops.PARITY4_TAPS),
                            dsrc.data_ptr(), None if res is None else res.data_ptr())
        d.Co, d.out_stride = 4 * n.cin, 2
        d.par_cin, d.par_mask = n.cin, ops.PARITY4_MASK
        d.flags |= L.MATH_F16X2 | L.CONV_PARITY4
        d.amax_in, d.amax_w = net._amax_or_none(self.bufs, 'dz:' + n.name), n.wamax.data_ptr()
        if fuse_m is not None:
            self.fuse_bn_bwd(d, fuse_m, 0, 0)
        autotune_desc(d)
        if fuse_m is not None:
            mt = self.lib.vd_conv_igemm_mtiles(C.byref(d))
            self.stats_rows_fit(mt, fuse_m.cout)
            seg.add('vd_fill', self.stats_ws.data_ptr(), 0.0, mt * 2 * fuse_m.cout)
        seg.add('vd_conv_igemm', C.byref(d), meta=dict(
            kind='dgrad', node=n.name, k=n.k, stride=n.stride, fused_s2=True,
            flops=2.0 * n.cin * n.cout * 9 * Ho * Wo * B * n.fr, bytes=net._flops(n, B, H, W, 'dgrad')['bytes']))
        if fuse_m is not None:
            self.fused_param_grads(fuse_m, mt)

    def frame_chunks(self, n, plans, NF):
        nchunks = 1
        chunk_mb = self.sw.s2_chunk_mb
        if not self.bf16 and len(plans) == 4 and n.kd == 1 and chunk_mb > 0:
            dz_mb = 4.0 * NF * (self.H // n.div_out) * (self.W // n.div_out) * n.co_pad / 1e6
            nchunks = max(1, min(NF, int(math.ceil(dz_mb / chunk_mb))))
        fchunk = (NF + nchunks - 1) // nchunks
        return fchunk, (NF + fchunk - 1) // fchunk

    def fork_parity(self):
        net, seg = self.net, self.seg
        if getattr(net, '_par_streams', None) is None:
            net._par_streams = [torch.cuda.Stream() for _ in range(3)]
        e_fork = torch.cuda.Event()
        seg.add_py(ev_record(e_fork))
        for st in net._par_streams:
            seg.add_py(ev_wait(e_fork, st))
        return net._par_streams

    def dgrad_parity_loop(self, n, dz, dsrc, res, fuse_m, plans):
        net, seg, bf16, esz, B, H, W = self.net, self.seg, self.bf16, self.esz, self.B, self.H, self.W
        Hi, Wi = H // n.div_in, W // n.div_in
        Ho, Wo = H // n.div_out, W // n.div_out
        NF = B * n.fr
        fchunk, nchunks = self.frame_chunks(n, plans, NF)
        kp = dz.shape[-1]
        wpks = []
        for plan in plans:
            assert plan['taps'], "a parity class without taps would leave its gradient unwritten"
            wpk = torch.empty(n.cin * len(plan['taps']) * kp, dtype=self.dt, device=self.dev)
            self.dgrad_packs.append((n, plan, wpk))
            wpks.append(wpk)
        in_img, out_img = Ho * Wo * kp * esz, Hi * Wi * n.cin * esz
        nplans = n.stride * n.stride
        bs_rows = 0
        for ch in range(nchunks):
            f0 = ch * fchunk
            fn_ = min(NF, f0 + fchunk) - f0
            par = None
            if not bf16 and self.sw.parity_streams and len(plans) == 4 and net.overlap_wgrad:
                par = self.fork_parity()
            for pi, plan in enumerate(plans):
                d = self.dgrad_desc(n, dz.data_ptr() + f0 * in_img, Ho, Wo, kp, fn_, wpks[pi], plan,
                                    dsrc.data_ptr() + f0 * out_img, None if res is None else res.data_ptr() + f0 * out_img)
                d.Kfr = n.fr if n.kd > 1 else 1
                d.out_stride, d.out_oy, d.out_ox = n.stride, plan['py'], plan['px']
                if not bf16:
                    d.amax_in, d.amax_w = net._amax_or_none(self.bufs, 'dz:' + n.name), n.wamax.data_ptr()
                net._set_streamk(d, pi if (par is not None) else 0)
                if fuse_m is not None:
                    self.fuse_bn_bwd(d, fuse_m, f0 * out_img, bs_rows * 2 * fuse_m.cout * 4)
                if bf16 or fuse_m is not None:
                    self.tune(d)
                if fuse_m is not None:
                    bs_rows += self.mtiles(C.byref(d))
                    self.stats_rows_fit(bs_rows, fuse_m.cout)
                self.add_conv(d, meta=dict(
                    kind='dgrad', node=n.name, k=n.k, stride=n.stride,
                    flops=2.0 * n.cin * n.cout * len(plan['taps']) * plan['Hg'] * plan['Wg'] * fn_,
                    bytes=net._flops(n, B, H, W, 'dgrad', esz)['bytes'] / nplans * fn_ / NF),
                    stream=(par[pi - 1] if (par is not None and pi > 0) else None))
            if par is not None:
                for st in par:
                    e_join = torch.cuda.Event()
                    seg.add_py(ev_record(e_join, st))
                    seg.add_py(ev_wait(e_join))
        if fuse_m is not None:
            self.fused_param_grads(fuse_m, bs_rows)
```

Measured before the change: 1044 frames/s.

## Fuse stem BN backward apply into stem weight-gradient kernel

For the stem convolution with batchnorm, the BN-backward apply (computing dz from z, dy and the reduced sums) is folded into the stem wgrad kernel, so dz is no longer written to and re-read from global memory. The dz scratch buffers are sized without the stem, which is the largest activation, cutting memory. A vectorized variant stages the computed dz through a per-wave LDS patch for the bf16 path. This adds an extra dy read inside the wgrad kernel and more register/LDS use. The stem dz amax range tracking is skipped.

```diff
diff --git a/include/viddet_hip.h b/include/viddet_hip.h
--- a/include/viddet_hip.h
+++ b/include/viddet_hip.h
@@ -126,6 +126,9 @@
 int64_t vd_stem_wgrad_ws_bytes(int N, int H, int W);
 int vd_stem_wgrad(const float* x_nchw, const float* dz, int ldd, float* dwp, int N, int H, int W, void* ws,
                   int64_t ws_bytes, void* stream);
+int vd_stem_wgrad_bn(const float* x_nchw, const float* z, int ldz, const float* dy, int ldy, const float* scale,
+                     const float* shift, const float* save_mean, const float* save_invstd, const double* sums2, double count,
+                     float slope, float* dwp, int N, int H, int W, void* ws, int64_t ws_bytes, void* stream);
 int vd_stem_im2col(const float* in, float* col, int N, int H, int W, int nchw, void* stream);
 
 int vd_pack_weight_fwd(const float* w_oihw, float* wp, int Co, int Co_pad, int Ci,
@@ -267,6 +270,9 @@
 int vd_corr_bwd_bf16(const void* dy, const void* x, void* dx, int B, int K, int H, int W, int C, int d, int ldy, void* stream);
 int vd_stem_wgrad_bf16(const float* x_nchw, const void* dz, int ldd, float* dwp, int N, int H, int W, void* ws, int64_t ws_bytes,
                        void* stream);
+int vd_stem_wgrad_bn_bf16(const float* x_nchw, const void* z, int ldz, const void* dy, int ldy, const float* scale,
+                          const float* shift, const float* save_mean, const float* save_invstd, const double* sums2, double count,
+                          float slope, float* dwp, int N, int H, int W, void* ws, int64_t ws_bytes, void* stream);
 int vd_yolo_loss_fwd_bwd_bf16(const vd_head_desc* h, const float* gt, int M, const float* obj_t, const float* center_t,
                               const float* scale_t, const float* weight_t, const float* class_t, float ignore_thresh,
                               int label_smooth, float* losses, void* const dhead[3], float* box_out, void* ws, int64_t ws_bytes,
diff --git a/viddet_amd/csrc/vd_bn.hip b/viddet_amd/csrc/vd_bn.hip
--- a/viddet_amd/csrc/vd_bn.hip
+++ b/viddet_amd/csrc/vd_bn.hip
@@ -1,4 +1,5 @@
 #include "vd_common.h"
+#include "vd_bn_math.h"
 #include <stdlib.h>
 
 namespace {
@@ -346,12 +347,7 @@
         const f32x4 d = vd_ld4(dy, i);
         f32x4 o;
 #pragma unroll
-        for (int e = 0; e < 4; ++e) {
-            const float u = v[e] * sc[e] + sh[e];
-            const float g = u > 0.f ? d[e] : d[e] * slope;
-            const float xh = (v[e] - mu[e]) * is[e];
-            o[e] = sc[e] * (g - mg[e] - xh * mgx[e]);
-        }
+        for (int e = 0; e < 4; ++e) o[e] = vd_bn_bwd_dz(v[e], d[e], sc[e], sh[e], mu[e], is[e], mg[e], mgx[e], slope);
         vd_st4(dx, i, o);
         amx = fmaxf(amx, fmaxf(fmaxf(fabsf(o[0]), fabsf(o[1])), fmaxf(fabsf(o[2]), fabsf(o[3]))));
     }
@@ -467,12 +463,8 @@
         if (!ok[j]) continue;
         VEC o;
 #pragma unroll
-        for (int e = 0; e < V; ++e) {
-            const float u = v[j][e] * k.sc[e] + k.sh[e];
-            const float g = u > 0.f ? d[j][e] : d[j][e] * slope;
-            const float xh = (v[j][e] - k.mu[e]) * k.is[e];
-            o[e] = k.sc[e] * (g - k.mg[e] - xh * k.mgx[e]);
-        }
+        for (int e = 0; e < V; ++e)
+            o[e] = vd_bn_bwd_dz(v[j][e], d[j][e], k.sc[e], k.sh[e], k.mu[e], k.is[e], k.mg[e], k.mgx[e], slope);
         bn_io<V, false>::st(dx, i + j * stride, o);
         amx = bn_vec_amax<V>(amx, o);
     }
diff --git a/viddet_amd/csrc/vd_bn_math.h b/viddet_amd/csrc/vd_bn_math.h
--- /dev/null
+++ b/viddet_amd/csrc/vd_bn_math.h
@@ -0,0 +1,10 @@
+#pragma once
+#include <hip/hip_runtime.h>
+
+__device__ __forceinline__ float vd_bn_bwd_dz(float z, float dy, float sc, float sh, float mu, float is, float mg, float mgx,
+                                              float slope) {
+    const float u = z * sc + sh;
+    const float g = u > 0.f ? dy : dy * slope;
+    const float xh = (z - mu) * is;
+    return sc * (g - mg - xh * mgx);
+}
diff --git a/viddet_amd/csrc/vd_stem.hip b/viddet_amd/csrc/vd_stem.hip
--- a/viddet_amd/csrc/vd_stem.hip
+++ b/viddet_amd/csrc/vd_stem.hip
@@ -1,4 +1,5 @@
 #include "vd_common.h"
+#include "vd_bn_math.h"
 #include <stdlib.h>
 
 namespace {
@@ -159,8 +160,38 @@
 }
 
 template <typename T>
+struct stem_bn_args {
+    const T* dy;
+    int ldy;
+    const float *scale, *shift, *mean, *invstd;
+    const double* sums2;
+    double count;
+    float slope;
+};
+
+struct stem_bn_lane {
+    float sc, sh, mu, is, mg, mgx, slope;
+    template <typename T> __device__ __forceinline__ void load(const stem_bn_args<T>& bn, int co) {
+        const float inv_count = (float)(1.0 / bn.count);
+        sc = bn.scale[co];
+        sh = bn.shift[co];
+        mu = bn.mean[co];
+        is = bn.invstd[co];
+        mg = (float)bn.sums2[co] * inv_count;
+        mgx = (float)bn.sums2[SC + co] * inv_count;
+        slope = bn.slope;
+    }
+    template <typename T> __device__ __forceinline__ float dz(float z, float dy) const {
+        const float v = vd_bn_bwd_dz(z, dy, sc, sh, mu, is, mg, mgx, slope);
+        if constexpr (sizeof(T) == 2) return (float)(__bf16)v;
+        else return v;
+    }
+};
+
+template <typename T, bool BN>
 __global__ __launch_bounds__(256) void k_stem_wgrad(const float* __restrict__ x, const T* __restrict__ dz, int ldd,
-                                                    float* __restrict__ part, int N, int H, int W, int64_t px_per_wave) {
+                                                    const stem_bn_args<T> bn, float* __restrict__ part, int N, int H, int W,
+                                                    int64_t px_per_wave) {
     const int lane = threadIdx.x & 63, wave = threadIdx.x >> 6;
     const int64_t HW = (int64_t)H * W, P = (int64_t)N * HW;
     const int64_t gw = (int64_t)blockIdx.x * 4 + wave;
@@ -183,13 +214,16 @@
         xx = r - y * W;
     }
     constexpr int UNR = 8;
+    stem_bn_lane kc;
+    if constexpr (BN) kc.load(bn, k);
     for (; p - par < p_end; p += 2 * UNR) {
-        float a[UNR], b[UNR];
+        float a[UNR], b[UNR], g[UNR];
 #pragma unroll
         for (int u = 0; u < UNR; ++u) {
             const int64_t pu = p + 2 * u;
             const bool in_run = pu < p_end;
             a[u] = in_run ? (float)dz[pu * ldd + k] : 0.f;
+            if constexpr (BN) g[u] = in_run ? (float)bn.dy[pu * bn.ldy + k] : 0.f;
             const int iy = y + dy, ix = xx + dx;
             const bool ok = in_run && k_ok && (unsigned)iy < (unsigned)H && (unsigned)ix < (unsigned)W;
             b[u] = ok ? x[((int64_t)n * 3 + c) * HW + (int64_t)iy * W + ix] : 0.f;
@@ -197,6 +231,10 @@
             while (xx >= W) { xx -= W; ++y; }
             if (y >= H) { y -= H; ++n; }
         }
+        if constexpr (BN) {
+#pragma unroll
+            for (int u = 0; u < UNR; ++u) a[u] = p + 2 * u < p_end ? kc.dz<T>(a[u], g[u]) : 0.f;
+        }
 #pragma unroll
         for (int u = 0; u < UNR; ++u) acc = __builtin_amdgcn_mfma_f32_32x32x2f32(a[u], b[u], acc, 0, 0, 0);
     }
@@ -209,10 +247,19 @@
 }
 
 constexpr int SROWS = 4;
-template <typename T>
+constexpr int SPATCH = 16 * SC;
+
+__device__ __forceinline__ void stem_wave_sync() {
+    __builtin_amdgcn_fence(__ATOMIC_RELEASE, "wavefront");
+    __builtin_amdgcn_wave_barrier();
+    __builtin_amdgcn_fence(__ATOMIC_ACQUIRE, "wavefront");
+}
+
+template <typename T, bool BN, bool VEC = false>
 __global__ __launch_bounds__(256) void k_stem_wgrad_rows(const float* __restrict__ x, const T* __restrict__ dz, int ldd,
-                                                         float* __restrict__ part, int N, int H, int W, int P) {
-    extern __shared__ float win[];
+                                                         const stem_bn_args<T> bn, float* __restrict__ part, int N, int H,
+                                                         int W, int P) {
+    extern __shared__ __attribute__((aligned(16))) float win[];
     const int tid = threadIdx.x, lane = tid & 63, wave = tid >> 6;
     const int groups = (H + SROWS - 1) / SROWS;
     const int n = blockIdx.x / groups, y0 = (blockIdx.x % groups) * SROWS;
@@ -236,13 +283,73 @@
         const float* b0 = win + (c * (SROWS + 2) + wave + tap / 3) * P + (tap % 3) + par;
         const T* a0 = dz + ((int64_t)n * HW + (int64_t)y * W + par) * ldd + k;
         constexpr int UNR = 8;
+        stem_bn_lane kc;
+        const T* g0 = nullptr;
+        if constexpr (BN && !VEC) {
+            kc.load(bn, k);
+            g0 = bn.dy + ((int64_t)n * HW + (int64_t)y * W + par) * bn.ldy + k;
+        }
+        if constexpr (BN && VEC) {
+            constexpr int VC = 16 / (int)sizeof(T);
+            constexpr int LPP = SC / VC, PPL = 64 / LPP;
+            constexpr int NL = 2 * UNR / PPL;
+            typedef typename vd_select<sizeof(T) == 2, vd_bf16x8, f32x4>::type vec_t;
+            const int tile_floats = 4 * SC * 32, win_floats = 3 * (SROWS + 2) * P;
+            T* patch = reinterpret_cast<T*>(win + (win_floats > tile_floats ? win_floats : tile_floats)) + wave * SPATCH;
+            const int vp = lane / LPP, vc = (lane % LPP) * VC;
+            stem_bn_lane kv[VC];
+#pragma unroll
+            for (int e = 0; e < VC; ++e) kv[e].load(bn, vc + e);
+            const T* zr = dz + ((int64_t)n * HW + (int64_t)y * W) * ldd + vc;
+            const T* gr = bn.dy + ((int64_t)n * HW + (int64_t)y * W) * bn.ldy + vc;
+            vec_t zv[NL], gv[NL];
+            auto load = [&](int x0) {
+#pragma unroll
+                for (int j = 0; j < NL; ++j) {
+                    const int px = x0 + j * PPL + vp;
+                    if (px < W) {
+                        zv[j] = *reinterpret_cast<const vec_t*>(zr + (int64_t)px * ldd);
+                        gv[j] = *reinterpret_cast<const vec_t*>(gr + (int64_t)px * bn.ldy);
+                    }
+                }
+            };
+            load(0);
+            for (int x0 = 0; x0 < W; x0 += 2 * UNR) {
+#pragma unroll
+                for (int j = 0; j < NL; ++j) {
+                    if (x0 + j * PPL + vp < W) {
+                        vec_t o;
+#pragma unroll
+                        for (int e = 0; e < VC; ++e) o[e] = (T)kv[e].template dz<T>((float)zv[j][e], (float)gv[j][e]);
+                        *reinterpret_cast<vec_t*>(patch + (j * PPL + vp) * SC + vc) = o;
+                    }
+                }
+                if (x0 + 2 * UNR < W) load(x0 + 2 * UNR);
+                stem_wave_sync();
+                float a[UNR], b[UNR];
+#pragma unroll
+                for (int u = 0; u < UNR; ++u) {
+                    const bool in = x0 + 2 * u + par < W;
+                    a[u] = in ? (float)patch[(2 * u + par) * SC + k] : 0.f;
+                    b[u] = (in && k_ok) ? b0[x0 + 2 * u] : 0.f;
+                }
+#pragma unroll
+                for (int u = 0; u < UNR; ++u) acc = __builtin_amdgcn_mfma_f32_32x32x2f32(a[u], b[u], acc, 0, 0, 0);
+                stem_wave_sync();
+            }
+        } else
         for (int x0 = 0; x0 < W; x0 += 2 * UNR) {
-            float a[UNR], b[UNR];
+            float a[UNR], b[UNR], g[UNR];
 #pragma unroll
             for (int u = 0; u < UNR; ++u) {
                 const bool in = x0 + 2 * u + par < W;
                 a[u] = in ? (float)a0[(int64_t)(x0 + 2 * u) * ldd] : 0.f;
+                if constexpr (BN) g[u] = in ? (float)g0[(int64_t)(x0 + 2 * u) * bn.ldy] : 0.f;
                 b[u] = (in && k_ok) ? b0[x0 + 2 * u] : 0.f;
+            }
+            if constexpr (BN) {
+#pragma unroll
+                for (int u = 0; u < UNR; ++u) a[u] = x0 + 2 * u + par < W ? kc.dz<T>(a[u], g[u]) : 0.f;
             }
 #pragma unroll
             for (int u = 0; u < UNR; ++u) acc = __builtin_amdgcn_mfma_f32_32x32x2f32(a[u], b[u], acc, 0, 0, 0);
@@ -322,6 +429,10 @@
     static const int on = getenv("VD_STEM_WGRAD_ROWS") ? atoi(getenv("VD_STEM_WGRAD_ROWS")) : 1;
     return on && stem_rows_lds(W) <= 64 * 1024;
 }
+static bool stem_bn_vec(bool bf16) {
+    const char* e = getenv("VD_STEM_BN_VEC");
+    return e ? atoi(e) != 0 : bf16;
+}
 static int64_t stem_run_waves(int N, int H, int W) {
     const int64_t P = (int64_t)N * H * W;
     int64_t waves = vd_cdiv(P, 256);
@@ -335,8 +446,44 @@
     return (tiles + STEM_RED_CHUNKS) * SC * 32 * (int64_t)sizeof(float);
 }
 
-static int stem_wgrad_any(const float* x_nchw, const void* dz, int dz_bf16, int ldd, float* dwp, int N, int H, int W, void* ws,
-                         int64_t ws_bytes, void* stream) {
+struct stem_bn_host {
+    const void* dy;
+    int ldy;
+    const float *scale, *shift, *mean, *invstd;
+    const double* sums2;
+    double count;
+    float slope;
+};
+
+extern "C++" {
+template <typename T, bool BN>
+static void stem_wgrad_launch(const float* x_nchw, const void* dz, int ldd, const stem_bn_host& h, float* part, int N, int H, int W,
+                              int64_t* tiles, hipStream_t s) {
+    const stem_bn_args<T> bn = {(const T*)h.dy, h.ldy, h.scale, h.shift, h.mean, h.invstd, h.sums2, h.count, h.slope};
+    if (stem_rows_ok(W)) {
+        *tiles = (int64_t)N * vd_cdiv(H, SROWS);
+        const int P = stem_rows_pitch(W), lds = (int)stem_rows_lds(W), lds_vec = lds + 4 * SPATCH * (int)sizeof(T);
+        const bool vec = BN && stem_bn_vec(sizeof(T) == 2) && lds_vec <= 64 * 1024 &&
+                         (((uintptr_t)dz | (uintptr_t)h.dy | (uintptr_t)(ldd * sizeof(T)) | (uintptr_t)(h.ldy * sizeof(T))) & 15) == 0;
+        if (vec)
+            hipLaunchKernelGGL((k_stem_wgrad_rows<T, BN, BN>), dim3((unsigned)*tiles), dim3(256), lds_vec, s, x_nchw, (const T*)dz, ldd,
+                               bn, part, N, H, W, P);
+        else
+            hipLaunchKernelGGL((k_stem_wgrad_rows<T, BN>), dim3((unsigned)*tiles), dim3(256), lds, s, x_nchw, (const T*)dz, ldd, bn, part,
+                               N, H, W, P);
+    } else {
+        const int64_t P = (int64_t)N * H * W;
+        *tiles = stem_run_waves(N, H, W);
+        int64_t ppw = vd_cdiv(P, *tiles);
+        ppw = vd_cdiv(ppw, 2) * 2;
+        hipLaunchKernelGGL((k_stem_wgrad<T, BN>), dim3((unsigned)(*tiles / 4)), dim3(256), 0, s, x_nchw, (const T*)dz, ldd, bn, part,
+                           N, H, W, ppw);
+    }
+}
+}
+
+static int stem_wgrad_any(const float* x_nchw, const void* dz, int dz_bf16, int ldd, const stem_bn_host& bn, float* dwp, int N,
+                          int H, int W, void* ws, int64_t ws_bytes, void* stream) {
     VD_REQUIRE(x_nchw && dz && dwp && N > 0 && H > 0 && W > 0 && ldd >= SC, "vd_stem_wgrad: bad args");
     const int64_t need = vd_stem_wgrad_ws_bytes(N, H, W);
     if (!ws || ws_bytes < need) {
@@ -344,27 +491,13 @@
         return VD_EWORKSPACE;
     }
     hipStream_t s = (hipStream_t)stream;
-    int64_t tiles;
-    if (stem_rows_ok(W)) {
-        tiles = (int64_t)N * vd_cdiv(H, SROWS);
-        const int P = stem_rows_pitch(W), lds = (int)stem_rows_lds(W);
-        if (dz_bf16)
-            hipLaunchKernelGGL(k_stem_wgrad_rows<__bf16>, dim3((unsigned)tiles), dim3(256), lds, s, x_nchw, (const __bf16*)dz, ldd,
-                               (float*)ws, N, H, W, P);
-        else
-            hipLaunchKernelGGL(k_stem_wgrad_rows<float>, dim3((unsigned)tiles), dim3(256), lds, s, x_nchw, (const float*)dz, ldd,
-                               (float*)ws, N, H, W, P);
+    int64_t tiles = 0;
+    if (bn.dy) {
+        if (dz_bf16) stem_wgrad_launch<__bf16, true>(x_nchw, dz, ldd, bn, (float*)ws, N, H, W, &tiles, s);
+        else stem_wgrad_launch<float, true>(x_nchw, dz, ldd, bn, (float*)ws, N, H, W, &tiles, s);
     } else {
-        const int64_t P = (int64_t)N * H * W;
-        tiles = stem_run_waves(N, H, W);
-        int64_t ppw = vd_cdiv(P, tiles);
-        ppw = vd_cdiv(ppw, 2) * 2;
-        if (dz_bf16)
-            hipLaunchKernelGGL(k_stem_wgrad<__bf16>, dim3((unsigned)(tiles / 4)), dim3(256), 0, s, x_nchw, (const __bf16*)dz, ldd, (float*)ws,
-                               N, H, W, ppw);
-        else
-            hipLaunchKernelGGL(k_stem_wgrad<float>, dim3((unsigned)(tiles / 4)), dim3(256), 0, s, x_nchw, (const float*)dz, ldd, (float*)ws,
-                               N, H, W, ppw);
+        if (dz_bf16) stem_wgrad_launch<__bf16, false>(x_nchw, dz, ldd, bn, (float*)ws, N, H, W, &tiles, s);
+        else stem_wgrad_launch<float, false>(x_nchw, dz, ldd, bn, (float*)ws, N, H, W, &tiles, s);
     }
     VD_CHECK_LAUNCH("vd_stem_wgrad");
     float* lvl1 = (float*)ws + tiles * (SC * 32);
@@ -377,12 +510,28 @@
 
 int vd_stem_wgrad(const float* x_nchw, const float* dz, int ldd, float* dwp, int N, int H, int W, void* ws, int64_t ws_bytes,
                   void* stream) {
-    return stem_wgrad_any(x_nchw, dz, 0, ldd, dwp, N, H, W, ws, ws_bytes, stream);
+    return stem_wgrad_any(x_nchw, dz, 0, ldd, stem_bn_host{}, dwp, N, H, W, ws, ws_bytes, stream);
 }
 
 int vd_stem_wgrad_bf16(const float* x_nchw, const void* dz, int ldd, float* dwp, int N, int H, int W, void* ws, int64_t ws_bytes,
                        void* stream) {
-    return stem_wgrad_any(x_nchw, dz, 1, ldd, dwp, N, H, W, ws, ws_bytes, stream);
-}
-
-}
+    return stem_wgrad_any(x_nchw, dz, 1, ldd, stem_bn_host{}, dwp, N, H, W, ws, ws_bytes, stream);
+}
+
+int vd_stem_wgrad_bn(const float* x_nchw, const float* z, int ldz, const float* dy, int ldy, const float* scale, const float* shift,
+                     const float* save_mean, const float* save_invstd, const double* sums2, double count, float slope, float* dwp,
+                     int N, int H, int W, void* ws, int64_t ws_bytes, void* stream) {
+    VD_REQUIRE(dy && ldy >= SC && scale && shift && save_mean && save_invstd && sums2 && count > 0, "vd_stem_wgrad_bn: bad args");
+    const stem_bn_host bn = {dy, ldy, scale, shift, save_mean, save_invstd, sums2, count, slope};
+    return stem_wgrad_any(x_nchw, z, 0, ldz, bn, dwp, N, H, W, ws, ws_bytes, stream);
+}
+
+int vd_stem_wgrad_bn_bf16(const float* x_nchw, const void* z, int ldz, const void* dy, int ldy, const float* scale,
+                          const float* shift, const float* save_mean, const float* save_invstd, const double* sums2, double count,
+                          float slope, float* dwp, int N, int H, int W, void* ws, int64_t ws_bytes, void* stream) {
+    VD_REQUIRE(dy && ldy >= SC && scale && shift && save_mean && save_invstd && sums2 && count > 0, "vd_stem_wgrad_bn_bf16: bad args");
+    const stem_bn_host bn = {dy, ldy, scale, shift, save_mean, save_invstd, sums2, count, slope};
+    return stem_wgrad_any(x_nchw, z, 1, ldz, bn, dwp, N, H, W, ws, ws_bytes, stream);
+}
+
+}
diff --git a/viddet_amd/lib.py b/viddet_amd/lib.py
--- a/viddet_amd/lib.py
+++ b/viddet_amd/lib.py
@@ -126,6 +126,7 @@
     "vd_stem_conv_c32_bf16": (_i, [_p, _p, _p, _p, C.c_float, C.POINTER(ConvDesc), _p]),
     "vd_stem_wgrad_ws_bytes": (_i64, [_i, _i, _i]),
     "vd_stem_wgrad": (_i, [_p, _p, _i, _p, _i, _i, _i, _p, _i64, _p]),
+    "vd_stem_wgrad_bn": (_i, [_p, _p, _i, _p, _i, _p, _p, _p, _p, _p, _d, _f, _p, _i, _i, _i, _p, _i64, _p]),
     "vd_preprocess_u8_nhwc": (_i, [_p, _p, _i64, _p]),
     "vd_preprocess_u8_nchw": (_i, [_p, _p, _i, _i, _i, _p]),
     "vd_temporal_pool": (_i, [_p, _p, _p, _i, _i, _i64, _i, _p]),
@@ -162,6 +163,7 @@
     "vd_pack_weight_dgrad_bf16": (_i, [_p, _p, _i, _i, _i, _i, _i, _i, C.POINTER(C.c_int32), _i, _i, _p]),
     "vd_upsample2x_concat_bwd_bf16": (_i, [_p, _p, _p, _i, _i, _i, _i, _i, _p]),
     "vd_stem_wgrad_bf16": (_i, [_p, _p, _i, _p, _i, _i, _i, _p, _i64, _p]),
+    "vd_stem_wgrad_bn_bf16": (_i, [_p, _p, _i, _p, _i, _p, _p, _p, _p, _p, _d, _f, _p, _i, _i, _i, _p, _i64, _p]),
     "vd_yolo_loss_fwd_bwd_bf16": (_i, [C.POINTER(HeadDesc), _p, _i, _p, _p, _p, _p, _p, _f, _i, _p,
                                        C.POINTER(_fp * 3), _p, _p, _i64, _p]),
     "vd_temporal_pool_idx": (_i, [_p, _p, _p, _i, _i, _i, _i64, _i, _p]),
diff --git a/viddet_amd/model.py b/viddet_amd/model.py
--- a/viddet_amd/model.py
+++ b/viddet_amd/model.py
@@ -29,9 +29,9 @@
         self.keep = []
         self.streams = []
 
-    def add(self, fname, *args, meta=None, stream=None):
+    def add(self, fname, *args, meta=None, stream=None, label=None):
         fn = getattr(L.load(), fname)
-        self.recs.append((fname, fn, args))
+        self.recs.append((label or fname, fn, args))
         self.meta.append(meta)
         self.streams.append(stream)
 
@@ -1359,7 +1359,8 @@
             self._wamax_dirty = False
 
     def _buffers(self, key, B, H, W, train, bf16=False):
-        ck = ('buf', B, H, W, train) + (('bf16',) if bf16 else ())
+        stem_dz = train and not train_plan.stem_fuse_bwd()
+        ck = ('buf', B, H, W, train) + (('bf16',) if bf16 else ()) + (('stem_dz',) if stem_dz else ())
         if ck in self._programs:
             return self._programs[ck]
         dev = self.device
@@ -1407,8 +1408,10 @@
                 if name != 'in':
                     bufs['d:' + name] = (torch.zeros_like if 'd:' + name in zeroed else torch.empty_like)(bufs[name], dtype=dt)
             mx = max(bufs[n.dst].numel() for n in self.conv_nodes)
-            bufs['dz'] = torch.empty(mx, dtype=dt, device=dev)
-            bufs['dz2'] = torch.empty(mx, dtype=dt, device=dev)
+            mz = mx if stem_dz else max(bufs[n.dst].numel() for n in self.conv_nodes
+                                        if not (n.stem and n.bn and not getattr(n, 'tvalid', False)))
+            bufs['dz'] = torch.empty(mz, dtype=dt, device=dev)
+            bufs['dz2'] = torch.empty(mz, dtype=dt, device=dev)
             bufs['tmp'] = torch.empty(mx, dtype=dt, device=dev)
         for nm, t in bufs.items():
             if torch.is_tensor(t) and t.dtype == dt and not nm.startswith('amax') and nm not in zeroed:
@@ -1476,6 +1479,8 @@
         new = {}
         for i, n in enumerate(bn):
             for k, name in ((0, n.tdw.dst if getattr(n, 'tdw', None) is not None else n.dst), (1, 'dz:' + n.name)):
+                if k == 1 and n.stem:
+                    continue
                 if fl[2 * i + k] and name not in self._range_exact:
                     new[name] = float(ra[2 * i + k])
         if new:
diff --git a/viddet_amd/ops.py b/viddet_amd/ops.py
--- a/viddet_amd/ops.py
+++ b/viddet_amd/ops.py
@@ -278,6 +278,13 @@
     N, _, H, W = x_nchw.shape
     fn = _lib().vd_stem_wgrad_bf16 if dz.dtype == torch.bfloat16 else _lib().vd_stem_wgrad
     check(fn(ptr(x_nchw), ptr(dz), dz.shape[-1], ptr(dwp), N, H, W, ptr(ws), ws.numel() * ws.element_size(), _s()), "vd_stem_wgrad")
+
+
+def stem_wgrad_bn(x_nchw, z, dy, scale, shift, smean, sinv, sums2, count, dwp, ws, slope=0.1):
+    N, _, H, W = x_nchw.shape
+    fn = _lib().vd_stem_wgrad_bn_bf16 if z.dtype == torch.bfloat16 else _lib().vd_stem_wgrad_bn
+    check(fn(ptr(x_nchw), ptr(z), z.shape[-1], ptr(dy), dy.shape[-1], ptr(scale), ptr(shift), ptr(smean), ptr(sinv), ptr(sums2),
+             float(count), slope, ptr(dwp), N, H, W, ptr(ws), ws.numel() * ws.element_size(), _s()), "vd_stem_wgrad_bn")
 
 
 def bn_stats(x2d_rows, C_, x, sums, ws):
diff --git a/viddet_amd/train_plan.py b/viddet_amd/train_plan.py
--- a/viddet_amd/train_plan.py
+++ b/viddet_amd/train_plan.py
@@ -25,6 +25,11 @@
         self.parity_streams = env.get('VD_PARITY_STREAMS', '1') == '1'
         self.fuse_bwd_s2 = env.get('VD_FUSE_BWD_S2', '1') == '1'
         self.autotune = env.get('VD_AUTOTUNE', '1') != '0'
+        self.stem_fuse_bwd = stem_fuse_bwd(env)
+
+
+def stem_fuse_bwd(env=os.environ):
+    return env.get('VD_STEM_FUSE_BWD', '1') == '1'
 
 
 class TrainPlan:
@@ -325,15 +330,15 @@
             if not self.net.alias_skip_grad:
                 self.materialize(n.residual)
 
-    def side_launch(self, *wargs, meta):
+    def side_launch(self, *wargs, meta, label=None):
         seg, side = self.seg, self.side
         if side is None:
-            seg.add(*wargs, self.ws.data_ptr(), self.ws_bytes, meta=meta)
+            seg.add(*wargs, self.ws.data_ptr(), self.ws_bytes, meta=meta, label=label)
             return None
         e_ready, e_done = torch.cuda.Event(), torch.cuda.Event()
         seg.add_py(ev_record(e_ready))
         seg.add_py(ev_wait(e_ready, side))
-        seg.add(*wargs, self.ws_w.data_ptr(), self.ws_bytes, meta=meta, stream=side)
+        seg.add(*wargs, self.ws_w.data_ptr(), self.ws_bytes, meta=meta, stream=side, label=label)
         seg.add_py(ev_record(e_done, side))
         seg.hold(e_ready, e_done)
         self.last_side = e_done
@@ -564,12 +569,12 @@
         self.seg.add('vd_bn_param_grads', sums.data_ptr(), n.co_pad, self.bufs['tmp'].data_ptr(), n.gbias.data_ptr())
         return dz
 
+    def stem_fused(self, n):
+        return self.sw.stem_fuse_bwd and n.stem and n.bn and not getattr(n, 'tvalid', False)
+
     def bn_backward(self, n, dy):
         seg, bufs, sfx, M = self.seg, self.bufs, self.sfx, self.out_rows(n)
         z = bufs['z:' + n.dst]
-        slot = self.n_dz % 2
-        self.n_dz += 1
-        dz = self.dz_bufs[slot][:M * n.cout].view(-1, self.H // n.div_out, self.W // n.div_out, n.cout)
         bn = (n.b_scale.data_ptr(), n.b_shift.data_ptr(), n.b_mean.data_ptr(), n.b_invstd.data_ptr())
         if n.name not in self.fused_bwd:
             seg.add('vd_bn_bwd_reduce' + sfx, z.data_ptr(), dy.data_ptr(), *bn, M, n.cout, LEAKY_SLOPE, n.sums2.data_ptr(),
@@ -579,6 +584,13 @@
         if self.net._syncbn(n):
             seg.add_coll(self.net._syncbn_exchange(n.sums2))
             count = float(M * self.world)
+        if self.stem_fused(n):
+            self.stem_bn = (z, dy, bn, count)
+            return None, None
+        slot = self.n_dz % 2
+        self.n_dz += 1
+        assert M * n.cout <= self.dz_bufs[slot].numel(), "dz scratch too small for " + n.name
+        dz = self.dz_bufs[slot][:M * n.cout].view(-1, self.H // n.div_out, self.W // n.div_out, n.cout)
         if self.side is not None and self.dz_free[slot] is not None:
             seg.add_py(ev_wait(self.dz_free[slot]))
         seg.add('vd_bn_bwd_apply' + sfx, z.data_ptr(), dy.data_ptr(), *bn, n.sums2.data_ptr(), count, M, n.cout, LEAKY_SLOPE,
@@ -592,7 +604,13 @@
     def conv_wgrad(self, n, dz, slot):
         net, bufs, B, H, W = self.net, self.bufs, self.B, self.H, self.W
         Hi, Wi = H // n.div_in, W // n.div_in
-        if n.stem:
+        label = None
+        if n.stem and dz is None:
+            z, dy, bn, count = self.stem_bn
+            label = 'vd_stem_wgrad' + self.sfx
+            wargs = ('vd_stem_wgrad_bn' + self.sfx, bufs['in'].data_ptr(), z.data_ptr(), z.shape[-1], dy.data_ptr(), dy.shape[-1],
+                     *bn, n.sums2.data_ptr(), count, LEAKY_SLOPE, n.gwp.data_ptr(), B * n.fr, Hi, Wi)
+        elif n.stem:
             wargs = ('vd_stem_wgrad' + self.sfx, bufs['in'].data_ptr(), dz.data_ptr(), n.co_pad, n.gwp.data_ptr(),
                      B * n.fr, Hi, Wi)
         else:
@@ -611,8 +629,11 @@
                 autotune_wgrad(wd_, self.ws.data_ptr(), self.ws_bytes)
             self.seg.hold(wd_)
             wargs = ('vd_conv_wgrad', C.byref(wd_))
-        e_done = self.side_launch(*wargs, meta=net._flops(n, B, H, W, 'wgrad', self.esz))
-        if e_done is not None and not n.head:
+        meta = net._flops(n, B, H, W, 'wgrad', self.esz)
+        if label is not None:
+            meta['bytes'] += float(self.esz) * self.stem_bn[0].numel()
+        e_done = self.side_launch(*wargs, meta=meta, label=label)
+        if e_done is not None and slot is not None:
             self.dz_free[slot] = e_done
         self.close_bucket(n, n is self.first_wtrain or n.stem)
 
```

New measurement: 1057 frames/s (median of 6 runs). 1.3% higher.
